# better62/MM-VQA-Healthcare

Hardware: AMD Instinct MI355X
Metric: image-question pairs/sec, M3AE-base fine-tune step (fwd+bwd+AdamW) @384px (higher is better)
Workload: dtype bf16

## Files before the change

include/m3ae_hip.h:

```cpp
#ifndef M3AE_HIP_H
#define M3AE_HIP_H

#include <stdint.h>

#ifdef __cplusplus
extern "C" {
#endif

#define M3AE_ABI_VERSION 4

enum { M3AE_F32 = 0, M3AE_BF16 = 1 };
enum { M3AE_ACT_NONE = 0, M3AE_ACT_GELU = 1, M3AE_ACT_QUICKGELU = 2, M3AE_ACT_TANH = 3, M3AE_ACT_RELU = 4,
       M3AE_ACT_MULAUX = 5  };
enum { M3AE_ERR_ARG = -1, M3AE_ERR_UNSUPPORTED = -2, M3AE_ERR_ALIGN = -3, M3AE_ERR_WORKSPACE = -4 };

int m3ae_abi_version(void);
void m3ae_desc_sizes(int64_t out3[3]);
const char* m3ae_last_gemm_path(void);

typedef struct {
    int64_t M, N, K;
    int64_t batch1, batch2;
    const void* A; int64_t a_sm, a_sk, a_sb1, a_sb2;
    const void* B; int64_t b_sk, b_sn, b_sb1, b_sb2;
    void* C;       int64_t c_sm, c_sn, c_sb1, c_sb2;
    int32_t dtype_a, dtype_b, dtype_c;
    float alpha;
    int32_t accumulate;
    const float* bias;
    int32_t act;
    void* preact;
    const void* residual;
    const void* dact_aux;
    int32_t dact;
    int32_t force_generic;
    float* a_rowsum;
    float dropout_p;
    uint64_t dropout_seed;
    int32_t preact_grad;
    int32_t launch_flags;
    const void* dropout_salt;
} m3ae_gemm_desc;
enum { M3AE_GEMM_NO_PERSISTENT = 1,
       M3AE_GEMM_F32_X3 = 2,
       M3AE_GEMM_DETERMINISTIC = 4  };
#define M3AE_GEMM_NT_VARIANT(v) ((((v) + 1) & 0xf) << 8)
#define M3AE_GEMM_TN_VARIANT(v) ((((v) + 1) & 0xf) << 12)
#define M3AE_GEMM_COL_GROUP(g) (((g) & 0xf) << 16)
int m3ae_gemm(const m3ae_gemm_desc* d, void* stream);
int m3ae_gemm_rows(const m3ae_gemm_desc* d, int64_t row_base, int64_t row_step, void* stream);
int64_t m3ae_gemm_det_workspace_bytes(const m3ae_gemm_desc* d);
int m3ae_gemm_det(const m3ae_gemm_desc* d, void* workspace, int64_t workspace_bytes, void* stream);

typedef struct {
    int64_t B, H, Lq, Lk, Dh;
    const void* q; int64_t q_sb, q_sl;
    const void* k; int64_t k_sb, k_sl;
    const void* v; int64_t v_sb, v_sl;
    void* o;       int64_t o_sb, o_sl;
    const float* key_mask;
    const float* pos_bias;
    float scale;
    int32_t causal;
    float* lse; int64_t lse_stride;
    int32_t dtype;
    void* workspace; int64_t workspace_bytes;
    const void* d_o;
    void* dq; void* dk; void* dv;
    float* delta;
    float* d_pos_bias;
    float dropout_p;
    uint64_t dropout_seed;
    const void* dropout_salt;
    int32_t launch_flags;
} m3ae_attn_desc;
enum { M3AE_ATTN_LEGACY_KERNELS = 1,
       M3AE_ATTN_F32_X3 = 2    };
int64_t m3ae_attn_workspace_bytes(const m3ae_attn_desc* d, int backward);
int m3ae_attn_fwd(const m3ae_attn_desc* d, void* stream);
int m3ae_attn_bwd(const m3ae_attn_desc* d, void* stream);
int m3ae_attn_fwd_rows(const m3ae_attn_desc* d, int64_t row_base, int64_t row_step, void* stream);
int m3ae_attn_bwd_rows(const m3ae_attn_desc* d, int64_t row_base, int64_t row_step, void* stream);
int m3ae_attn_probs(const m3ae_attn_desc* d, float* probs, int64_t p_sb, int64_t p_sh, int64_t p_sq, void* stream);

typedef struct {
    int32_t dir;
    int64_t B, Lq, Lk, D, H;
    const void* x;
    const void* y;
    const float* key_mask;
    const void *wq, *wq_t, *wkv, *wkv_t, *wo, *wo_t;
    const float *bq, *bkv, *bo, *ln_g, *ln_b;
    float ln_eps;
    float dropout_p;
    uint64_t seed_attn, seed_hidden;
    void* proj;
    void* prime;
    float* colbias;
    void* probs;
    void* probs_drop;
    float* rowsum;
    void* zctx;
    void* ctx;
    void* s;
    void* out;
    float *mean, *rstd;
    const void* d_out;
    void* dx;
    void* dy;
    float *g_wq, *g_wkv, *g_wo, *g_bq, *g_bkv, *g_bo, *g_ln_g, *g_ln_b;
    void* ws_ds;
    void* ws_dsd;
    void* ws_dscores;
    void* ws_dprime;
    void* ws_dproj;
    void* ws_dz;
    void* ws_dctx;
    float* ws_vec;
    float* ws_ln;
    int32_t launch_flags;
    const void* dropout_salt;
} m3ae_xattn_desc;
enum { M3AE_XATTN_NO_PERSISTENT = 1,
       M3AE_XATTN_LEGACY_CHAIN = 2     };
int m3ae_xattn_supported(const m3ae_xattn_desc* d);
int m3ae_xattn_bwd_supported(const m3ae_xattn_desc* d);
int64_t m3ae_xattn_probs_ld(const m3ae_xattn_desc* d);
int m3ae_xattn_fwd(const m3ae_xattn_desc* d, void* stream);
int m3ae_xattn_bwd(const m3ae_xattn_desc* d, void* stream);
int m3ae_xattn_probs_export(const m3ae_xattn_desc* d, int dropped, float* out, int64_t o_sb, int64_t o_sh, int64_t o_sq,
                            void* stream);

int m3ae_layernorm_fwd(const void* x, const float* gamma, const float* beta, void* y, float* mean, float* rstd,
                       int64_t M, int64_t D, float eps, int dtype, int act, int rms, void* stream);
int64_t m3ae_layernorm_bwd_blocks(int64_t M);
int m3ae_layernorm_bwd(const void* dy, const void* x, const float* gamma, const float* beta, const float* mean,
                       const float* rstd, void* dx, const void* dx_add, float* dgamma, float* dbeta, float* workspace,
                       int64_t M, int64_t D, int dtype, int act, int rms, void* stream);
int m3ae_layernorm_bwd_drop(const void* dy, const void* x, const float* gamma, const float* beta, const float* mean,
                            const float* rstd, void* dx, void* dx_drop, float dropout_p, uint64_t dropout_seed,
                            const void* dropout_salt, float* dgamma, float* dbeta, float* workspace, int64_t M, int64_t D,
                            int dtype, void* stream);
int m3ae_layernorm_bwd_drop_rows(const void* dy, const void* x, const float* gamma, const float* beta, const float* mean,
                                 const float* rstd, void* dx, void* dx_drop, float dropout_p, uint64_t dropout_seed,
                                 const void* dropout_salt, float* dgamma, float* dbeta, float* workspace, int64_t M, int64_t D,
                                 int dtype, int64_t row_base, int64_t row_step, void* stream);
int m3ae_layernorm_fwd_mixed(const float* x, const float* gamma, const float* beta, void* y, float* mean, float* rstd,
                             int64_t M, int64_t D, float eps, void* stream);
int m3ae_layernorm_bwd_mixed(const void* dy, const float* x, const float* gamma, const float* mean, const float* rstd,
                             float* dx, const float* dx_add, void* dx_lo, float* dgamma, float* dbeta, float* workspace,
                             int64_t M, int64_t D, void* stream);
int m3ae_layernorm_bwd_mixed_det(const void* dy, const float* x, const float* gamma, const float* mean, const float* rstd,
                                 float* dx, const float* dx_add, void* dx_lo, float* dgamma, float* dbeta, float* workspace,
                                 int64_t M, int64_t D, void* stream);
int m3ae_dropout(const void* x, void* out, uint8_t* keep_mask, int64_t rows, int64_t cols, float p, uint64_t seed,
                 const void* salt, int dtype, void* stream);
int m3ae_dropout_rows(const void* x, void* out, uint8_t* keep_mask, int64_t rows, int64_t cols, float p, uint64_t seed,
                      const void* salt, int dtype, int64_t row_base, int64_t row_step, void* stream);

int m3ae_colsum(const void* x, float* out, int64_t M, int64_t N, int64_t ldx, int dtype, int accumulate,
                void* stream);

int m3ae_roberta_embed_fwd(const int64_t* ids, const float* word, const float* pos, const float* type, void* out,
                           int64_t B, int64_t S, int64_t D, int64_t pad_id, int dtype, void* stream);
int m3ae_roberta_embed_bwd(const int64_t* ids, const void* d_out, float* d_word, float* d_pos, float* d_type,
                           int64_t B, int64_t S, int64_t D, int64_t pad_id, int dtype, void* stream);

int m3ae_patchify(const float* img, void* out, int64_t B, int64_t R, int64_t P, int dtype, void* stream);
int m3ae_image_normalize_u8(const uint8_t* in, float* out, int64_t B, int64_t H, int64_t W, const float* mean3,
                            const float* std3, void* stream);
int64_t m3ae_image_resample_workspace_bytes(int64_t total_rows, int64_t size);
int m3ae_image_resample_u8(const uint8_t* src, int64_t src_bytes, const int64_t* plan, const int32_t* tab, int64_t tab_ints, int64_t B,
                           int64_t size, uint8_t* workspace, int64_t workspace_bytes, float* out, uint8_t* out_u8,
                           const float* mean3, const float* std3, void* stream);
int m3ae_vit_tokens_fwd(const void* patch, const float* cls, const float* pos, void* out, int64_t B, int64_t G,
                        int64_t D, int dtype, void* stream);
int m3ae_vit_tokens_bwd(const void* d_out, void* d_patch, float* d_cls, float* d_pos, int64_t B, int64_t G,
                        int64_t D, int dtype, void* stream);

int m3ae_bce_logits(const void* logits, const float* targets, float* loss, void* d_logits, int64_t B, int64_t C,
                    float grad_scale, int dtype, void* stream);
int m3ae_xent(const void* logits, const int64_t* labels, float* loss, void* d_logits, float* workspace,
              int64_t rows, int64_t C, int64_t ld, float grad_scale, int dtype, void* stream);

int m3ae_adamw(float* p, const float* g, float* m, float* v, void* shadow_bf16, int64_t n, float lr, float beta1,
               float beta2, float eps, float wd, int64_t step, float grad_scale, const float* hyper_dev, void* stream);

int m3ae_cast_transpose(const float* in, void* out, void* out_t, int64_t R, int64_t C, void* stream);
int m3ae_cast_transpose_batched(const void* jobs_dev, int njobs, int64_t total_tiles, void* stream);
int m3ae_transpose_bf16_batched(const void* jobs_dev, int njobs, int64_t total_tiles, void* stream);
int m3ae_cast(const void* in, void* out, int64_t n, int dtype_in, int dtype_out, void* stream);
int m3ae_zero(void* p, int64_t bytes, void* stream);
int m3ae_add(const void* a, const void* b, void* out, int64_t n, int dtype, void* stream);
int m3ae_act_fwd(const void* x, void* y, int64_t n, int act, int dtype, void* stream);
int m3ae_act_bwd(const void* dy, const void* x_pre, void* dx, int64_t n, int act, int dtype, void* stream);
int m3ae_gather_rows(const void* in, const int64_t* idx, void* out, int64_t n_out, int64_t D, int dtype,
                     void* stream);
int m3ae_scatter_add_rows(const void* d_out, const int64_t* idx, void* d_in, int64_t n_out, int64_t D, int dtype,
                          void* stream);

int m3ae_mask_ranks(const float* noise, int64_t* ids_restore, int64_t* keep_rows, float* mask, int64_t B, int64_t L,
                    int64_t len_keep, void* stream);
int m3ae_mim_targets(const float* img, float* out, int64_t B, int64_t C, int64_t H, int64_t W, int64_t P, int norm_pix,
                     void* stream);
int m3ae_mim_loss_fwd(const void* x, const float* target, const float* mask, float* acc, float* loss, int64_t B, int64_t L,
                      int64_t D, int dtype, void* stream);
int m3ae_mim_loss_bwd(const void* x, const float* target, const float* mask, const float* acc, const float* gout, void* dx,
                      int64_t B, int64_t L, int64_t D, int dtype, void* stream);

enum { M3AE_DET_COLSUM = 0, M3AE_DET_EMBED_BWD = 1, M3AE_DET_BCE = 2, M3AE_DET_XENT = 3, M3AE_DET_MIM = 4 };
int64_t m3ae_det_workspace_bytes(int op, int64_t rows, int64_t cols);
int m3ae_colsum_det(const void* x, float* out, int64_t M, int64_t N, int64_t ldx, int dtype, int accumulate, void* workspace,
                    int64_t workspace_bytes, void* stream);
int m3ae_layernorm_bwd_det(const void* dy, const void* x, const float* gamma, const float* beta, const float* mean,
                           const float* rstd, void* dx, const void* dx_add, float* dgamma, float* dbeta, float* workspace,
                           int64_t M, int64_t D, int dtype, int act, int rms, void* stream);
int m3ae_layernorm_bwd_drop_det(const void* dy, const void* x, const float* gamma, const float* beta, const float* mean,
                                const float* rstd, void* dx, void* dx_drop, float dropout_p, uint64_t dropout_seed,
                                const void* dropout_salt, float* dgamma, float* dbeta, float* workspace, int64_t M, int64_t D,
                                int dtype, void* stream);
int m3ae_roberta_embed_bwd_det(const int64_t* ids, const void* d_out, float* d_word, float* d_pos, float* d_type, int64_t B,
                               int64_t S, int64_t D, int64_t pad_id, int dtype, void* workspace, int64_t workspace_bytes,
                               void* stream);
int m3ae_bce_logits_det(const void* logits, const float* targets, float* loss, void* d_logits, int64_t B, int64_t C,
                        float grad_scale, int dtype, void* workspace, int64_t workspace_bytes, void* stream);
int m3ae_xent_det(const void* logits, const int64_t* labels, float* loss, void* d_logits, int64_t rows, int64_t C, int64_t ld,
                  float grad_scale, int dtype, void* workspace, int64_t workspace_bytes, void* stream);
int m3ae_mim_loss_fwd_det(const void* x, const float* target, const float* mask, float* acc, float* loss, int64_t B, int64_t L,
                          int64_t D, int dtype, void* workspace, int64_t workspace_bytes, void* stream);

int64_t m3ae_beam_topk_workspace_bytes(int64_t B, int64_t nb, int64_t V, int64_t chunk);
int m3ae_beam_topk(const float* logits, int64_t ld, const float* beam_scores, int64_t B, int64_t nb, int64_t V, int64_t chunk,
                   void* workspace, int64_t workspace_bytes, float* top_s, int32_t* top_i, void* stream);
int m3ae_beam_step(const float* top_s, const int32_t* top_i, const int64_t* ids_in, int64_t* ids_out, int64_t* last_tok,
                   float* beam_scores, int64_t* order, int32_t* done, int32_t* n_hyp, double* hyp_score, int32_t* hyp_len,
                   int64_t* hyp_tok, int32_t* open_count, int64_t* err, int64_t B, int64_t nb, int64_t V, int64_t max_length,
                   int64_t cur_len, int64_t eos, int64_t pad, double div, void* stream);
int m3ae_beam_finalize(const int64_t* ids, const float* beam_scores, const int32_t* done, int32_t* n_hyp, double* hyp_score,
                       int32_t* hyp_len, int64_t* hyp_tok, int64_t* seq, int64_t* len, int64_t B, int64_t nb, int64_t max_length,
                       int64_t cur_len, int64_t eos, int64_t pad, double div, void* stream);

int m3ae_expand_samples(const void* in, const int64_t* src, void* out, int64_t n_out, int64_t n_in, int64_t R, int dtype,
                        void* stream);
int m3ae_segment_sum_rows(const void* d_out, const int64_t* offsets, const int64_t* members, void* d_in, int64_t n_in,
                          int64_t n_out, int64_t R, int dtype, void* stream);

int m3ae_selftest(int32_t* out, void* stream);

#ifdef __cplusplus
}
#endif
#endif
```

mm-vqa-healthcare_amd/csrc/common.h:

```cpp
#pragma once
#include <hip/hip_runtime.h>
#include <stdint.h>
#include "m3ae_hip.h"

typedef uint16_t bf16_t;
typedef __attribute__((ext_vector_type(2))) float f32x2;
typedef __attribute__((ext_vector_type(4))) float f32x4;
typedef __attribute__((ext_vector_type(16))) float f32x16;
typedef __attribute__((ext_vector_type(4))) short s16x4;
typedef __attribute__((ext_vector_type(8))) short s16x8;
typedef __attribute__((ext_vector_type(8))) __bf16 bf16x8_t;
typedef __attribute__((ext_vector_type(4))) unsigned int u32x4;
typedef __attribute__((ext_vector_type(2))) unsigned int u32x2;

#define DEVINL __device__ __forceinline__

DEVINL float bf2f(bf16_t h) { return __uint_as_float(((uint32_t)h) << 16); }
DEVINL bf16_t f2bf(float f) {
    __bf16 b = (__bf16)f;
    return __builtin_bit_cast(bf16_t, b);
}
typedef __attribute__((ext_vector_type(2))) __bf16 bf16x2_t;
DEVINL uint32_t pack2bf(float lo, float hi) {
    const bf16x2_t v = __builtin_convertvector((f32x2){lo, hi}, bf16x2_t);
    return __builtin_bit_cast(uint32_t, v);
}

template <typename T> struct Elem;
template <> struct Elem<float> {
    static DEVINL float ld(const float* p) { return *p; }
    static DEVINL void st(float* p, float v) { *p = v; }
};
template <> struct Elem<bf16_t> {
    static DEVINL float ld(const bf16_t* p) { return bf2f(*p); }
    static DEVINL void st(bf16_t* p, float v) { *p = f2bf(v); }
};

DEVINL float act_fwd(float x, int act) {
    switch (act) {
        case M3AE_ACT_GELU: return 0.5f * x * (1.0f + erff(x * 0.70710678118654752440f));
        case M3AE_ACT_QUICKGELU: return x / (1.0f + expf(-1.702f * x));
        case M3AE_ACT_TANH: return tanhf(x);
        case M3AE_ACT_RELU: return x > 0.f ? x : 0.f;
        default: return x;
    }
}
DEVINL float act_bwd(float x, int act) {
    switch (act) {
        case M3AE_ACT_GELU: {
            float cdf = 0.5f * (1.0f + erff(x * 0.70710678118654752440f));
            float pdf = 0.39894228040143267794f * expf(-0.5f * x * x);
            return cdf + x * pdf;
        }
        case M3AE_ACT_QUICKGELU: {
            float s = 1.0f / (1.0f + expf(-1.702f * x));
            return s * (1.0f + 1.702f * x * (1.0f - s));
        }
        case M3AE_ACT_TANH: {
            float t = tanhf(x);
            return 1.0f - t * t;
        }
        case M3AE_ACT_MULAUX: return x;
        case M3AE_ACT_RELU: return x > 0.f ? 1.f : 0.f;
        default: return 1.0f;
    }
}

DEVINL void gelu_terms_fast(float x, float& cdf, float& pdf) {
    const float z = fabsf(x) * 0.70710678118654752440f;
    const float t = __builtin_amdgcn_rcpf(fmaf(0.3275911f, z, 1.0f));
    const float e = __builtin_amdgcn_exp2f(x * x * -0.72134752044448170368f);
    float poly = fmaf(1.061405429f, t, -1.453152027f);
    poly = fmaf(poly, t, 1.421413741f);
    poly = fmaf(poly, t, -0.284496736f);
    poly = fmaf(poly, t, 0.254829592f);
    const float half_erfc = 0.5f * poly * t * e;
    cdf = x < 0.f ? half_erfc : 1.0f - half_erfc;
    pdf = 0.39894228040143267794f * e;
}
DEVINL float act_fwd_fast(float x, int act) {
    if (act == M3AE_ACT_GELU) {
        float cdf, pdf;
        gelu_terms_fast(x, cdf, pdf);
        return x * cdf;
    }
    if (act == M3AE_ACT_QUICKGELU) return x * __builtin_amdgcn_rcpf(1.0f + __builtin_amdgcn_exp2f(-2.45546695959f * x));
// ... 153 lines not shown
```

mm-vqa-healthcare_amd/csrc/gemm_generic.hip:

```cpp
#include "common.h"

namespace {

constexpr int TM = 64, TN = 64, TK = 16, PAD = 4;

template <typename TA, typename TB, typename TC>
__global__ __launch_bounds__(256) void gemm_generic_kernel(m3ae_gemm_desc d, int64_t row_base, int64_t row_step) {
    __shared__ float As[TK][TM + PAD];
    __shared__ float Bs[TK][TN + PAD];
    const int tid = threadIdx.x;
    const int tx = tid & 15, ty = tid >> 4;
    const int64_t m0 = (int64_t)blockIdx.y * TM, n0 = (int64_t)blockIdx.x * TN;
    const int64_t b1 = blockIdx.z / d.batch2, b2 = blockIdx.z % d.batch2;
    const TA* A = (const TA*)d.A + b1 * d.a_sb1 + b2 * d.a_sb2;
    const TB* B = (const TB*)d.B + b1 * d.b_sb1 + b2 * d.b_sb2;
    const int64_t coff = b1 * d.c_sb1 + b2 * d.c_sb2;
    const bool a_kfast = (d.a_sk == 1), b_nfast = (d.b_sn == 1);

    float acc[4][4];
#pragma unroll
    for (int i = 0; i < 4; ++i)
#pragma unroll
        for (int j = 0; j < 4; ++j) acc[i][j] = 0.f;
    const bool do_rowsum = d.a_rowsum != nullptr && blockIdx.x == 0 && tx == 0;
    float rs[4] = {0.f, 0.f, 0.f, 0.f};

    for (int64_t k0 = 0; k0 < d.K; k0 += TK) {
#pragma unroll
        for (int i = 0; i < 4; ++i) {
            int e = tid + i * 256;
            int mm, kk;
            if (a_kfast) { kk = e & 15; mm = e >> 4; } else { mm = e & 63; kk = e >> 6; }
            int64_t gm = m0 + mm, gk = k0 + kk;
            float v = 0.f;
            if (gm < d.M && gk < d.K) v = Elem<TA>::ld(A + gm * d.a_sm + gk * d.a_sk);
            As[kk][mm] = v;
        }
#pragma unroll
        for (int i = 0; i < 4; ++i) {
            int e = tid + i * 256;
            int nn, kk;
            if (b_nfast) { nn = e & 63; kk = e >> 6; } else { kk = e & 15; nn = e >> 4; }
            int64_t gn = n0 + nn, gk = k0 + kk;
            float v = 0.f;
            if (gn < d.N && gk < d.K) v = Elem<TB>::ld(B + gk * d.b_sk + gn * d.b_sn);
            Bs[kk][nn] = v;
        }
        __syncthreads();
#pragma unroll
        for (int kk = 0; kk < TK; ++kk) {
            float a[4], b[4];
#pragma unroll
            for (int i = 0; i < 4; ++i) a[i] = As[kk][ty * 4 + i];
#pragma unroll
            for (int j = 0; j < 4; ++j) b[j] = Bs[kk][tx * 4 + j];
#pragma unroll
            for (int i = 0; i < 4; ++i)
#pragma unroll
                for (int j = 0; j < 4; ++j) acc[i][j] = fmaf(a[i], b[j], acc[i][j]);
            if (do_rowsum) {
#pragma unroll
                for (int i = 0; i < 4; ++i) rs[i] += a[i];
            }
        }
        __syncthreads();
    }
    if (do_rowsum) {
#pragma unroll
        for (int i = 0; i < 4; ++i) {
            const int64_t gm = m0 + ty * 4 + i;
            if (gm < d.M) d.a_rowsum[gm] += rs[i];
        }
    }

    DropState drop = make_drop_dev(d.dropout_p, d.dropout_seed, d.dropout_salt, row_base, row_step);
    drop_resolve(drop);
    TC* C = (TC*)d.C + coff;
    TC* P = d.preact ? (TC*)d.preact + coff : nullptr;
    const TC* R = d.residual ? (const TC*)d.residual + coff : nullptr;
    const TC* X = d.dact_aux ? (const TC*)d.dact_aux + coff : nullptr;
#pragma unroll
    for (int i = 0; i < 4; ++i) {
        int64_t gm = m0 + ty * 4 + i;
        if (gm >= d.M) continue;
#pragma unroll
        for (int j = 0; j < 4; ++j) {
            int64_t gn = n0 + tx * 4 + j;
            if (gn >= d.N) continue;
            int64_t off = gm * d.c_sm + gn * d.c_sn;
            float x = acc[i][j] * d.alpha;
            if (d.bias) x += d.bias[gn];
            if (P) Elem<TC>::st(P + off, d.preact_grad ? act_bwd(x, d.act) : x);
            x = act_fwd(x, d.act);
            if (d.dropout_p > 0.f) x = drop_apply(drop, (uint64_t)(drop_row(drop, gm) * drop_ld(d.N) + gn), x);
            if (R) x += Elem<TC>::ld(R + off);
            if (X) x *= act_bwd(Elem<TC>::ld(X + off), d.dact);
            if (d.accumulate) x += Elem<TC>::ld(C + off);
            Elem<TC>::st(C + off, x);
        }
    }
}

template <typename TA, typename TB, typename TC>
int launch(const m3ae_gemm_desc& d, hipStream_t s, DropRows rows) {
    dim3 grid((unsigned)cdiv(d.N, TN), (unsigned)cdiv(d.M, TM), (unsigned)(d.batch1 * d.batch2));
    if (grid.y > 65535u || grid.z > 65535u) return M3AE_ERR_UNSUPPORTED;
    hipLaunchKernelGGL((gemm_generic_kernel<TA, TB, TC>), grid, dim3(256), 0, s, d, rows.base, rows.step);
    return hip_launch_status();
}

}

int m3ae_gemm_generic(const m3ae_gemm_desc& d, hipStream_t s, DropRows rows) {
    if (d.dtype_a != d.dtype_b) return M3AE_ERR_UNSUPPORTED;
    if (d.dtype_a == M3AE_F32 && d.dtype_c == M3AE_F32) return launch<float, float, float>(d, s, rows);
    if (d.dtype_a == M3AE_BF16 && d.dtype_c == M3AE_BF16) return launch<bf16_t, bf16_t, bf16_t>(d, s, rows);
    if (d.dtype_a == M3AE_BF16 && d.dtype_c == M3AE_F32) return launch<bf16_t, bf16_t, float>(d, s, rows);
    return M3AE_ERR_UNSUPPORTED;
}
```

mm-vqa-healthcare_amd/csrc/gemm_mfma.hip:

```cpp
#include "gemm_nt_common.h"
#include "launch.h"
#include <stdlib.h>

namespace {

constexpr int BM = 128, BN = 128, BK = 64;
constexpr int STAGE_BYTES = (BM + BN) * BK * 2;
constexpr int LDS_BYTES = 2 * STAGE_BYTES;

using namespace m3g;

template <int BM_, int BN_, int BKT, int NST, int WM, int EPI>
__global__ __launch_bounds__((BM_ / WM) * (BN_ / 64) * 64, 2) void gemm_nt_bf16_kernel(MfmaArgs a) {
    if (a.has_drop) drop_resolve(a.drop);
    constexpr int WAVES_N = BN_ / 64, NWAVES = (BM_ / WM) * WAVES_N, MI = WM / 16;
    constexpr int A_BYTES = BM_ * BKT * 2, ST_BYTES = (BM_ + BN_) * BKT * 2;
    constexpr int A_SEGS = A_BYTES / 1024 / NWAVES, B_SEGS = BN_ * BKT * 2 / 1024 / NWAVES;
    constexpr int G = A_SEGS + B_SEGS;
    extern __shared__ __attribute__((aligned(16))) char smem[];
    const int tid = threadIdx.x;
    const int lane = tid & 63;
    const int wave = __builtin_amdgcn_readfirstlane(tid >> 6);
    const int wr = wave / WAVES_N, wc = wave % WAVES_N;

    const unsigned tiles_n = (unsigned)((a.N + BN_ - 1) / BN_);
    unsigned tm, tn;
    nt_tile_coords(xcd_remap(blockIdx.x, gridDim.x), gridDim.x / tiles_n, tiles_n, tm, tn);
    const int64_t m0 = (int64_t)tm * BM_;
    const int64_t n0 = (int64_t)tn * BN_;

    f32x4 acc[MI][4];
#pragma unroll
    for (int i = 0; i < MI; ++i)
#pragma unroll
        for (int j = 0; j < 4; ++j) acc[i][j] = (f32x4){0.f, 0.f, 0.f, 0.f};

    const int nt = (int)(a.K / BKT);
#pragma unroll
    for (int s = 0; s < NST - 1; ++s) {
        if (s < nt) {
            nt_stage<BKT, A_SEGS, NWAVES>(a.A, a.lda, m0, a.M, (int64_t)s * BKT, smem + s * ST_BYTES, wave, lane);
            nt_stage<BKT, B_SEGS, NWAVES>(a.B, a.ldb, n0, a.N, (int64_t)s * BKT, smem + s * ST_BYTES + A_BYTES, wave, lane);
        }
    }

    const int frow = lane & 15, fchunk = lane >> 4;
    int cur_s = 0, nxt_s = NST - 1;
    for (int t = 0; t < nt; ++t) {
        if (t + NST - 2 < nt) asm volatile("s_waitcnt vmcnt(%0)" ::"n"((NST - 2) * G) : "memory");
        else asm volatile("s_waitcnt vmcnt(0)" ::: "memory");
        __builtin_amdgcn_s_barrier();
        asm volatile("" ::: "memory");
        if (t + NST - 1 < nt) {
            char* nxt = smem + nxt_s * ST_BYTES;
            nt_stage<BKT, A_SEGS, NWAVES>(a.A, a.lda, m0, a.M, (int64_t)(t + NST - 1) * BKT, nxt, wave, lane);
            nt_stage<BKT, B_SEGS, NWAVES>(a.B, a.ldb, n0, a.N, (int64_t)(t + NST - 1) * BKT, nxt + A_BYTES, wave, lane);
        }
        const char* At = smem + cur_s * ST_BYTES;
        const char* Bt = At + A_BYTES;
#pragma unroll
        for (int kk = 0; kk < BKT / 32; ++kk) {
            s16x8 af[MI], bfr[4];
#pragma unroll
            for (int j = 0; j < 4; ++j) bfr[j] = nt_frag<BKT>(Bt, wc * 64 + j * 16 + frow, kk * 4 + fchunk);
#pragma unroll
            for (int i = 0; i < MI; ++i) af[i] = nt_frag<BKT>(At, wr * WM + i * 16 + frow, kk * 4 + fchunk);
#pragma unroll
            for (int i = 0; i < MI; ++i)
#pragma unroll
                for (int j = 0; j < 4; ++j)
                    acc[i][j] = __builtin_amdgcn_mfma_f32_16x16x32_bf16(
                        __builtin_bit_cast(bf16x8_t, bfr[j]), __builtin_bit_cast(bf16x8_t, af[i]), acc[i][j], 0, 0, 0);
        }
        asm volatile("" ::: "memory");
        cur_s = cur_s + 1 == NST ? 0 : cur_s + 1;
        nxt_s = nxt_s + 1 == NST ? 0 : nxt_s + 1;
    }

    if (a.rows_epi) {
        __builtin_amdgcn_s_barrier();
        asm volatile("" ::: "memory");
        if (a.c_f32) epilogue_rows<float, EPI, MI>(a, smem, wave, lane, m0 + wr * WM, n0 + wc * 64, acc);
        else epilogue_rows<bf16_t, EPI, MI>(a, smem, wave, lane, m0 + wr * WM, n0 + wc * 64, acc);
        return;
    }
#pragma unroll
    for (int i = 0; i < MI; ++i) {
        const int64_t m = m0 + wr * WM + i * 16 + (lane & 15);
        if (m >= a.M) continue;
#pragma unroll
        for (int j = 0; j < 4; ++j) {
            const int64_t n = n0 + wc * 64 + j * 16 + 4 * (lane >> 4);
            if (n >= a.N) continue;
            if (a.c_f32) epilogue4<float, EPI>(a, m, n, acc[i][j]);
            else epilogue4<bf16_t, EPI>(a, m, n, acc[i][j]);
        }
    }
}

template <int BM_, int BN_, int WM, int BKR, int NST, bool DET = false>
__global__ __launch_bounds__((BM_ / WM) * (BN_ / 64) * 64, 2) void gemm_tn_bf16_kernel(MfmaArgs a) {
    constexpr int WAVES_N = BN_ / 64, NWAVES = (BM_ / WM) * WAVES_N, MI = WM / 16;
    constexpr int A_BYTES = BM_ * BKR * 2, ST_BYTES = (BM_ + BN_) * BKR * 2;
    constexpr int A_SEGS = A_BYTES / 1024 / NWAVES, B_SEGS = BN_ * BKR * 2 / 1024 / NWAVES;
    constexpr int G = A_SEGS + B_SEGS;
    extern __shared__ __attribute__((aligned(16))) char smem[];
    const int tid = threadIdx.x;
    const int lane = tid & 63;
    const int wave = __builtin_amdgcn_readfirstlane(tid >> 6);
    const int wr = wave / WAVES_N, wc = wave % WAVES_N;

    const unsigned tiles_n = (unsigned)(a.N / BN_);
    const unsigned tiles = (unsigned)(a.M / BM_) * tiles_n;
    const unsigned wg = xcd_remap(blockIdx.x, gridDim.x);
    const unsigned tile_id = wg % tiles, split = wg / tiles;
    const int64_t m0 = (int64_t)(tile_id / tiles_n) * BM_;
    const int64_t n0 = (int64_t)(tile_id % tiles_n) * BN_;
    const int64_t r_begin = (int64_t)split * a.k_chunk;
    int64_t r_end = r_begin + a.k_chunk;
    if (r_end > a.K) r_end = a.K;
    if (r_begin >= r_end) return;
    const int nt = (int)((r_end - r_begin + BKR - 1) / BKR);

    f32x4 acc[MI][4];
#pragma unroll
    for (int i = 0; i < MI; ++i)
#pragma unroll
        for (int j = 0; j < 4; ++j) acc[i][j] = (f32x4){0.f, 0.f, 0.f, 0.f};

    const bool do_rowsum = a.a_rowsum != nullptr && n0 == 0 && wc == 0;
    f32x4 rsum[MI];
#pragma unroll
    for (int i = 0; i < MI; ++i) rsum[i] = (f32x4){0.f, 0.f, 0.f, 0.f};
    const s16x8 ones = {0x3F80, 0x3F80, 0x3F80, 0x3F80, 0x3F80, 0x3F80, 0x3F80, 0x3F80};

#pragma unroll
    for (int s = 0; s < NST - 1; ++s) {
        if (s < nt) {
            const int64_t r0 = r_begin + (int64_t)s * BKR;
// ... 45 lines not shown
#pragma unroll
            for (int i = 0; i < MI; ++i) *(f32x4*)(rs + i * 16) = rsum[i];
        }
        float* P = (float*)a.C + ((int64_t)split * tiles + tile_id) * (BM_ * BN_) + ((int64_t)wave * MI * 4 * 64 + lane) * 4;
#pragma unroll
        for (int i = 0; i < MI; ++i)
#pragma unroll
            for (int j = 0; j < 4; ++j) *(f32x4*)(P + (i * 4 + j) * 256) = acc[i][j];
        return;
    }
    if (do_rowsum && (lane & 15) == 0) {
#pragma unroll
        for (int i = 0; i < MI; ++i)
#pragma unroll
            for (int r = 0; r < 4; ++r) atomicAdd(a.a_rowsum + m0 + wr * WM + i * 16 + 4 * (lane >> 4) + r, rsum[i][r]);
    }

    float* C = (float*)a.C;
    const bool atomic = a.splits > 1;
#pragma unroll
    for (int i = 0; i < MI; ++i)
#pragma unroll
        for (int j = 0; j < 4; ++j)
#pragma unroll
            for (int r = 0; r < 4; ++r) {
                const int64_t n1 = m0 + wr * WM + i * 16 + 4 * (lane >> 4) + r;
                const int64_t n2 = n0 + wc * 64 + j * 16 + (lane & 15);
                float* p = C + n1 * a.ldc + n2;
                const float x = acc[i][j][r] * a.alpha;
                if (atomic) atomicAdd(p, x);
                else if (a.accumulate) *p += x;
                else *p = x;
            }
}

}

static thread_local const char* g_last_path = "none";
const char* m3ae_last_gemm_path(void) { return g_last_path; }

int m3ae_gemm_generic(const m3ae_gemm_desc& d, hipStream_t s, DropRows rows = DropRows{0, 1});
int m3ae_gemm_f32x3(const m3ae_gemm_desc& d, hipStream_t s, DropRows rows = DropRows{0, 1});

static bool aligned16(const void* p) { return (((uintptr_t)p) & 15) == 0; }


template <int BM_, int BN_, int BKT, int NST, int WM, int EPI>
static int launch_nt_t(const MfmaArgs& a, hipStream_t s) {
    constexpr int nwaves = (BM_ / WM) * (BN_ / 64);
    constexpr int ring = NST * (BM_ + BN_) * BKT * 2, slabs = nwaves * 32 * 68 * 4;
    constexpr int lds = ring > slabs ? ring : slabs;
    constexpr int threads = nwaves * 64;
    const int64_t tiles = cdiv(a.M, BM_) * cdiv(a.N, BN_);
    return launch_dyn<gemm_nt_bf16_kernel<BM_, BN_, BKT, NST, WM, EPI>>(dim3((unsigned)tiles), dim3(threads), lds, s, a);
}


#if defined(M3AE_EXP_NT_NODMA)
#define PP_STAGE(G, ld, r0, nr, k0, tile) do { } while (0)
#elif defined(M3AE_EXP_NT_CONTIG)
template <int BKT, int SEGS_PER_WAVE, int NWAVES>
DEVINL void nt_stage_contig(const bf16_t* G, int64_t ld, int64_t row0, int64_t nrows, int64_t k0, char* tile, int wave, int lane) {
    constexpr int CPR = BKT / 8, RPS = 64 / CPR;
#pragma unroll
    for (int q = 0; q < SEGS_PER_WAVE; ++q) {
        const int seg = q * NWAVES + wave;
        const int row = seg * RPS + lane / CPR;
        int64_t grow = row0 + row;
        grow = grow < nrows ? grow : nrows - 1;
        glds16(G + (k0 / BKT) * nrows * BKT + grow * BKT + (lane % CPR) * 8, tile + seg * 1024);
    }
}
#ifdef M3AE_EXP_NT_L2HOT
#define PP_STAGE(G, ld, r0, nr, k0, tile) nt_stage_contig<CK, 2, NW>(G, ld, 0, nr, k0, tile, wave, lane)
#else
#define PP_STAGE(G, ld, r0, nr, k0, tile) nt_stage_contig<CK, 2, NW>(G, ld, r0, nr, k0, tile, wave, lane)
#endif
#elif defined(M3AE_EXP_NT_L2HOT)
#define PP_STAGE(G, ld, r0, nr, k0, tile) nt_stage<CK, 2, NW>(G, ld, 0, nr, k0, tile, wave, lane)
#else
#define PP_STAGE(G, ld, r0, nr, k0, tile) nt_stage<CK, 2, NW>(G, ld, r0, nr, k0, tile, wave, lane)
#endif

template <int EPI>
__global__ __launch_bounds__(512, 2) void gemm_nt_pp_kernel(MfmaArgs a) {
    if (a.has_drop) drop_resolve(a.drop);
    constexpr int CK = 32, NW = 8, A_BYTES = 256 * CK * 2, SLOT = 2 * A_BYTES;
    extern __shared__ __attribute__((aligned(16))) char smem[];
    const int tid = threadIdx.x;
    const int lane = tid & 63;
    const int wave = __builtin_amdgcn_readfirstlane(tid >> 6);
    const int wr = wave >> 2, wc = wave & 3;

    const unsigned tiles_n = (unsigned)((a.N + 255) / 256);
    unsigned tm, tn;
    nt_tile_coords(xcd_remap(blockIdx.x, gridDim.x), gridDim.x / tiles_n, tiles_n, tm, tn, (unsigned)a.col_group);
    const int64_t m0 = (int64_t)tm * 256;
    const int64_t n0 = (int64_t)tn * 256;

    f32x4 acc[8][4];
#pragma unroll
    for (int i = 0; i < 8; ++i)
#pragma unroll
        for (int j = 0; j < 4; ++j) acc[i][j] = (f32x4){0.f, 0.f, 0.f, 0.f};

    const int nc = (int)(a.K / CK);
#pragma unroll
    for (int c = 0; c < 3; ++c) {
        if (c < nc) {
            PP_STAGE(a.B, a.ldb, n0, a.N, (int64_t)c * CK, smem + c * SLOT + A_BYTES);
            PP_STAGE(a.A, a.lda, m0, a.M, (int64_t)c * CK, smem + c * SLOT);
        }
    }
    if (nc >= 3) asm volatile("s_waitcnt vmcnt(8)" ::: "memory");
    else if (nc == 2) asm volatile("s_waitcnt vmcnt(4)" ::: "memory");
    else asm volatile("s_waitcnt vmcnt(0)" ::: "memory");
    PP_FENCE();
    __builtin_amdgcn_s_barrier();
    PP_FENCE();
    if (wr == 1) { __builtin_amdgcn_s_barrier(); PP_FENCE(); }

    const int frow = lane & 15, fchunk = lane >> 4;
    for (int c = 0; c < nc; ++c) {
        const char* At = smem + (c & 3) * SLOT;
        const char* Bt = At + A_BYTES;
        char* nxt = smem + ((c + 3) & 3) * SLOT;
        const bool more = c + 3 < nc;
        s16x8 bfr[4], af[4];
#pragma unroll
        for (int j = 0; j < 4; ++j) bfr[j] = nt_frag<CK>(Bt, wc * 64 + j * 16 + frow, fchunk);
#pragma unroll
        for (int i = 0; i < 4; ++i) af[i] = nt_frag<CK>(At, wr * 128 + i * 16 + frow, fchunk);
        if (more) PP_STAGE(a.B, a.ldb, n0, a.N, (int64_t)(c + 3) * CK, nxt + A_BYTES);
        PP_FENCE();
        __builtin_amdgcn_s_barrier();
        PP_FENCE();
        asm volatile("s_waitcnt lgkmcnt(0)" ::: "memory");
        __builtin_amdgcn_sched_barrier(0);
        __builtin_amdgcn_s_setprio(1);
#pragma unroll
        for (int i = 0; i < 4; ++i)
#pragma unroll
            for (int j = 0; j < 4; ++j)
                acc[i][j] = __builtin_amdgcn_mfma_f32_16x16x32_bf16(
                    __builtin_bit_cast(bf16x8_t, bfr[j]), __builtin_bit_cast(bf16x8_t, af[i]), acc[i][j], 0, 0, 0);
        __builtin_amdgcn_s_setprio(0);
        PP_FENCE();
        __builtin_amdgcn_s_barrier();
        PP_FENCE();
#pragma unroll
        for (int i = 0; i < 4; ++i) af[i] = nt_frag<CK>(At, wr * 128 + 64 + i * 16 + frow, fchunk);
        if (more) PP_STAGE(a.A, a.lda, m0, a.M, (int64_t)(c + 3) * CK, nxt);
        {
            const int rem = nc - 1 - c;
            if (rem >= 3) asm volatile("s_waitcnt vmcnt(8)" ::: "memory");
            else if (rem == 2) asm volatile("s_waitcnt vmcnt(4)" ::: "memory");
            else asm volatile("s_waitcnt vmcnt(0)" ::: "memory");
        }
        PP_FENCE();
        __builtin_amdgcn_s_barrier();
        PP_FENCE();
        asm volatile("s_waitcnt lgkmcnt(0)" ::: "memory");
        __builtin_amdgcn_sched_barrier(0);
        __builtin_amdgcn_s_setprio(1);
#pragma unroll
        for (int i = 0; i < 4; ++i)
#pragma unroll
            for (int j = 0; j < 4; ++j)
                acc[4 + i][j] = __builtin_amdgcn_mfma_f32_16x16x32_bf16(
                    __builtin_bit_cast(bf16x8_t, bfr[j]), __builtin_bit_cast(bf16x8_t, af[i]), acc[4 + i][j], 0, 0, 0);
        __builtin_amdgcn_s_setprio(0);
        PP_FENCE();
        __builtin_amdgcn_s_barrier();
        PP_FENCE();
    }
    if (wr == 0) { __builtin_amdgcn_s_barrier(); PP_FENCE(); }

    if (a.rows_epi) {
        if (a.c_f32) epilogue_rows<float, EPI, 8>(a, smem, wave, lane, m0 + wr * 128, n0 + wc * 64, acc);
        else epilogue_rows<bf16_t, EPI, 8>(a, smem, wave, lane, m0 + wr * 128, n0 + wc * 64, acc);
        return;
    }
#pragma unroll
    for (int i = 0; i < 8; ++i) {
        const int64_t m = m0 + wr * 128 + i * 16 + (lane & 15);
        if (m >= a.M) continue;
#pragma unroll
        for (int j = 0; j < 4; ++j) {
            const int64_t n = n0 + wc * 64 + j * 16 + 4 * (lane >> 4);
            if (n >= a.N) continue;
            if (a.c_f32) epilogue4<float, EPI>(a, m, n, acc[i][j]);
            else epilogue4<bf16_t, EPI>(a, m, n, acc[i][j]);
        }
    }
}

template <int EPI>
static int launch_nt_pp(const MfmaArgs& a, hipStream_t s) {
    constexpr int lds = 4 * (256 + 256) * 32 * 2;
    const int64_t tiles = cdiv(a.M, 256) * cdiv(a.N, 256);
    g_last_path = "mfma_nt_pp";
    return launch_dyn<gemm_nt_pp_kernel<EPI>>(dim3((unsigned)tiles), dim3(512), lds, s, a);
}


#ifdef M3AE_NT_TRACE
__device__ uint64_t g_nt_trace[1024 * 2 * 8];
#define NT_CLK() ({ __builtin_amdgcn_sched_barrier(0); uint64_t t_ = __builtin_readcyclecounter(); __builtin_amdgcn_sched_barrier(0); t_; })
#define NT_ACC(i) do { const uint64_t n_ = NT_CLK(); nt_acc[i] += n_ - nt_t; nt_t = n_; } while (0)
#else
#define NT_ACC(i) do { } while (0)
#endif

template <int EPI>
__global__ __launch_bounds__(512, 2) void gemm_nt_pp_persistent_kernel(MfmaArgs a) {
    if (a.has_drop) drop_resolve(a.drop);
    constexpr int CK = 32, NW = 8, A_BYTES = 256 * CK * 2, SLOT = 2 * A_BYTES;
    extern __shared__ __attribute__((aligned(16))) char smem[];
    const int tid = threadIdx.x;
    const int lane = tid & 63;
    const int wave = __builtin_amdgcn_readfirstlane(tid >> 6);
    const int wr = wave >> 2, wc = wave & 3;
    const unsigned tiles_n = (unsigned)((a.N + 255) / 256);
    const unsigned tiles_m = (unsigned)((a.M + 255) / 256);
    const unsigned total = tiles_m * tiles_n;
    const int nc = (int)(a.K / CK);
    const int frow = lane & 15, fchunk = lane >> 4;

    unsigned v = blockIdx.x;
    unsigned tm, tn;
    nt_tile_coords(xcd_remap(v, total), tiles_m, tiles_n, tm, tn, (unsigned)a.col_group);
    int64_t m0 = (int64_t)tm * 256, n0 = (int64_t)tn * 256;
#pragma unroll
    for (int c = 0; c < 3; ++c) {
        char* sl = smem + ((c + 2) & 3) * SLOT;
        PP_STAGE(a.B, a.ldb, n0, a.N, (int64_t)c * CK, sl + A_BYTES);
        PP_STAGE(a.A, a.lda, m0, a.M, (int64_t)c * CK, sl);
    }
    int top_wait = 0;
#ifdef M3AE_NT_TRACE
    uint64_t nt_acc[8] = {0, 0, 0, 0, 0, 0, 0, 0}, nt_t = 0;
#endif
    const int interior_wait = a.c_f32 ? 1 : (a.preact ? 3 : 2);
    for (;;) {
        f32x4 acc[8][4];
#pragma unroll
        for (int i = 0; i < 8; ++i)
#pragma unroll
            for (int j = 0; j < 4; ++j) acc[i][j] = (f32x4){0.f, 0.f, 0.f, 0.f};
        if (top_wait == 0) asm volatile("s_waitcnt vmcnt(8)" ::: "memory");
        else if (top_wait == 2) asm volatile("s_waitcnt vmcnt(20)" ::: "memory");
        else if (top_wait == 3) asm volatile("s_waitcnt vmcnt(36)" ::: "memory");
        else asm volatile("s_waitcnt vmcnt(4)" ::: "memory");
        PP_FENCE();
        __builtin_amdgcn_s_barrier();
        PP_FENCE();
        if (wr == 1) { __builtin_amdgcn_s_barrier(); PP_FENCE(); }
#ifdef M3AE_NT_TRACE
        nt_t = NT_CLK();
#endif
        for (int c = 0; c < nc; ++c) {
            const char* At = smem + ((c + 2) & 3) * SLOT;
            const char* Bt = At + A_BYTES;
            char* nxt = smem + ((c + 5) & 3) * SLOT;
            const bool more = c + 3 < nc;
            s16x8 bfr[4], af[4];
#pragma unroll
            for (int j = 0; j < 4; ++j) bfr[j] = nt_frag<CK>(Bt, wc * 64 + j * 16 + frow, fchunk);
#pragma unroll
            for (int i = 0; i < 4; ++i) af[i] = nt_frag<CK>(At, wr * 128 + i * 16 + frow, fchunk);
            NT_ACC(0);
            if (more) PP_STAGE(a.B, a.ldb, n0, a.N, (int64_t)(c + 3) * CK, nxt + A_BYTES);
            NT_ACC(1);
            PP_FENCE();
            __builtin_amdgcn_s_barrier();
            PP_FENCE();
            NT_ACC(2);
            asm volatile("s_waitcnt lgkmcnt(0)" ::: "memory");
            __builtin_amdgcn_sched_barrier(0);
            NT_ACC(3);
            __builtin_amdgcn_s_setprio(1);
#pragma unroll
            for (int i = 0; i < 4; ++i)
#pragma unroll
                for (int j = 0; j < 4; ++j)
                    acc[i][j] = __builtin_amdgcn_mfma_f32_16x16x32_bf16(
                        __builtin_bit_cast(bf16x8_t, bfr[j]), __builtin_bit_cast(bf16x8_t, af[i]), acc[i][j], 0, 0, 0);
            __builtin_amdgcn_s_setprio(0);
            NT_ACC(4);
            PP_FENCE();
            __builtin_amdgcn_s_barrier();
            PP_FENCE();
            NT_ACC(5);
#pragma unroll
            for (int i = 0; i < 4; ++i) af[i] = nt_frag<CK>(At, wr * 128 + 64 + i * 16 + frow, fchunk);
            NT_ACC(0);
            if (more) PP_STAGE(a.A, a.lda, m0, a.M, (int64_t)(c + 3) * CK, nxt);
            NT_ACC(1);
            {
                const int rem = nc - 1 - c;
                if (rem >= 3) asm volatile("s_waitcnt vmcnt(8)" ::: "memory");
                else if (rem == 2) asm volatile("s_waitcnt vmcnt(4)" ::: "memory");
                else asm volatile("s_waitcnt vmcnt(0)" ::: "memory");
            }
            NT_ACC(6);
            PP_FENCE();
            __builtin_amdgcn_s_barrier();
            PP_FENCE();
            NT_ACC(2);
            asm volatile("s_waitcnt lgkmcnt(0)" ::: "memory");
            __builtin_amdgcn_sched_barrier(0);
            NT_ACC(3);
            __builtin_amdgcn_s_setprio(1);
#pragma unroll
            for (int i = 0; i < 4; ++i)
#pragma unroll
                for (int j = 0; j < 4; ++j)
                    acc[4 + i][j] = __builtin_amdgcn_mfma_f32_16x16x32_bf16(
                        __builtin_bit_cast(bf16x8_t, bfr[j]), __builtin_bit_cast(bf16x8_t, af[i]), acc[4 + i][j], 0, 0, 0);
            __builtin_amdgcn_s_setprio(0);
            NT_ACC(4);
            PP_FENCE();
            __builtin_amdgcn_s_barrier();
            PP_FENCE();
            NT_ACC(5);
        }
#ifdef M3AE_NT_TRACE
        nt_acc[7] += (uint64_t)nc;
#endif
        if (wr == 0) { __builtin_amdgcn_s_barrier(); PP_FENCE(); }
        const unsigned vn = v + gridDim.x;
        const bool again = vn < total;
        const int64_t m_cur = m0, n_cur = n0;
        if (again) {
            nt_tile_coords(xcd_remap(vn, total), tiles_m, tiles_n, tm, tn, (unsigned)a.col_group);
            m0 = (int64_t)tm * 256; n0 = (int64_t)tn * 256;
#pragma unroll
            for (int c = 0; c < 2; ++c) {
                char* sl = smem + ((c + 2) & 3) * SLOT;
                PP_STAGE(a.B, a.ldb, n0, a.N, (int64_t)c * CK, sl + A_BYTES);
                PP_STAGE(a.A, a.lda, m0, a.M, (int64_t)c * CK, sl);
            }
        }
        if (a.c_f32) epilogue_rows<float, EPI, 8, 1>(a, smem, wave, lane, m_cur + wr * 128, n_cur + wc * 64, acc);
        else epilogue_rows<bf16_t, EPI, 8, 1>(a, smem, wave, lane, m_cur + wr * 128, n_cur + wc * 64, acc);
#ifdef M3AE_NT_TRACE
        if (!again && lane == 0 && (wave & 3) == 0 && blockIdx.x < 1024)
            for (int q_ = 0; q_ < 8; ++q_) g_nt_trace[((size_t)blockIdx.x * 2 + wr) * 8 + q_] = nt_acc[q_];
#endif
        if (!again) break;
        top_wait = (m_cur + 256 <= a.M && n_cur + 256 <= a.N) ? interior_wait : 1;
        PP_FENCE();
        __builtin_amdgcn_s_barrier();
        PP_FENCE();
        {
            char* sl = smem + ((2 + 2) & 3) * SLOT;
            PP_STAGE(a.B, a.ldb, n0, a.N, (int64_t)2 * CK, sl + A_BYTES);
            PP_STAGE(a.A, a.lda, m0, a.M, (int64_t)2 * CK, sl);
        }
        v = vn;
    }
}

template <int EPI>
static int launch_nt_pp_persistent(const MfmaArgs& a, hipStream_t s) {
    constexpr int lds = 4 * (256 + 256) * 32 * 2;
    g_last_path = "mfma_nt_pp";
    const int dev = current_device();
    return launch_dyn_on<gemm_nt_pp_persistent_kernel<EPI>>(dev, dim3((unsigned)device_cus8(dev)), dim3(512), lds, s, a);
}

template <int EPI>
static int launch_nt_v(const MfmaArgs& a, hipStream_t s) {
    const int g_nt_variant = a.nt_variant;
    if (g_nt_variant < 0) {
        const int64_t t256 = cdiv(a.M, 256) * cdiv(a.N, 256), t128 = cdiv(a.M, 128) * cdiv(a.N, 128);
        const double eff256 = (double)t256 / (double)(cdiv(t256, 256) * 256);
        const double eff128 = (double)t128 / (double)(cdiv(t128, 512) * 512);
        const bool big = a.M > 128 && a.N > 128 && eff256 >= 0.93 * eff128;
        const bool persist_ok = t256 >= 512;
        if (big && a.rows_epi && a.K >= 256) {
            g_last_path = "mfma_nt_pp2";
            return launch_nt_pp2(a, EPI, persist_ok && !a.no_persist, s);
        }
        if (big && persist_ok && !a.no_persist && a.rows_epi && a.K >= 96) return launch_nt_pp_persistent<EPI>(a, s);
        if (big) return launch_nt_pp<EPI>(a, s);
        return launch_nt_t<128, 128, 64, 2, 64, EPI>(a, s);
    }
    if ((g_nt_variant == 9 || g_nt_variant == 10) && a.M > 128 && a.N > 128 && a.rows_epi && a.K >= 256) {
        g_last_path = "mfma_nt_pp2";
        return launch_nt_pp2(a, EPI, g_nt_variant == 10, s);
    }
    if (g_nt_variant == 7 && a.M > 128 && a.N > 128) return launch_nt_pp<EPI>(a, s);
    if (g_nt_variant == 8 && a.rows_epi && a.K >= 96 && cdiv(a.M, 256) * cdiv(a.N, 256) >= 512)
        return launch_nt_pp_persistent<EPI>(a, s);
    if (g_nt_variant == 8 && a.M > 128 && a.N > 128) return launch_nt_pp<EPI>(a, s);
    if (g_nt_variant == 4 && a.M > 128 && a.N > 128) return launch_nt_t<256, 256, 64, 2, 128, EPI>(a, s);
    return launch_nt_t<128, 128, 64, 2, 64, EPI>(a, s);
}

static int launch_nt(const m3ae_gemm_desc& d, hipStream_t s, DropRows rows) {
    MfmaArgs a{};
    a.A = (const bf16_t*)d.A; a.lda = d.a_sm;
    a.B = (const bf16_t*)d.B; a.ldb = d.b_sn;
    a.C = d.C; a.ldc = d.c_sm;
    a.M = d.M; a.N = d.N; a.K = d.K;
    a.c_f32 = d.dtype_c == M3AE_F32;
    a.alpha = d.alpha; a.accumulate = d.accumulate; a.bias = d.bias; a.act = d.act; a.preact = d.preact;
    a.preact_grad = d.preact_grad;
    a.residual = d.residual; a.dact_aux = d.dact_aux; a.dact = d.dact;
    a.rows_epi = (d.N % 8 == 0 && d.c_sm % 8 == 0) ? 1 : 0;
    {
        const int tiles_n = (int)((d.N + 255) / 256);
        const int g_nt_col_group = (d.launch_flags >> 16) & 0xf;
        a.col_group = g_nt_col_group > 0 ? g_nt_col_group : (tiles_n <= 9 ? tiles_n : 6);
    }
    a.has_drop = d.dropout_p > 0.f;
    a.drop = make_drop(d.dropout_p, d.dropout_seed, d.dropout_salt, rows);
    a.no_persist = (d.launch_flags & M3AE_GEMM_NO_PERSISTENT) ? 1 : 0;
    a.nt_variant = ((d.launch_flags >> 8) & 0xf) - 1;
    a.st_policy = (d.launch_flags >> 20) & 0x3;
    if (a.st_policy == 0) a.st_policy = (d.M * d.N >= (int64_t)16 << 20) ? 3 : 1;
    const bool has_act = d.act != M3AE_ACT_NONE, has_dact = d.dact_aux != nullptr;
    if (!has_act && !has_dact && !d.preact) return launch_nt_v<EPI_PLAIN>(a, s);
    if (!has_dact && d.act == M3AE_ACT_RELU) return launch_nt_v<EPI_RELU>(a, s);
    if (!has_act && has_dact && d.dact == M3AE_ACT_MULAUX) return launch_nt_v<EPI_DMUL>(a, s);
    if (a.has_drop) return launch_nt_v<EPI_ANY>(a, s);
    if (!has_dact && d.act == M3AE_ACT_GELU) return launch_nt_v<EPI_GELU>(a, s);
    if (!has_dact && d.act == M3AE_ACT_QUICKGELU) return launch_nt_v<EPI_QGELU>(a, s);
    if (!has_act && d.dact == M3AE_ACT_GELU) return launch_nt_v<EPI_DGELU>(a, s);
    if (!has_act && d.dact == M3AE_ACT_QUICKGELU) return launch_nt_v<EPI_DQGELU>(a, s);
    return launch_nt_v<EPI_ANY>(a, s);
}


#ifdef M3AE_TN_TRACE
__device__ uint64_t g_tn_trace[512 * 2 * 16];
#define TN_STAMP(k) do { if (tn_tr) g_tn_trace[((size_t)blockIdx.x * 2 + wr) * 16 + (k)] = __builtin_readcyclecounter(); } while (0)
extern "C" int m3ae_tn_trace_dump(uint64_t* out) {
    hipDeviceSynchronize();
    hipMemcpyFromSymbol(out, HIP_SYMBOL(g_tn_trace), sizeof(uint64_t) * 512 * 2 * 16);
    static uint64_t zeros[512 * 2 * 16];
    hipMemcpyToSymbol(HIP_SYMBOL(g_tn_trace), zeros, sizeof(zeros));
    return 0;
}
#else
#define TN_STAMP(k) do { } while (0)
#endif
template <bool DET>
__global__ __launch_bounds__(512, 2) void gemm_tn_pp_kernel(MfmaArgs a) {
    constexpr int CK = 32, NW = 8, A_BYTES = 256 * CK * 2, SLOT = 2 * A_BYTES;
    extern __shared__ __attribute__((aligned(16))) char smem[];
    const int tid = threadIdx.x;
    const int lane = tid & 63;
    const int wave = __builtin_amdgcn_readfirstlane(tid >> 6);
    const int wr = wave >> 2, wc = wave & 3;

    const unsigned tiles_n = (unsigned)(a.N / 256);
    const unsigned tiles = (unsigned)(a.M / 256) * tiles_n;
    const unsigned wg = xcd_remap(blockIdx.x, gridDim.x);
    const unsigned tile_id = wg % tiles, split = wg / tiles;
    const int64_t m0 = (int64_t)(tile_id / tiles_n) * 256;
    const int64_t n0 = (int64_t)(tile_id % tiles_n) * 256;
    const int64_t r_begin = (int64_t)split * a.k_chunk;
    int64_t r_end = r_begin + a.k_chunk;
    if (r_end > a.K) r_end = a.K;
    if (r_begin >= r_end) return;
    const int nc = (int)((r_end - r_begin + CK - 1) / CK);

    f32x4 acc[8][4];
#pragma unroll
    for (int i = 0; i < 8; ++i)
#pragma unroll
        for (int j = 0; j < 4; ++j) acc[i][j] = (f32x4){0.f, 0.f, 0.f, 0.f};
    const bool do_rowsum = a.a_rowsum != nullptr && n0 == 0 && wc == 0;
    f32x4 rsum[8];
#pragma unroll
    for (int i = 0; i < 8; ++i) rsum[i] = (f32x4){0.f, 0.f, 0.f, 0.f};
    const s16x8 ones = {0x3F80, 0x3F80, 0x3F80, 0x3F80, 0x3F80, 0x3F80, 0x3F80, 0x3F80};

#pragma unroll
    for (int c = 0; c < 3; ++c) {
        if (c < nc) {
            const int64_t r0 = r_begin + (int64_t)c * CK;
            tn_stage<256, 2, NW>(a.B, a.ldb, r0, r_end, n0, smem + c * SLOT + A_BYTES, wave, lane);
            tn_stage<256, 2, NW>(a.A, a.lda, r0, r_end, m0, smem + c * SLOT, wave, lane);
        }
    }
    if (nc >= 3) asm volatile("s_waitcnt vmcnt(8)" ::: "memory");
    else if (nc == 2) asm volatile("s_waitcnt vmcnt(4)" ::: "memory");
    else asm volatile("s_waitcnt vmcnt(0)" ::: "memory");
    PP_FENCE();
    __builtin_amdgcn_s_barrier();
    PP_FENCE();
    if (wr == 1) { __builtin_amdgcn_s_barrier(); PP_FENCE(); }

    for (int c = 0; c < nc; ++c) {
#ifdef M3AE_TN_TRACE
        const bool tn_tr = (c == 64 || c == 65) && lane == 0 && wc == 0 && blockIdx.x < 512;
        if (tn_tr && c == 65) g_tn_trace[((size_t)blockIdx.x * 2 + wr) * 16 + 8] = __builtin_readcyclecounter();
#undef TN_STAMP
#define TN_STAMP(k) do { if (tn_tr && c == 64) g_tn_trace[((size_t)blockIdx.x * 2 + wr) * 16 + (k)] = __builtin_readcyclecounter(); } while (0)
#endif
// ... 206 lines not shown
    if (splits > ksteps / min_steps) splits = ksteps / min_steps;
    if (splits < 1) splits = 1;
    if (!d.accumulate) splits = 1;
    const int64_t steps_per = cdiv(ksteps, splits);
    *k_chunk = steps_per * 64;
    return cdiv(ksteps, steps_per);
}

template <int BM_, int BN_, int WM, int BKR, int NST>
static int launch_tn_t(MfmaArgs a, const m3ae_gemm_desc& d, hipStream_t s, float* det_ws = nullptr) {
    static_assert(BM_ == 128 && BN_ == 128, "tn_t_splits and tn_det_fold assume the 128 x 128 tile");
    constexpr int lds = tn_t_lds(NST, BKR);
    constexpr int threads = (BM_ / WM) * (BN_ / 64) * 64;
    const int64_t tiles = (d.M / BM_) * (d.N / BN_);
    const int64_t splits = tn_t_splits(d, lds, &a.k_chunk);
    a.splits = (int)splits;
    if (det_ws) return tn_run<gemm_tn_bf16_kernel<BM_, BN_, WM, BKR, NST, true>>(a, d, tiles * splits, threads, lds, BM_, WM, det_ws, s);
    return tn_run<gemm_tn_bf16_kernel<BM_, BN_, WM, BKR, NST>>(a, d, tiles * splits, threads, lds, BM_, WM, nullptr, s);
}

static int tn_kernel_choice(const m3ae_gemm_desc& d) {
    const bool pp_ok = d.M % 256 == 0 && d.N % 256 == 0 && d.K >= 4096;
    const int g_tn_variant = ((d.launch_flags >> 12) & 0xf) - 1;
    if (g_tn_variant == 5 && pp_ok) return 5;
    if (g_tn_variant < 0 || g_tn_variant == 6) {
        const bool r3_rule = pp_ok && (d.K >= 65536 || (d.K >= 32768 && d.M * d.N >= 768 * 3072));
        const bool r4_rule = pp_ok && d.K >= 65536 && d.M * d.N >= 768 * 3072;
        if (g_tn_variant == 6 ? r3_rule : r4_rule) return 5;
        return 2;
    }
    if (g_tn_variant == 2) return 2;
    return 0;
}

static int launch_tn(const m3ae_gemm_desc& d, hipStream_t s, float* det_ws = nullptr) {
    MfmaArgs a{};
    a.A = (const bf16_t*)d.A; a.lda = d.a_sk;
    a.B = (const bf16_t*)d.B; a.ldb = d.b_sk;
    a.C = d.C; a.ldc = d.c_sm;
    a.M = d.M; a.N = d.N; a.K = d.K;
    a.c_f32 = 1; a.alpha = d.alpha; a.accumulate = d.accumulate; a.a_rowsum = d.a_rowsum;
    const int k = tn_kernel_choice(d);
    if (k == 5) return launch_tn_pp(a, d, s, det_ws);
    if (k == 2) return launch_tn_t<128, 128, 64, 32, 2>(a, d, s, det_ws);
    return launch_tn_t<128, 128, 64, 64, 2>(a, d, s, det_ws);
}

#ifdef M3AE_NT_TRACE
extern "C" int m3ae_nt_trace_dump(uint64_t* host_out) {
    return (int)hipMemcpyFromSymbol(host_out, HIP_SYMBOL(g_nt_trace), sizeof(uint64_t) * 1024 * 2 * 8);
}
#endif

enum GemmRoute { ROUTE_BAD_DIMS, ROUTE_F32X3, ROUTE_NT, ROUTE_TN, ROUTE_GENERIC };
static GemmRoute gemm_route(const m3ae_gemm_desc& d) {
    if (d.M <= 0 || d.N <= 0 || d.K <= 0 || d.batch1 <= 0 || d.batch2 <= 0) return ROUTE_BAD_DIMS;
    if ((d.launch_flags & M3AE_GEMM_F32_X3) && !d.force_generic) return ROUTE_F32X3;
    const bool bf = d.dtype_a == M3AE_BF16 && d.dtype_b == M3AE_BF16;
    const bool single = d.batch1 == 1 && d.batch2 == 1;
    if (bf && single && !d.force_generic && d.c_sn == 1) {
        const bool ptr_ok = aligned16(d.A) && aligned16(d.B) && aligned16(d.C) &&
                            (!d.preact || aligned16(d.preact)) && (!d.residual || aligned16(d.residual)) &&
                            (!d.dact_aux || aligned16(d.dact_aux)) && (!d.bias || aligned16(d.bias));
        if (ptr_ok && !d.a_rowsum && d.a_sk == 1 && d.b_sk == 1 && d.K % BK == 0 && d.N % 4 == 0 && d.a_sm % 8 == 0 &&
            d.b_sn % 8 == 0 && d.c_sm % 4 == 0)
            return ROUTE_NT;
        if (ptr_ok && d.a_sm == 1 && d.b_sn == 1 && d.dtype_c == M3AE_F32 && d.M % BM == 0 && d.N % BN == 0 &&
            d.a_sk % 8 == 0 && d.b_sk % 8 == 0 && !d.bias && d.act == M3AE_ACT_NONE && !d.preact && !d.residual &&
            !d.dact_aux)
            return ROUTE_TN;
    }
    return ROUTE_GENERIC;
}

extern "C" int m3ae_gemm(const m3ae_gemm_desc* dp, void* stream) { return m3ae_gemm_rows(dp, 0, 1, stream); }

extern "C" int m3ae_gemm_rows(const m3ae_gemm_desc* dp, int64_t row_base, int64_t row_step, void* stream) {
    if (!dp || !dp->A || !dp->B || !dp->C) return M3AE_ERR_ARG;
    const m3ae_gemm_desc& d = *dp;
    const GemmRoute route = gemm_route(d);
    if (route == ROUTE_BAD_DIMS) return M3AE_ERR_ARG;
    const DropRows rows{row_base, row_step};
    if (!drop_rows_ok(rows, d.M, d.N)) return M3AE_ERR_ARG;
    if (route == ROUTE_TN && d.dropout_p > 0.f && (row_base != 0 || row_step != 1)) return M3AE_ERR_UNSUPPORTED;
    if (d.launch_flags & M3AE_GEMM_DETERMINISTIC) return M3AE_ERR_UNSUPPORTED;
    hipStream_t s = (hipStream_t)stream;
    switch (route) {
    case ROUTE_F32X3:
        if (d.dtype_a != M3AE_F32 || d.dtype_b != M3AE_F32 || d.dtype_c != M3AE_F32) return M3AE_ERR_UNSUPPORTED;
        g_last_path = "f32x3";
        return m3ae_gemm_f32x3(d, s, rows);
    case ROUTE_NT:
        g_last_path = "mfma_nt";
        return launch_nt(d, s, rows);
    case ROUTE_TN:
        g_last_path = "mfma_tn";
        return launch_tn(d, s);
    default:
        g_last_path = "generic";
        return m3ae_gemm_generic(d, s, rows);
    }
}

extern "C" int64_t m3ae_gemm_det_workspace_bytes(const m3ae_gemm_desc* dp) {
    if (!dp) return M3AE_ERR_ARG;
    const m3ae_gemm_desc& d = *dp;
    if (gemm_route(d) != ROUTE_TN) return 0;
    int64_t k_chunk = 0;
    const int k = tn_kernel_choice(d);
    const int64_t splits = k == 5 ? tn_pp_splits(d, &k_chunk) : tn_t_splits(d, tn_t_lds(2, k == 2 ? 32 : 64), &k_chunk);
    return tn_det_bytes(d, splits);
}

extern "C" int m3ae_gemm_det(const m3ae_gemm_desc* dp, void* workspace, int64_t workspace_bytes, void* stream) {
    if (!dp || !dp->A || !dp->B || !dp->C) return M3AE_ERR_ARG;
    const m3ae_gemm_desc& d = *dp;
    if (!(d.launch_flags & M3AE_GEMM_DETERMINISTIC)) return M3AE_ERR_ARG;
    if (gemm_route(d) != ROUTE_TN) return M3AE_ERR_UNSUPPORTED;
    if (!workspace || !aligned16(workspace) || workspace_bytes < m3ae_gemm_det_workspace_bytes(dp)) return M3AE_ERR_WORKSPACE;
    g_last_path = "mfma_tn";
    return launch_tn(d, (hipStream_t)stream, (float*)workspace);
}
```

mm-vqa-healthcare_amd/csrc/gemm_nt_common.h:

```cpp
#pragma once
#include "mfma_tiles.h"

namespace m3g {

enum { EPI_PLAIN = 0, EPI_GELU = 1, EPI_QGELU = 2, EPI_DGELU = 3, EPI_DQGELU = 4, EPI_ANY = 5, EPI_DMUL = 6, EPI_RELU = 7 };

struct MfmaArgs {
    const bf16_t* A; int64_t lda;
    const bf16_t* B; int64_t ldb;
    void* C; int64_t ldc;
    int64_t M, N, K;
    int c_f32;
    float alpha;
    int accumulate;
    const float* bias;
    int act;
    void* preact;
    int preact_grad;
    const void* residual;
    const void* dact_aux;
    int dact;
    float* a_rowsum;
    DropState drop;
    int has_drop;
    int rows_epi;
    int splits;
    int64_t k_chunk;
    int col_group;
    int no_persist;
    int nt_variant;
    int st_policy;
};

DEVINL void nt_tile_coords(unsigned wg, unsigned tiles_m, unsigned tiles_n, unsigned& tm, unsigned& tn, unsigned GC = 4) {
    const unsigned per_group = tiles_m * GC;
    const unsigned g = wg / per_group;
    const unsigned first = g * GC;
    const unsigned gc = tiles_n - first < GC ? tiles_n - first : GC;
    const unsigned local = wg - g * per_group;
    tm = local / gc;
    tn = first + local % gc;
}

template <typename TC> struct Vec4;
template <> struct Vec4<float> {
    static DEVINL void ld(const float* p, float* x) {
        const f32x4 v = *(const f32x4*)p;
        x[0] = v[0]; x[1] = v[1]; x[2] = v[2]; x[3] = v[3];
    }
    static DEVINL void st(float* p, const float* x) { *(f32x4*)p = (f32x4){x[0], x[1], x[2], x[3]}; }
};
template <> struct Vec4<bf16_t> {
    static DEVINL void ld(const bf16_t* p, float* x) {
        const u32x2 v = *(const u32x2*)p;
        x[0] = __uint_as_float(v[0] << 16); x[1] = __uint_as_float(v[0] & 0xffff0000u);
        x[2] = __uint_as_float(v[1] << 16); x[3] = __uint_as_float(v[1] & 0xffff0000u);
    }
    static DEVINL void st(bf16_t* p, const float* x) { *(u32x2*)p = (u32x2){pack2bf(x[0], x[1]), pack2bf(x[2], x[3])}; }
};

template <typename TC, int EPI>
DEVINL void epilogue4(const MfmaArgs& a, int64_t m, int64_t n, f32x4 v) {
    const int64_t off = m * a.ldc + n;
    float x[4] = {v[0] * a.alpha, v[1] * a.alpha, v[2] * a.alpha, v[3] * a.alpha};
    float y[4];
    if (a.bias) {
        Vec4<float>::ld(a.bias + n, y);
#pragma unroll
        for (int t = 0; t < 4; ++t) x[t] += y[t];
    }
    if (EPI == EPI_GELU || EPI == EPI_QGELU || EPI == EPI_RELU || EPI == EPI_ANY) {
        const int act = EPI == EPI_GELU ? M3AE_ACT_GELU : (EPI == EPI_QGELU ? M3AE_ACT_QUICKGELU : (EPI == EPI_RELU ? M3AE_ACT_RELU : a.act));
        if (a.preact && a.preact_grad) {
            float dd[4];
            act_fwd_grad_fast_n<4>(x, dd, act);
            Vec4<TC>::st((TC*)a.preact + off, dd);
        } else {
            if (a.preact) Vec4<TC>::st((TC*)a.preact + off, x);
            act_fwd_fast_n<4>(x, act);
        }
    }
    if ((EPI == EPI_PLAIN || EPI == EPI_ANY || EPI == EPI_RELU || EPI == EPI_DMUL) && a.has_drop) {
        drop_apply4(a.drop, (uint64_t)(drop_row(a.drop, m) * a.N + n), x);
    }
    if (a.residual) {
        Vec4<TC>::ld((const TC*)a.residual + off, y);
#pragma unroll
        for (int t = 0; t < 4; ++t) x[t] += y[t];
    }
    if (EPI == EPI_DMUL) {
        Vec4<TC>::ld((const TC*)a.dact_aux + off, y);
#pragma unroll
        for (int t = 0; t < 4; ++t) x[t] *= y[t];
    }
    if (EPI == EPI_DGELU || EPI == EPI_DQGELU || EPI == EPI_ANY) {
        if (a.dact_aux) {
            const int dact = EPI == EPI_DGELU ? M3AE_ACT_GELU : (EPI == EPI_DQGELU ? M3AE_ACT_QUICKGELU : a.dact);
            Vec4<TC>::ld((const TC*)a.dact_aux + off, y);
            act_bwd_mul_fast_n<4>(x, y, dact);
        }
    }
    if (a.accumulate) {
        Vec4<TC>::ld((const TC*)a.C + off, y);
#pragma unroll
        for (int t = 0; t < 4; ++t) x[t] += y[t];
    }
    Vec4<TC>::st((TC*)a.C + off, x);
}

template <typename TC> struct Vec8;
template <> struct Vec8<float> {
    static DEVINL void unpack(const u32x4&, float*) {}
    static DEVINL void ld(const float* p, float* x) { Vec4<float>::ld(p, x); Vec4<float>::ld(p + 4, x + 4); }
    static DEVINL void st(float* p, const float* x) { Vec4<float>::st(p, x); Vec4<float>::st(p + 4, x + 4); }
// ... 176 lines not shown
```

mm-vqa-healthcare_amd/csrc/gemm_nt_pp2.hip:

```cpp
#include "gemm_nt_common.h"
#include "launch.h"

using namespace m3g;

#ifdef M3AE_EXP_PP2_CLOCK
__device__ uint64_t g_pp2_clock[2 * 256];
extern "C" int m3ae_diag_pp2_clock(uint64_t* out, int n) {
    return hipMemcpyFromSymbol(out, HIP_SYMBOL(g_pp2_clock), (size_t)n * sizeof(uint64_t)) == hipSuccess ? 0 : 1;
}
#endif

namespace {

template <int BASE> DEVINL void wait_vm_s(int s) {
    if (s == 0) asm volatile("s_waitcnt vmcnt(%0)" ::"n"(BASE) : "memory");
    else if (s == 16) asm volatile("s_waitcnt vmcnt(%0)" ::"n"(BASE + 16) : "memory");
    else asm volatile("s_waitcnt vmcnt(%0)" ::"n"(BASE + 32) : "memory");
}

DEVINL void glds16_asm(const void* base, unsigned voff, unsigned dst) {
    unsigned keep;
    asm volatile("s_mov_b32 %0, m0\n\ts_mov_b32 m0, %3\n\ts_nop 0\n\tglobal_load_lds_dwordx4 %1, %2\n\ts_mov_b32 m0, %0"
                 : "=&s"(keep) : "v"(voff), "s"(base), "s"(dst) : "memory");
}
// ... 21 lines not shown
        for (int p = 0; p < 2; ++p) L.pre[i][p] = (u32x4){0u, 0u, 0u, 0u};
    const int64_t m_last = a.M - 1;
    if (EPI == EPI_ANY) {
        if (L.has_bias) {
            L.bias[0] = *(const u32x4*)(a.bias + ncol);
            L.bias[1] = *(const u32x4*)(a.bias + ncol + 4);
        }
        if (L.has_pre) {
#pragma unroll
            for (int i = 0; i < 8; ++i)
#pragma unroll
                for (int p = 0; p < 2; ++p) {
                    const int64_t m = m_base + 16 * i + p * 8 + (lane >> 3);
                    L.pre[i][p] = *(const u32x4*)(src + (m < m_last ? m : m_last) * a.ldc + ncol);
                }
        }
        return;
    }
    if (L.has_bias) {
        gload16_asm(L.bias[0], a.bias + ncol);
        gload16_asm(L.bias[1], a.bias + ncol + 4);
    }
    if (L.has_pre) {
        if (a.st_policy >= 3) {
#pragma unroll
            for (int i = 0; i < 8; ++i)
#pragma unroll
                for (int p = 0; p < 2; ++p) {
                    const int64_t m = m_base + 16 * i + p * 8 + (lane >> 3);
                    gload16_asm_nt(L.pre[i][p], src + (m < m_last ? m : m_last) * a.ldc + ncol);
                }
        } else {
#pragma unroll
            for (int i = 0; i < 8; ++i)
#pragma unroll
                for (int p = 0; p < 2; ++p) {
                    const int64_t m = m_base + 16 * i + p * 8 + (lane >> 3);
                    gload16_asm(L.pre[i][p], src + (m < m_last ? m : m_last) * a.ldc + ncol);
                }
        }
    }
}

template <typename TC, int EPI>
DEVINL void epi_wait_loads(EpiLoads<TC, EPI>& L, bool prefetched) {
    if (EPI == EPI_ANY) return;
    if (prefetched) asm volatile("s_waitcnt vmcnt(16)" ::: "memory");
    else asm volatile("s_waitcnt vmcnt(0)" ::: "memory");
    asm volatile("" : "+v"(L.bias[0]), "+v"(L.bias[1]));
#pragma unroll
    for (int i = 0; i < 8; ++i) asm volatile("" : "+v"(L.pre[i][0]), "+v"(L.pre[i][1]));
}

template <typename TC, int EPI>
DEVINL void epi_finish(const MfmaArgs& a, float* slab, int lane, int64_t m_base, int64_t n_base, f32x4 (&acc)[8][4],
                       EpiLoads<TC, EPI>& L, bool prefetched) {
    const int wrow = lane & 15, wq = lane >> 4;
    const int rq = lane & 7;
    float bias8[8];
#pragma unroll
    for (int i = 0; i < 8; ++i) {
#pragma unroll
        for (int j = 0; j < 4; ++j) *(f32x4*)(slab + wrow * 64 + (((4 * j + wq) ^ wrow) << 2)) = acc[i][j];
        if (i == 0) {
            epi_wait_loads(L, prefetched);
#pragma unroll
            for (int t = 0; t < 8; ++t) {
                const u32x4 v = L.bias[t >> 2];
                bias8[t] = __uint_as_float(v[t & 3]);
            }
        }
#pragma unroll
        for (int p = 0; p < 2; ++p) {
            const int row = p * 8 + (lane >> 3);
            const f32x4 v0 = *(const f32x4*)(slab + row * 64 + (((2 * rq) ^ row) << 2));
            const f32x4 v1 = *(const f32x4*)(slab + row * 64 + (((2 * rq + 1) ^ row) << 2));
            float x[8] = {v0[0], v0[1], v0[2], v0[3], v1[0], v1[1], v1[2], v1[3]};
            const int64_t m = m_base + 16 * i + row, n = n_base + rq * 8;
            if (m < a.M && n < a.N) epilogue8<TC, EPI>(a, m, n, x, bias8, L.has_pre, L.pre[i][p]);
        }
    }
}

template <int EPI>
__global__ __launch_bounds__(512, 2) void gemm_nt_pp2_kernel(MfmaArgs a) {
    if (a.has_drop) drop_resolve(a.drop);
    constexpr int CK = 32, A_BYTES = 256 * CK * 2, SLOT = 2 * A_BYTES, RING = 4 * SLOT;
    extern __shared__ __attribute__((aligned(16))) char smem[];
    const int tid = threadIdx.x;
    const int lane = tid & 63;
    const int wave = __builtin_amdgcn_readfirstlane(tid >> 6);
    const int wr = wave >> 2, wc = wave & 3;
    const unsigned tiles_n = (unsigned)((a.N + 255) / 256);
    const unsigned tiles_m = (unsigned)((a.M + 255) / 256);
    const unsigned total = tiles_m * tiles_n;
    const int nc = (int)(a.K / CK);
    constexpr int npre = 4;
    const int frow = lane & 15, fchunk = lane >> 4;
    const unsigned lds_wave = (unsigned)(uintptr_t)(lds_void*)smem + (unsigned)wave * 1024u;
    unsigned v = blockIdx.x;
    if (v >= total) return;
#ifdef M3AE_EXP_PP2_STAGGER
    {
        const unsigned k = (blockIdx.x >> 3) & 3u;
        const uint64_t t0 = __builtin_readcyclecounter();
        while (__builtin_readcyclecounter() - t0 < (uint64_t)k * M3AE_EXP_PP2_STAGGER) __builtin_amdgcn_s_sleep(32);
    }
#endif
    unsigned tm, tn;
    nt_tile_coords(xcd_remap(v, total), tiles_m, tiles_n, tm, tn, (unsigned)a.col_group);
    int64_t m0 = (int64_t)tm * 256, n0 = (int64_t)tn * 256;

    const bf16_t *abase, *bbase;
    unsigned va0, va1, vb0, vb1;
    auto set_ptrs = [&]() {
        int lane_p = lane;
        asm volatile("" : "+v"(lane_p));
        const int r0 = wave * 16 + (lane_p >> 2), r1 = r0 + 128;
        const unsigned c0 = (unsigned)(((lane_p & 3) ^ nt_swz<CK>(r0)) * 16), c1 = (unsigned)(((lane_p & 3) ^ nt_swz<CK>(r1)) * 16);
        const int ma = (int)(a.M - 1 - m0 < 255 ? a.M - 1 - m0 : 255), mb = (int)(a.N - 1 - n0 < 255 ? a.N - 1 - n0 : 255);
        abase = a.A + m0 * a.lda;
        bbase = a.B + n0 * a.ldb;
        va0 = (unsigned)(r0 < ma ? r0 : ma) * (unsigned)a.lda * 2u + c0;
        va1 = (unsigned)(r1 < ma ? r1 : ma) * (unsigned)a.lda * 2u + c1;
        vb0 = (unsigned)(r0 < mb ? r0 : mb) * (unsigned)a.ldb * 2u + c0;
        vb1 = (unsigned)(r1 < mb ? r1 : mb) * (unsigned)a.ldb * 2u + c1;
    };
    auto issue_b = [&](int c) {
        const unsigned dst = lds_wave + (unsigned)(c & 3) * SLOT + A_BYTES;
        glds16_asm(bbase + (int64_t)c * CK, vb0, dst);
        glds16_asm(bbase + (int64_t)c * CK, vb1, dst + 8192u);
    };
    auto issue_a = [&](int c) {
        const unsigned dst = lds_wave + (unsigned)(c & 3) * SLOT;
        glds16_asm(abase + (int64_t)c * CK, va0, dst);
        glds16_asm(abase + (int64_t)c * CK, va1, dst + 8192u);
    };
    set_ptrs();
    for (int c = 0; c < npre; ++c) { issue_b(c); issue_a(c); }

#ifdef M3AE_EXP_PP2_CLOCK
    const uint64_t clk_c0 = __builtin_amdgcn_s_memtime(), clk_r0 = __builtin_amdgcn_s_memrealtime();
#endif
    int s_prev = 0;
    const int s_interior = a.c_f32 || a.accumulate ? 0 : (a.preact ? 32 : 16);
    for (;;) {
        f32x4 acc[8][4];
#pragma unroll
        for (int i = 0; i < 8; ++i)
#pragma unroll
            for (int j = 0; j < 4; ++j) acc[i][j] = (f32x4){0.f, 0.f, 0.f, 0.f};
        wait_vm_s<12>(s_prev);
        PP_FENCE();
        __builtin_amdgcn_s_barrier();
        PP_FENCE();
        if (wr == 1) { __builtin_amdgcn_s_barrier(); PP_FENCE(); }

        for (int c = 0; c < nc; ++c) {
            unsigned slot_off = (unsigned)(c & 3) * SLOT;
            asm volatile("" : "+s"(slot_off));
            const char* At = smem + slot_off;
            const char* Bt = At + A_BYTES;
            const bool issue = c >= 1 && c + 3 < nc;
            auto wait_next = [&]() {
                if (c >= 3 && c + 3 < nc) asm volatile("s_waitcnt vmcnt(8)" ::: "memory");
                else if (c < 3) wait_vm_s<8>(s_prev);
                else if (c == nc - 3) asm volatile("s_waitcnt vmcnt(4)" ::: "memory");
                else if (c == nc - 2) asm volatile("s_waitcnt vmcnt(0)" ::: "memory");
            };
            s16x8 bfr[4];
            {
                s16x8 af[4];
#pragma unroll
                for (int j = 0; j < 4; ++j) bfr[j] = nt_frag<CK>(Bt, wc * 64 + j * 16 + frow, fchunk);
#pragma unroll
                for (int i = 0; i < 4; ++i) af[i] = nt_frag<CK>(At, wr * 128 + i * 16 + frow, fchunk);
                if (issue) issue_b(c + 3);
                asm volatile("s_waitcnt lgkmcnt(0)" ::: "memory");
                PP_FENCE();
                __builtin_amdgcn_s_barrier();
                PP_FENCE();
                __builtin_amdgcn_s_setprio(1);
#pragma unroll
                for (int i = 0; i < 4; ++i)
#pragma unroll
                    for (int j = 0; j < 4; ++j)
                        acc[i][j] = __builtin_amdgcn_mfma_f32_16x16x32_bf16(
                            __builtin_bit_cast(bf16x8_t, bfr[j]), __builtin_bit_cast(bf16x8_t, af[i]), acc[i][j], 0, 0, 0);
                __builtin_amdgcn_s_setprio(0);
                PP_FENCE();
                __builtin_amdgcn_s_barrier();
                PP_FENCE();
#ifndef M3AE_EXP_PP2_HALFREADS
#pragma unroll
                for (int i = 0; i < 4; ++i) af[i] = nt_frag<CK>(At, wr * 128 + 64 + i * 16 + frow, fchunk);
#endif
                if (issue) issue_a(c + 3);
                wait_next();
                asm volatile("s_waitcnt lgkmcnt(0)" ::: "memory");
                PP_FENCE();
                __builtin_amdgcn_s_barrier();
                PP_FENCE();
                __builtin_amdgcn_s_setprio(1);
#pragma unroll
                for (int i = 0; i < 4; ++i)
#pragma unroll
                    for (int j = 0; j < 4; ++j)
                        acc[4 + i][j] = __builtin_amdgcn_mfma_f32_16x16x32_bf16(
                            __builtin_bit_cast(bf16x8_t, bfr[j]), __builtin_bit_cast(bf16x8_t, af[i]), acc[4 + i][j], 0, 0, 0);
                __builtin_amdgcn_s_setprio(0);
                PP_FENCE();
                __builtin_amdgcn_s_barrier();
                PP_FENCE();
            }
        }
        if (wr == 0) { __builtin_amdgcn_s_barrier(); PP_FENCE(); }
        const unsigned vn = v + gridDim.x;
        const bool again = vn < total;
        const int64_t m_cur = m0 + wr * 128, n_cur = n0 + wc * 64;
        const bool interior = m0 + 256 <= a.M && n0 + 256 <= a.N;
        auto prefetch_next = [&]() {
            if (again) {
                nt_tile_coords(xcd_remap(vn, total), tiles_m, tiles_n, tm, tn, (unsigned)a.col_group);
                m0 = (int64_t)tm * 256; n0 = (int64_t)tn * 256;
                set_ptrs();
                for (int c = 0; c < npre; ++c) { issue_b(c); issue_a(c); }
            }
        };
        int lane_e = lane;
        asm volatile("" : "+v"(lane_e));
        float* slab = (float*)(smem + RING) + wave * 1024;
        if (a.c_f32) {
            EpiLoads<float, EPI> L;
            epi_issue_loads<float, EPI>(a, lane_e, m_cur, n_cur, L);
            prefetch_next();
            epi_finish<float, EPI>(a, slab, lane_e, m_cur, n_cur, acc, L, again);
        } else {
            EpiLoads<bf16_t, EPI> L;
            epi_issue_loads<bf16_t, EPI>(a, lane_e, m_cur, n_cur, L);
            prefetch_next();
            epi_finish<bf16_t, EPI>(a, slab, lane_e, m_cur, n_cur, acc, L, again);
        }
#ifdef M3AE_EXP_PP2_CLOCK
        if (!again && tid == 0 && blockIdx.x < 256) {
            g_pp2_clock[2 * blockIdx.x] = __builtin_amdgcn_s_memtime() - clk_c0;
            g_pp2_clock[2 * blockIdx.x + 1] = __builtin_amdgcn_s_memrealtime() - clk_r0;
        }
#endif
        if (!again) break;
        s_prev = interior ? s_interior : 0;
        v = vn;
    }
}

template <int EPI>
int launch_pp2_t(const MfmaArgs& a, bool persistent, hipStream_t s) {
    constexpr int lds = 4 * (256 + 256) * 32 * 2 + 8 * 4096;
    const int dev = current_device();
    const int64_t tiles = cdiv(a.M, 256) * cdiv(a.N, 256), cus = device_cus8(dev);
    const unsigned grid = (unsigned)(persistent && tiles > cus ? cus : tiles);
    return launch_dyn_on<gemm_nt_pp2_kernel<EPI>>(dev, dim3(grid), dim3(512), lds, s, a);
}

int launch_pp2_e(const MfmaArgs& a, int epi, bool persistent, hipStream_t s) {
    switch (epi) {
        case EPI_PLAIN: return launch_pp2_t<EPI_PLAIN>(a, persistent, s);
        case EPI_GELU: return launch_pp2_t<EPI_GELU>(a, persistent, s);
        case EPI_QGELU: return launch_pp2_t<EPI_QGELU>(a, persistent, s);
        case EPI_DGELU: return launch_pp2_t<EPI_DGELU>(a, persistent, s);
        case EPI_DQGELU: return launch_pp2_t<EPI_DQGELU>(a, persistent, s);
        case EPI_DMUL: return launch_pp2_t<EPI_DMUL>(a, persistent, s);
        case EPI_RELU: return launch_pp2_t<EPI_RELU>(a, persistent, s);
        default: return launch_pp2_t<EPI_ANY>(a, persistent, s);
    }
}

}

int m3g::launch_nt_pp2(const MfmaArgs& a, int epi, bool persistent, hipStream_t s) { return launch_pp2_e(a, epi, persistent, s); }
```

mm-vqa-healthcare_amd/csrc/mfma_tiles.h:

```cpp
#pragma once
#include "common.h"

typedef __attribute__((address_space(3))) void lds_void;
typedef __attribute__((address_space(1))) const void gbl_cvoid;

static __device__ __attribute__((aligned(256))) uint32_t g_m3ae_zero_page[64];

#define PP_FENCE() do { asm volatile("" ::: "memory"); __builtin_amdgcn_sched_barrier(0); } while (0)

DEVINL unsigned xcd_remap(unsigned bid, unsigned nwg) {
    const unsigned q = nwg >> 3, r = nwg & 7, xcd = bid & 7;
    const unsigned base = (xcd < r) ? xcd * (q + 1) : r * (q + 1) + (xcd - r) * q;
    return base + (bid >> 3);
}

DEVINL void glds16(const void* src, char* lds_dst_uniform) {
    __builtin_amdgcn_global_load_lds((gbl_cvoid*)src, (lds_void*)lds_dst_uniform, 16, 0, 0);
}
DEVINL void glds16_raw(const void* src, char* lds_dst_uniform) {
    unsigned keep;
    const unsigned dst = (unsigned)(uintptr_t)(lds_void*)lds_dst_uniform;
    asm volatile("s_mov_b32 %0, m0\n\ts_mov_b32 m0, %2\n\ts_nop 0\n\tglobal_load_lds_dwordx4 %1, off\n\ts_mov_b32 m0, %0"
                 : "=&s"(keep) : "v"(src), "s"(dst) : "memory");
}

template <int BKT> DEVINL int nt_swz(int row) {
    return BKT == 64 ? ((row >> 1) & 7) : ((4 - ((row >> 2) & 3)) & 3);
}

template <int BKT, int SEGS_PER_WAVE, int NWAVES>
DEVINL void nt_stage(const bf16_t* G, int64_t ld, int64_t row0, int64_t nrows, int64_t k0, char* tile, int wave,
                     int lane) {
    constexpr int CPR = BKT / 8;
    constexpr int RPS = 64 / CPR;
#pragma unroll
    for (int q = 0; q < SEGS_PER_WAVE; ++q) {
        const int seg = q * NWAVES + wave;
        const int row = seg * RPS + lane / CPR;
        const int chunk = (lane % CPR) ^ nt_swz<BKT>(row);
        int64_t grow = row0 + row;
        grow = grow < nrows ? grow : nrows - 1;
        glds16(G + grow * ld + k0 + chunk * 8, tile + seg * 1024);
    }
}

template <int BKT> DEVINL s16x8 nt_frag(const char* tile, int row, int chunk) {
    return *(const s16x8*)(tile + row * (BKT * 2) + ((chunk ^ nt_swz<BKT>(row)) << 4));
}

DEVINL int tn_swz(int row) { return (((row & 3) << 1) | ((row >> 3) & 1)) << 1; }

template <int COLS, int SEGS_PER_WAVE, int NWAVES>
DEVINL void tn_stage(const bf16_t* G, int64_t ld, int64_t r0, int64_t r_end, int64_t n0, char* tile, int wave,
                     int lane) {
    constexpr int CPR = COLS / 8;
    constexpr int RPS = 64 / CPR;
#pragma unroll
    for (int q = 0; q < SEGS_PER_WAVE; ++q) {
        const int seg = q * NWAVES + wave;
        const int row = seg * RPS + lane / CPR;
        const int chunk = (lane % CPR) ^ tn_swz(row);
        const int64_t grow = r0 + row;
        const void* src = (grow < r_end) ? (const void*)(G + grow * ld + n0 + chunk * 8)
                                         : (const void*)((const char*)g_m3ae_zero_page + (lane & 15) * 16);
        glds16_raw(src, tile + seg * 1024);
    }
}

template <int COLS>
DEVINL s16x8 tn_frag(const char* tile, int kbase, int ncol0, int lane) {
    const int g = lane >> 4, i16 = lane & 15, q = i16 >> 2, p = i16 & 3;
    const int col = ncol0 + 4 * p;
    const int chunk = col >> 3, within = (col & 7) * 2;
    const int r1 = kbase + 8 * g + q, r2 = r1 + 4;
    const char* a1 = tile + r1 * (COLS * 2) + ((chunk ^ tn_swz(r1)) << 4) + within;
    const char* a2 = tile + r2 * (COLS * 2) + ((chunk ^ tn_swz(r2)) << 4) + within;
    typedef __attribute__((address_space(3))) s16x4 lds_s16x4;
    const s16x4 lo = __builtin_amdgcn_ds_read_tr16_b64_v4i16((lds_s16x4*)a1);
    const s16x4 hi = __builtin_amdgcn_ds_read_tr16_b64_v4i16((lds_s16x4*)a2);
    return (s16x8){lo[0], lo[1], lo[2], lo[3], hi[0], hi[1], hi[2], hi[3]};
}


template <int BKT> DEVINL int nt_frag_off(int row, int chunk) { return row * (BKT * 2) + ((chunk ^ nt_swz<BKT>(row)) << 4); }
DEVINL s16x8 nt_frag_at(const char* tile, int off) { return *(const s16x8*)(tile + off); }
template <int COLS> DEVINL void tn_frag_offs(int ncol0, int lane, int& o1, int& o2) {
    const int g = lane >> 4, i16 = lane & 15, q = i16 >> 2, p = i16 & 3;
    const int col = ncol0 + 4 * p;
    const int chunk = col >> 3, within = (col & 7) * 2;
    const int r1 = 8 * g + q, r2 = r1 + 4;
    o1 = r1 * (COLS * 2) + ((chunk ^ tn_swz(r1)) << 4) + within;
    o2 = r2 * (COLS * 2) + ((chunk ^ tn_swz(r2)) << 4) + within;
}
DEVINL s16x8 tn_frag_at(const char* tile, int o1, int o2) {
    typedef __attribute__((address_space(3))) s16x4 lds_s16x4;
    const s16x4 lo = __builtin_amdgcn_ds_read_tr16_b64_v4i16((lds_s16x4*)(tile + o1));
    const s16x4 hi = __builtin_amdgcn_ds_read_tr16_b64_v4i16((lds_s16x4*)(tile + o2));
    return (s16x8){lo[0], lo[1], lo[2], lo[3], hi[0], hi[1], hi[2], hi[3]};
}
```

mm-vqa-healthcare_amd/csrc/misc.hip:

```cpp
#include "common.h"
#include "det_fold.h"

namespace {

template <typename T> DEVINL float ldf(const void* p, int64_t i) { return Elem<T>::ld((const T*)p + i); }
template <typename T> DEVINL void stf(void* p, int64_t i, float v) { Elem<T>::st((T*)p + i, v); }

#define DT_SWITCH(dtype, CALL)                        \
    do {                                              \
        if ((dtype) == M3AE_F32) { using T = float; CALL; }        \
        else if ((dtype) == M3AE_BF16) { using T = bf16_t; CALL; } \
        else return M3AE_ERR_UNSUPPORTED;             \
    } while (0)

constexpr int EW_BLOCK = 256;
inline unsigned ew_grid(int64_t n) {
    int64_t g = cdiv(n, EW_BLOCK);
    return (unsigned)(g < 1 ? 1 : (g > 8192 ? 8192 : g));
}

template <typename T> DEVINL void ld8(const T* p, float* x);
template <> DEVINL void ld8<float>(const float* p, float* x) {
    const f32x4 a = *(const f32x4*)p, b = *(const f32x4*)(p + 4);
    x[0] = a[0]; x[1] = a[1]; x[2] = a[2]; x[3] = a[3]; x[4] = b[0]; x[5] = b[1]; x[6] = b[2]; x[7] = b[3];
// ... 384 lines not shown
        }
        tile[j][tx] = v;
    }
    __syncthreads();
    if (out_t) {
        for (int j = ty; j < 32; j += 8) {
            const int64_t c = c0 + j, r = r0 + tx;
            if (r < R && c < C) out_t[c * R + r] = f2bf(tile[tx][j]);
        }
    }
}
struct TransposeJob { const float* in; bf16_t* out_t; int64_t R, C; int64_t first_tile; };
__global__ void cast_transpose_batched_kernel(const TransposeJob* jobs, int njobs) {
    __shared__ float tile[32][33];
    const int64_t tid = blockIdx.x;
    int lo = 0, hi = njobs - 1;
    while (lo < hi) {
        const int mid = (lo + hi + 1) >> 1;
        if (jobs[mid].first_tile <= tid) lo = mid; else hi = mid - 1;
    }
    const TransposeJob j = jobs[lo];
    const int64_t local = tid - j.first_tile;
    const int64_t tiles_c = (j.C + 31) / 32;
    const int64_t c0 = (local % tiles_c) * 32, r0 = (local / tiles_c) * 32;
    const int tx = threadIdx.x & 31, ty = threadIdx.x >> 5;
    for (int k = ty; k < 32; k += 8) {
        const int64_t r = r0 + k, c = c0 + tx;
        tile[k][tx] = (r < j.R && c < j.C) ? j.in[r * j.C + c] : 0.f;
    }
    __syncthreads();
    for (int k = ty; k < 32; k += 8) {
        const int64_t c = c0 + k, r = r0 + tx;
        if (r < j.R && c < j.C) j.out_t[c * j.R + r] = f2bf(tile[tx][k]);
    }
}

struct TransposeJob16 { const bf16_t* in; bf16_t* out_t; int64_t R, C; int64_t first_tile; };
__global__ __launch_bounds__(256) void transpose_bf16_batched_kernel(const TransposeJob16* jobs, int njobs) {
    __shared__ __attribute__((aligned(16))) bf16_t tile[64][66];
    const int64_t tid = blockIdx.x;
    int lo = 0, hi = njobs - 1;
    while (lo < hi) {
        const int mid = (lo + hi + 1) >> 1;
        if (jobs[mid].first_tile <= tid) lo = mid; else hi = mid - 1;
    }
    const TransposeJob16 j = jobs[lo];
    const int64_t local = tid - j.first_tile;
    const int64_t tiles_c = (j.C + 63) / 64;
    const int64_t c0 = (local % tiles_c) * 64, r0 = (local / tiles_c) * 64;
    const int t = threadIdx.x, q = t >> 3, ch = t & 7;
    const bool fast = ((j.R | j.C) & 7) == 0 && r0 + 64 <= j.R && c0 + 64 <= j.C &&
                      ((((uintptr_t)j.in) | ((uintptr_t)j.out_t)) & 15) == 0;
    if (fast) {
#pragma unroll
        for (int p = 0; p < 2; ++p) {
            const int r = q + 32 * p;
            const u32x4 v = *(const u32x4*)(j.in + (r0 + r) * j.C + c0 + ch * 8);
            uint32_t* d = (uint32_t*)&tile[r][ch * 8];
            d[0] = v[0]; d[1] = v[1]; d[2] = v[2]; d[3] = v[3];
        }
        __syncthreads();
#pragma unroll
        for (int p = 0; p < 2; ++p) {
            const int c = q + 32 * p;
            u32x4 v;
#pragma unroll
            for (int i = 0; i < 4; ++i)
                v[i] = (uint32_t)tile[ch * 8 + 2 * i][c] | ((uint32_t)tile[ch * 8 + 2 * i + 1][c] << 16);
            *(u32x4*)(j.out_t + (c0 + c) * j.R + r0 + ch * 8) = v;
        }
        return;
    }
    for (int e = t; e < 64 * 64; e += 256) {
        const int r = e >> 6, c = e & 63;
        tile[r][c] = (r0 + r < j.R && c0 + c < j.C) ? j.in[(r0 + r) * j.C + c0 + c] : (bf16_t)0;
    }
    __syncthreads();
    for (int e = t; e < 64 * 64; e += 256) {
        const int c = e >> 6, r = e & 63;
        if (r0 + r < j.R && c0 + c < j.C) j.out_t[(c0 + c) * j.R + r0 + r] = tile[r][c];
    }
}

template <typename TI, typename TO>
__global__ void cast_kernel(const TI* in, TO* out, int64_t n) {
    for (int64_t i = (int64_t)blockIdx.x * blockDim.x + threadIdx.x; i < n; i += (int64_t)gridDim.x * blockDim.x)
        Elem<TO>::st(out + i, Elem<TI>::ld(in + i));
}
template <typename T>
__global__ void add_kernel(const T* a, const T* b, T* out, int64_t n) {
    for (int64_t i = (int64_t)blockIdx.x * blockDim.x + threadIdx.x; i < n; i += (int64_t)gridDim.x * blockDim.x)
        Elem<T>::st(out + i, Elem<T>::ld(a + i) + Elem<T>::ld(b + i));
}
__global__ void add_bf16x8_kernel(const u32x4* a, const u32x4* b, u32x4* out, int64_t n8) {
    for (int64_t i = (int64_t)blockIdx.x * blockDim.x + threadIdx.x; i < n8; i += (int64_t)gridDim.x * blockDim.x) {
        const u32x4 x = a[i], y = b[i];
        u32x4 r;
#pragma unroll
        for (int t = 0; t < 4; ++t)
            r[t] = pack2bf(__uint_as_float(x[t] << 16) + __uint_as_float(y[t] << 16),
                           __uint_as_float(x[t] & 0xffff0000u) + __uint_as_float(y[t] & 0xffff0000u));
        out[i] = r;
    }
}
template <typename T>
__global__ void act_fwd_kernel(const T* x, T* y, int64_t n, int act) {
    for (int64_t i = (int64_t)blockIdx.x * blockDim.x + threadIdx.x; i < n; i += (int64_t)gridDim.x * blockDim.x)
        Elem<T>::st(y + i, act_fwd(Elem<T>::ld(x + i), act));
}
template <typename T>
__global__ void act_bwd_kernel(const T* dy, const T* x, T* dx, int64_t n, int act) {
    for (int64_t i = (int64_t)blockIdx.x * blockDim.x + threadIdx.x; i < n; i += (int64_t)gridDim.x * blockDim.x)
        Elem<T>::st(dx + i, Elem<T>::ld(dy + i) * act_bwd(Elem<T>::ld(x + i), act));
}
template <typename T>
__global__ void dropout_kernel(const T* x, T* out, uint8_t* keep, int64_t n, int64_t cols, int64_t ld, DropState ds) {
    drop_resolve(ds);
    for (int64_t i = (int64_t)blockIdx.x * blockDim.x + threadIdx.x; i < n; i += (int64_t)gridDim.x * blockDim.x) {
        const int64_t r = i / cols;
        const bool k = drop_keep(ds, (uint64_t)(drop_row(ds, r) * ld + (i - r * cols)));
        if (out) Elem<T>::st(out + i, k ? Elem<T>::ld(x + i) * ds.inv_keep : 0.f);
        if (keep) keep[i] = k ? 1 : 0;
    }
}

template <typename T>
__global__ void gather_rows_kernel(const T* in, const int64_t* idx, T* out, int64_t n_out, int64_t D) {
    const int64_t total = n_out * D;
    for (int64_t i = (int64_t)blockIdx.x * blockDim.x + threadIdx.x; i < total; i += (int64_t)gridDim.x * blockDim.x) {
        const int64_t r = i / D, d = i - r * D;
        out[i] = in[idx[r] * D + d];
    }
}
template <typename T>
__global__ void scatter_add_rows_kernel(const T* d_out, const int64_t* idx, T* d_in, int64_t n_out, int64_t D) {
    const int64_t total = n_out * D;
    for (int64_t i = (int64_t)blockIdx.x * blockDim.x + threadIdx.x; i < total; i += (int64_t)gridDim.x * blockDim.x) {
        const int64_t r = i / D, d = i - r * D;
        const int64_t o = idx[r] * D + d;
        Elem<T>::st(d_in + o, Elem<T>::ld(d_in + o) + Elem<T>::ld(d_out + i));
    }
}

}

extern "C" int m3ae_abi_version(void) { return M3AE_ABI_VERSION; }
extern "C" void m3ae_desc_sizes(int64_t out3[3]) {
    out3[0] = (int64_t)sizeof(m3ae_gemm_desc); out3[1] = (int64_t)sizeof(m3ae_attn_desc); out3[2] = (int64_t)sizeof(m3ae_xattn_desc);
}

static int64_t colsum_chunks(int64_t M, int64_t N, int64_t* rows_per) {
    int64_t chunks = cdiv(1024, cdiv(N, 256));
    if (chunks > cdiv(M, 64)) chunks = cdiv(M, 64);
    if (chunks < 1) chunks = 1;
    *rows_per = cdiv(M, chunks);
    return cdiv(M, *rows_per);
}
static int colsum_impl(const void* x, float* out, int64_t M, int64_t N, int64_t ldx, int dtype, int accumulate, float* part,
                       hipStream_t s) {
    if (!part) {
        if (!accumulate) {
            hipError_t e = hipMemsetAsync(out, 0, N * sizeof(float), s);
            if (e != hipSuccess) return (int)e;
        }
        if (N % 8 == 0 && ldx == N && N / 8 <= 512 && M >= 4096 && ((((uintptr_t)x) & 15) == 0) &&
            (dtype == M3AE_BF16 || dtype == M3AE_F32)) {
// ... 92 lines not shown
                                        (const T*)d_out, (T*)d_patch, d_cls, d_pos, B, G, D));
    return hip_launch_status();
}

constexpr unsigned BCE_MAX_GRID = 64;
static int bce_impl(const void* logits, const float* targets, float* loss, void* d_logits, int64_t B, int64_t C, float grad_scale,
                    int dtype, float* part, hipStream_t s) {
    const int64_t n = B * C;
    const unsigned grid = ew_grid(n) > BCE_MAX_GRID ? BCE_MAX_GRID : ew_grid(n);
    if (part) {
        DT_SWITCH(dtype, hipLaunchKernelGGL((bce_kernel<T, true>), dim3(grid), dim3(EW_BLOCK), 0, s, (const T*)logits, targets, part,
                                            (T*)d_logits, n, 1.0f / (float)n, (float)C, grad_scale));
        det_fold(part, loss, nullptr, grid, 1, 1, 1, 1.0f, 0, s);
        return hip_launch_status();
    }
    hipError_t e = hipMemsetAsync(loss, 0, sizeof(float), s);
    if (e != hipSuccess) return (int)e;
    DT_SWITCH(dtype, hipLaunchKernelGGL(bce_kernel<T>, dim3(grid), dim3(EW_BLOCK), 0, s, (const T*)logits, targets, loss,
                                        (T*)d_logits, n, 1.0f / (float)n, (float)C, grad_scale));
    return hip_launch_status();
}
extern "C" int m3ae_bce_logits(const void* logits, const float* targets, float* loss, void* d_logits, int64_t B,
                               int64_t C, float grad_scale, int dtype, void* stream) {
    if (!logits || !targets || !loss || B <= 0 || C <= 0) return M3AE_ERR_ARG;
    return bce_impl(logits, targets, loss, d_logits, B, C, grad_scale, dtype, nullptr, (hipStream_t)stream);
}

static int xent_impl(const void* logits, const int64_t* labels, float* loss, void* d_logits, float* count, int64_t rows, int64_t C,
                     int64_t ld, float grad_scale, int dtype, float* part, hipStream_t s) {
    if (!part) {
        hipError_t e = hipMemsetAsync(loss, 0, sizeof(float), s);
        if (e != hipSuccess) return (int)e;
    }
    hipLaunchKernelGGL(xent_count_kernel, dim3(1), dim3(256), 0, s, labels, count, rows);
    if (part) {
        DT_SWITCH(dtype, hipLaunchKernelGGL((xent_kernel<T, true>), dim3((unsigned)rows), dim3(256), 0, s, (const T*)logits, labels,
                                            part, (T*)d_logits, count, C, ld, grad_scale));
        det_fold(part, loss, nullptr, rows, 1, 1, 1, 1.0f, 0, s);
    } else {
        DT_SWITCH(dtype, hipLaunchKernelGGL(xent_kernel<T>, dim3((unsigned)rows), dim3(256), 0, s, (const T*)logits, labels,
                                            loss, (T*)d_logits, count, C, ld, grad_scale));
    }
    return hip_launch_status();
}
extern "C" int m3ae_xent(const void* logits, const int64_t* labels, float* loss, void* d_logits, float* workspace,
                         int64_t rows, int64_t C, int64_t ld, float grad_scale, int dtype, void* stream) {
    if (!logits || !labels || !loss || !workspace || rows <= 0 || C <= 0) return M3AE_ERR_ARG;
    return xent_impl(logits, labels, loss, d_logits, workspace, rows, C, ld, grad_scale, dtype, nullptr, (hipStream_t)stream);
}

extern "C" int m3ae_adamw(float* p, const float* g, float* m, float* v, void* shadow_bf16, int64_t n, float lr,
                          float beta1, float beta2, float eps, float wd, int64_t step, float grad_scale,
                          const float* hyper_dev, void* stream) {
    if (!p || !g || !m || !v || n <= 0 || step <= 0) return M3AE_ERR_ARG;
    if (n % 4 != 0 || (((uintptr_t)p | (uintptr_t)g | (uintptr_t)m | (uintptr_t)v) & 15)) return M3AE_ERR_ALIGN;
    hipStream_t s = (hipStream_t)stream;
    const double bc1 = 1.0 - pow((double)beta1, (double)step), bc2 = 1.0 - pow((double)beta2, (double)step);
    const float step_size = (float)((double)lr * sqrt(bc2) / bc1);
    hipLaunchKernelGGL(adamw_kernel, dim3(ew_grid(n / 4)), dim3(EW_BLOCK), 0, s, p, g, m, v, (bf16_t*)shadow_bf16, n / 4,
                       lr, beta1, beta2, eps, wd, step_size, grad_scale, hyper_dev);
    return hip_launch_status();
}

extern "C" int m3ae_cast_transpose(const float* in, void* out, void* out_t, int64_t R, int64_t C, void* stream) {
    if (!in || R <= 0 || C <= 0) return M3AE_ERR_ARG;
    hipStream_t s = (hipStream_t)stream;
    dim3 grid((unsigned)cdiv(C, 32), (unsigned)cdiv(R, 32));
    if (grid.y > 65535u) return M3AE_ERR_UNSUPPORTED;
    hipLaunchKernelGGL(cast_transpose_kernel, grid, dim3(256), 0, s, in, (bf16_t*)out, (bf16_t*)out_t, R, C);
    return hip_launch_status();
}

extern "C" int m3ae_cast_transpose_batched(const void* jobs_dev, int njobs, int64_t total_tiles, void* stream) {
    if (!jobs_dev || njobs <= 0 || total_tiles <= 0) return M3AE_ERR_ARG;
    hipLaunchKernelGGL(cast_transpose_batched_kernel, dim3((unsigned)total_tiles), dim3(256), 0, (hipStream_t)stream,
                       (const TransposeJob*)jobs_dev, njobs);
    return hip_launch_status();
}

extern "C" int m3ae_transpose_bf16_batched(const void* jobs_dev, int njobs, int64_t total_tiles, void* stream) {
    if (!jobs_dev || njobs <= 0 || total_tiles <= 0) return M3AE_ERR_ARG;
    hipLaunchKernelGGL(transpose_bf16_batched_kernel, dim3((unsigned)total_tiles), dim3(256), 0, (hipStream_t)stream,
                       (const TransposeJob16*)jobs_dev, njobs);
    return hip_launch_status();
}

extern "C" int m3ae_cast(const void* in, void* out, int64_t n, int dtype_in, int dtype_out, void* stream) {
    if (!in || !out || n <= 0) return M3AE_ERR_ARG;
    hipStream_t s = (hipStream_t)stream;
    const dim3 g(ew_grid(n)), b(EW_BLOCK);
    if (dtype_in == M3AE_F32 && dtype_out == M3AE_BF16)
        hipLaunchKernelGGL((cast_kernel<float, bf16_t>), g, b, 0, s, (const float*)in, (bf16_t*)out, n);
    else if (dtype_in == M3AE_BF16 && dtype_out == M3AE_F32)
        hipLaunchKernelGGL((cast_kernel<bf16_t, float>), g, b, 0, s, (const bf16_t*)in, (float*)out, n);
    else if (dtype_in == M3AE_F32 && dtype_out == M3AE_F32)
        hipLaunchKernelGGL((cast_kernel<float, float>), g, b, 0, s, (const float*)in, (float*)out, n);
    else if (dtype_in == M3AE_BF16 && dtype_out == M3AE_BF16)
        hipLaunchKernelGGL((cast_kernel<bf16_t, bf16_t>), g, b, 0, s, (const bf16_t*)in, (bf16_t*)out, n);
    else return M3AE_ERR_UNSUPPORTED;
    return hip_launch_status();
}
extern "C" int m3ae_zero(void* p, int64_t bytes, void* stream) {
    if (!p || bytes <= 0) return M3AE_ERR_ARG;
    const hipError_t e = hipMemsetAsync(p, 0, (size_t)bytes, (hipStream_t)stream);
    return e == hipSuccess ? 0 : (int)e;
}
extern "C" int m3ae_add(const void* a, const void* b, void* out, int64_t n, int dtype, void* stream) {
    if (!a || !b || !out || n <= 0) return M3AE_ERR_ARG;
    hipStream_t s = (hipStream_t)stream;
    if (dtype == M3AE_BF16 && n % 8 == 0 && ((((uintptr_t)a) | ((uintptr_t)b) | ((uintptr_t)out)) & 15) == 0) {
        hipLaunchKernelGGL(add_bf16x8_kernel, dim3(ew_grid(n / 8)), dim3(EW_BLOCK), 0, s, (const u32x4*)a, (const u32x4*)b, (u32x4*)out, n / 8);
        return hip_launch_status();
    }
    DT_SWITCH(dtype, hipLaunchKernelGGL(add_kernel<T>, dim3(ew_grid(n)), dim3(EW_BLOCK), 0, s, (const T*)a, (const T*)b, (T*)out, n));
    return hip_launch_status();
}
extern "C" int m3ae_act_fwd(const void* x, void* y, int64_t n, int act, int dtype, void* stream) {
    if (!x || !y || n <= 0) return M3AE_ERR_ARG;
    hipStream_t s = (hipStream_t)stream;
    DT_SWITCH(dtype, hipLaunchKernelGGL(act_fwd_kernel<T>, dim3(ew_grid(n)), dim3(EW_BLOCK), 0, s, (const T*)x, (T*)y, n, act));
    return hip_launch_status();
}
extern "C" int m3ae_act_bwd(const void* dy, const void* x_pre, void* dx, int64_t n, int act, int dtype, void* stream) {
    if (!dy || !x_pre || !dx || n <= 0) return M3AE_ERR_ARG;
    hipStream_t s = (hipStream_t)stream;
    DT_SWITCH(dtype, hipLaunchKernelGGL(act_bwd_kernel<T>, dim3(ew_grid(n)), dim3(EW_BLOCK), 0, s, (const T*)dy, (const T*)x_pre, (T*)dx, n, act));
    return hip_launch_status();
}
extern "C" int m3ae_dropout(const void* x, void* out, uint8_t* keep_mask, int64_t rows, int64_t cols, float p,
                            uint64_t seed, const void* salt, int dtype, void* stream) {
    return m3ae_dropout_rows(x, out, keep_mask, rows, cols, p, seed, salt, dtype, 0, 1, stream);
}
extern "C" int m3ae_dropout_rows(const void* x, void* out, uint8_t* keep_mask, int64_t rows, int64_t cols, float p,
                                 uint64_t seed, const void* salt, int dtype, int64_t row_base, int64_t row_step, void* stream) {
    if (rows <= 0 || cols <= 0 || p < 0.f || p >= 1.f || (!out && !keep_mask) || (out && !x)) return M3AE_ERR_ARG;
    if (!drop_rows_ok(DropRows{row_base, row_step}, rows, cols)) return M3AE_ERR_ARG;
    const int64_t n = rows * cols;
    hipStream_t s = (hipStream_t)stream;
    const DropState ds = make_drop(p, seed, salt, DropRows{row_base, row_step});
    DT_SWITCH(dtype, hipLaunchKernelGGL(dropout_kernel<T>, dim3(ew_grid(n)), dim3(EW_BLOCK), 0, s, (const T*)x, (T*)out,
                                        keep_mask, n, cols, drop_ld(cols), ds));
    return hip_launch_status();
}

extern "C" int m3ae_gather_rows(const void* in, const int64_t* idx, void* out, int64_t n_out, int64_t D, int dtype,
                                void* stream) {
    if (!in || !idx || !out || n_out <= 0 || D <= 0) return M3AE_ERR_ARG;
    hipStream_t s = (hipStream_t)stream;
    DT_SWITCH(dtype, hipLaunchKernelGGL(gather_rows_kernel<T>, dim3(ew_grid(n_out * D)), dim3(EW_BLOCK), 0, s, (const T*)in, idx, (T*)out, n_out, D));
    return hip_launch_status();
}
extern "C" int m3ae_scatter_add_rows(const void* d_out, const int64_t* idx, void* d_in, int64_t n_out, int64_t D,
                                     int dtype, void* stream) {
    if (!d_out || !idx || !d_in || n_out <= 0 || D <= 0) return M3AE_ERR_ARG;
    hipStream_t s = (hipStream_t)stream;
    DT_SWITCH(dtype, hipLaunchKernelGGL(scatter_add_rows_kernel<T>, dim3(ew_grid(n_out * D)), dim3(EW_BLOCK), 0, s, (const T*)d_out, idx, (T*)d_in, n_out, D));
    return hip_launch_status();
}

namespace {
__global__ void mask_ranks_kernel(const float* __restrict__ noise, int64_t* __restrict__ ids_restore,
                                  int64_t* __restrict__ keep_rows, float* __restrict__ mask, int L, int len_keep) {
    extern __shared__ float row[];
    const int64_t b = blockIdx.x;
    for (int i = threadIdx.x; i < L; i += blockDim.x) row[i] = noise[b * L + i];
    __syncthreads();
// ... 204 lines not shown
```

mm-vqa-healthcare_amd/m3ae_amd/_lib.py:

```python
import ctypes as C
import os

_PKG = os.path.dirname(os.path.abspath(__file__))
DIAGNOSTIC = os.environ.get("M3AE_DIAGNOSTIC_LIB", "") == "1"
LIB_PATH = os.path.join(_PKG, "lib_diag" if DIAGNOSTIC else "lib", "libm3ae_hip.so")

F32, BF16 = 0, 1
ACT_NONE, ACT_GELU, ACT_QUICKGELU, ACT_TANH, ACT_RELU, ACT_MULAUX = 0, 1, 2, 3, 4, 5

vp, i64, i32, f32 = C.c_void_p, C.c_int64, C.c_int32, C.c_float


class GemmDesc(C.Structure):
    _fields_ = [
        ("M", i64), ("N", i64), ("K", i64), ("batch1", i64), ("batch2", i64),
        ("A", vp), ("a_sm", i64), ("a_sk", i64), ("a_sb1", i64), ("a_sb2", i64),
        ("B", vp), ("b_sk", i64), ("b_sn", i64), ("b_sb1", i64), ("b_sb2", i64),
        ("C", vp), ("c_sm", i64), ("c_sn", i64), ("c_sb1", i64), ("c_sb2", i64),
        ("dtype_a", i32), ("dtype_b", i32), ("dtype_c", i32),
        ("alpha", f32), ("accumulate", i32), ("bias", vp), ("act", i32), ("preact", vp), ("residual", vp),
        ("dact_aux", vp), ("dact", i32), ("force_generic", i32), ("a_rowsum", vp),
        ("dropout_p", f32), ("dropout_seed", C.c_uint64), ("preact_grad", i32), ("launch_flags", i32), ("dropout_salt", vp),
    ]


class AttnDesc(C.Structure):
    _fields_ = [
        ("B", i64), ("H", i64), ("Lq", i64), ("Lk", i64), ("Dh", i64),
        ("q", vp), ("q_sb", i64), ("q_sl", i64),
        ("k", vp), ("k_sb", i64), ("k_sl", i64),
        ("v", vp), ("v_sb", i64), ("v_sl", i64),
        ("o", vp), ("o_sb", i64), ("o_sl", i64),
        ("key_mask", vp), ("pos_bias", vp), ("scale", f32), ("causal", i32),
        ("lse", vp), ("lse_stride", i64), ("dtype", i32), ("workspace", vp), ("workspace_bytes", i64),
        ("d_o", vp), ("dq", vp), ("dk", vp), ("dv", vp), ("delta", vp), ("d_pos_bias", vp),
        ("dropout_p", f32), ("dropout_seed", C.c_uint64), ("dropout_salt", vp), ("launch_flags", i32),
    ]


class XattnDesc(C.Structure):
    _fields_ = [
        ("dir", i32), ("B", i64), ("Lq", i64), ("Lk", i64), ("D", i64), ("H", i64),
        ("x", vp), ("y", vp), ("key_mask", vp),
        ("wq", vp), ("wq_t", vp), ("wkv", vp), ("wkv_t", vp), ("wo", vp), ("wo_t", vp),
        ("bq", vp), ("bkv", vp), ("bo", vp), ("ln_g", vp), ("ln_b", vp),
        ("ln_eps", f32), ("dropout_p", f32), ("seed_attn", C.c_uint64), ("seed_hidden", C.c_uint64),
        ("proj", vp), ("prime", vp), ("colbias", vp), ("probs", vp), ("probs_drop", vp), ("rowsum", vp),
        ("zctx", vp), ("ctx", vp), ("s", vp), ("out", vp), ("mean", vp), ("rstd", vp),
        ("d_out", vp), ("dx", vp), ("dy", vp),
        ("g_wq", vp), ("g_wkv", vp), ("g_wo", vp), ("g_bq", vp), ("g_bkv", vp), ("g_bo", vp), ("g_ln_g", vp), ("g_ln_b", vp),
        ("ws_ds", vp), ("ws_dsd", vp), ("ws_dscores", vp), ("ws_dprime", vp), ("ws_dproj", vp), ("ws_dz", vp), ("ws_dctx", vp),
        ("ws_vec", vp), ("ws_ln", vp), ("launch_flags", i32), ("dropout_salt", vp),
    ]


GEMM_NO_PERSISTENT, GEMM_F32_X3, GEMM_DETERMINISTIC = 1, 2, 4
DET_COLSUM, DET_EMBED_BWD, DET_BCE, DET_XENT, DET_MIM = 0, 1, 2, 3, 4
ATTN_LEGACY_KERNELS, ATTN_F32_X3 = 1, 2
XATTN_NO_PERSISTENT, XATTN_LEGACY_CHAIN = 1, 2
ABI_VERSION = 4


_SIGS = {
    "m3ae_abi_version": (C.c_int, []),
    "m3ae_desc_sizes": (None, [C.POINTER(i64)]),
    "m3ae_last_gemm_path": (C.c_char_p, []),
    "m3ae_gemm": (C.c_int, [C.POINTER(GemmDesc), vp]),
    "m3ae_attn_workspace_bytes": (i64, [C.POINTER(AttnDesc), C.c_int]),
    "m3ae_attn_fwd": (C.c_int, [C.POINTER(AttnDesc), vp]),
    "m3ae_attn_bwd": (C.c_int, [C.POINTER(AttnDesc), vp]),
    "m3ae_attn_probs": (C.c_int, [C.POINTER(AttnDesc), vp, i64, i64, i64, vp]),
    "m3ae_xattn_supported": (C.c_int, [C.POINTER(XattnDesc)]),
    "m3ae_xattn_bwd_supported": (C.c_int, [C.POINTER(XattnDesc)]),
    "m3ae_xattn_probs_ld": (i64, [C.POINTER(XattnDesc)]),
    "m3ae_xattn_fwd": (C.c_int, [C.POINTER(XattnDesc), vp]),
    "m3ae_xattn_bwd": (C.c_int, [C.POINTER(XattnDesc), vp]),
    "m3ae_xattn_probs_export": (C.c_int, [C.POINTER(XattnDesc), C.c_int, vp, i64, i64, i64, vp]),
    "m3ae_layernorm_fwd": (C.c_int, [vp, vp, vp, vp, vp, vp, i64, i64, f32, C.c_int, C.c_int, C.c_int, vp]),
    "m3ae_layernorm_bwd_blocks": (i64, [i64]),
    "m3ae_layernorm_bwd": (C.c_int, [vp, vp, vp, vp, vp, vp, vp, vp, vp, vp, vp, i64, i64, C.c_int, C.c_int, C.c_int, vp]),
    "m3ae_layernorm_bwd_drop": (C.c_int, [vp, vp, vp, vp, vp, vp, vp, vp, f32, C.c_uint64, vp, vp, vp, vp, i64, i64, C.c_int, vp]),
    "m3ae_dropout": (C.c_int, [vp, vp, vp, i64, i64, f32, C.c_uint64, vp, C.c_int, vp]),
    "m3ae_colsum": (C.c_int, [vp, vp, i64, i64, i64, C.c_int, C.c_int, vp]),
    "m3ae_roberta_embed_fwd": (C.c_int, [vp, vp, vp, vp, vp, i64, i64, i64, i64, C.c_int, vp]),
    "m3ae_roberta_embed_bwd": (C.c_int, [vp, vp, vp, vp, vp, i64, i64, i64, i64, C.c_int, vp]),
    "m3ae_patchify": (C.c_int, [vp, vp, i64, i64, i64, C.c_int, vp]),
    "m3ae_image_normalize_u8": (C.c_int, [vp, vp, i64, i64, i64, C.POINTER(C.c_float), C.POINTER(C.c_float), vp]),
    "m3ae_vit_tokens_fwd": (C.c_int, [vp, vp, vp, vp, i64, i64, i64, C.c_int, vp]),
    "m3ae_vit_tokens_bwd": (C.c_int, [vp, vp, vp, vp, i64, i64, i64, C.c_int, vp]),
    "m3ae_bce_logits": (C.c_int, [vp, vp, vp, vp, i64, i64, f32, C.c_int, vp]),
    "m3ae_xent": (C.c_int, [vp, vp, vp, vp, vp, i64, i64, i64, f32, C.c_int, vp]),
    "m3ae_adamw": (C.c_int, [vp, vp, vp, vp, vp, i64, f32, f32, f32, f32, f32, i64, f32, vp, vp]),
    "m3ae_cast_transpose": (C.c_int, [vp, vp, vp, i64, i64, vp]),
    "m3ae_cast_transpose_batched": (C.c_int, [vp, C.c_int, i64, vp]),
    "m3ae_transpose_bf16_batched": (C.c_int, [vp, C.c_int, i64, vp]),
    "m3ae_cast": (C.c_int, [vp, vp, i64, C.c_int, C.c_int, vp]),
    "m3ae_zero": (C.c_int, [vp, i64, vp]),
    "m3ae_add": (C.c_int, [vp, vp, vp, i64, C.c_int, vp]),
    "m3ae_act_fwd": (C.c_int, [vp, vp, i64, C.c_int, C.c_int, vp]),
    "m3ae_act_bwd": (C.c_int, [vp, vp, vp, i64, C.c_int, C.c_int, vp]),
    "m3ae_gather_rows": (C.c_int, [vp, vp, vp, i64, i64, C.c_int, vp]),
    "m3ae_scatter_add_rows": (C.c_int, [vp, vp, vp, i64, i64, C.c_int, vp]),
    "m3ae_mask_ranks": (C.c_int, [vp, vp, vp, vp, i64, i64, i64, vp]),
    "m3ae_mim_targets": (C.c_int, [vp, vp, i64, i64, i64, i64, i64, C.c_int, vp]),
    "m3ae_mim_loss_fwd": (C.c_int, [vp, vp, vp, vp, vp, i64, i64, i64, C.c_int, vp]),
    "m3ae_mim_loss_bwd": (C.c_int, [vp, vp, vp, vp, vp, vp, i64, i64, i64, C.c_int, vp]),
    "m3ae_selftest": (C.c_int, [vp, vp]),
    "m3ae_gemm_det_workspace_bytes": (i64, [C.POINTER(GemmDesc)]),
    "m3ae_gemm_det": (C.c_int, [C.POINTER(GemmDesc), vp, i64, vp]),
    "m3ae_det_workspace_bytes": (i64, [C.c_int, i64, i64]),
    "m3ae_colsum_det": (C.c_int, [vp, vp, i64, i64, i64, C.c_int, C.c_int, vp, i64, vp]),
    "m3ae_layernorm_bwd_det": (C.c_int, [vp, vp, vp, vp, vp, vp, vp, vp, vp, vp, vp, i64, i64, C.c_int, C.c_int, C.c_int, vp]),
    "m3ae_layernorm_bwd_drop_det": (C.c_int, [vp, vp, vp, vp, vp, vp, vp, vp, f32, C.c_uint64, vp, vp, vp, vp, i64, i64, C.c_int, vp]),
    "m3ae_roberta_embed_bwd_det": (C.c_int, [vp, vp, vp, vp, vp, i64, i64, i64, i64, C.c_int, vp, i64, vp]),
    "m3ae_bce_logits_det": (C.c_int, [vp, vp, vp, vp, i64, i64, f32, C.c_int, vp, i64, vp]),
    "m3ae_xent_det": (C.c_int, [vp, vp, vp, vp, i64, i64, i64, f32, C.c_int, vp, i64, vp]),
    "m3ae_mim_loss_fwd_det": (C.c_int, [vp, vp, vp, vp, vp, i64, i64, i64, C.c_int, vp, i64, vp]),
    "m3ae_image_resample_workspace_bytes": (i64, [i64, i64]),
    "m3ae_image_resample_u8": (C.c_int, [vp, i64, vp, vp, i64, i64, i64, vp, i64, vp, vp, C.POINTER(C.c_float), C.POINTER(C.c_float), vp]),
    "m3ae_gemm_rows": (C.c_int, [C.POINTER(GemmDesc), i64, i64, vp]),
    "m3ae_attn_fwd_rows": (C.c_int, [C.POINTER(AttnDesc), i64, i64, vp]),
    "m3ae_attn_bwd_rows": (C.c_int, [C.POINTER(AttnDesc), i64, i64, vp]),
    "m3ae_layernorm_bwd_drop_rows": (C.c_int, [vp, vp, vp, vp, vp, vp, vp, vp, f32, C.c_uint64, vp, vp, vp, vp, i64, i64, C.c_int, i64, i64, vp]),
    "m3ae_dropout_rows": (C.c_int, [vp, vp, vp, i64, i64, f32, C.c_uint64, vp, C.c_int, i64, i64, vp]),
    "m3ae_beam_topk_workspace_bytes": (i64, [i64, i64, i64, i64]),
    "m3ae_beam_topk": (C.c_int, [vp, i64, vp, i64, i64, i64, i64, vp, i64, vp, vp, vp]),
    "m3ae_beam_step": (C.c_int, [vp, vp, vp, vp, vp, vp, vp, vp, vp, vp, vp, vp, vp, vp, i64, i64, i64, i64, i64, i64, i64, C.c_double, vp]),
    "m3ae_beam_finalize": (C.c_int, [vp, vp, vp, vp, vp, vp, vp, vp, vp, i64, i64, i64, i64, i64, i64, C.c_double, vp]),
    "m3ae_expand_samples": (C.c_int, [vp, vp, vp, i64, i64, i64, C.c_int, vp]),
    "m3ae_segment_sum_rows": (C.c_int, [vp, vp, vp, vp, i64, i64, i64, C.c_int, vp]),
    "m3ae_layernorm_fwd_mixed": (C.c_int, [vp, vp, vp, vp, vp, vp, i64, i64, f32, vp]),
    "m3ae_layernorm_bwd_mixed": (C.c_int, [vp, vp, vp, vp, vp, vp, vp, vp, vp, vp, vp, i64, i64, vp]),
    "m3ae_layernorm_bwd_mixed_det": (C.c_int, [vp, vp, vp, vp, vp, vp, vp, vp, vp, vp, vp, i64, i64, vp]),
}

EXPORTS = tuple(_SIGS)
_lib = None


class M3AEHipError(RuntimeError):
    pass


def lib():
    global _lib
    if _lib is None:
        if not os.path.exists(LIB_PATH):
            raise M3AEHipError(f"{LIB_PATH} is missing: build it with `python -m m3ae_amd.build` "
                               f"(or __graft_entry__.build()); this package has no CPU fallback")
        import torch
        if DIAGNOSTIC:
            import warnings
            warnings.warn(f"m3ae_amd: loading the DIAGNOSTIC library {LIB_PATH} (timing-only builds may compute wrong results)")
        l = C.CDLL(LIB_PATH)
        for name, (res, args) in _SIGS.items():
            fn = getattr(l, name)
            fn.restype, fn.argtypes = res, args
        if l.m3ae_abi_version() != ABI_VERSION:
            raise M3AEHipError(f"ABI version mismatch: library {l.m3ae_abi_version()}, binding {ABI_VERSION}")
        sizes = (i64 * 3)()
        l.m3ae_desc_sizes(sizes)
        mine = (C.sizeof(GemmDesc), C.sizeof(AttnDesc), C.sizeof(XattnDesc))
        if tuple(sizes) != mine:
            raise M3AEHipError(f"descriptor layout mismatch: library {tuple(sizes)}, binding {mine}")
        _lib = l
    return _lib


def check(rc, what):
    if rc != 0:
        kind = {-1: "invalid argument", -2: "unsupported shape/dtype", -3: "misaligned", -4: "workspace too small"}.get(
            rc, f"hipError_t {rc}" if rc > 0 else f"error {rc}")
        raise M3AEHipError(f"{what} failed: {kind}")
```

mm-vqa-healthcare_amd/m3ae_amd/ops.py:

```python
import contextlib
import ctypes as C
import functools
import math
import os
import threading

import torch

from . import _lib
from ._lib import (ACT_GELU, ACT_MULAUX, ACT_NONE, ACT_QUICKGELU, ACT_RELU, ACT_TANH, BF16, F32, AttnDesc, GemmDesc, XattnDesc,
                   check)

grad_ready_hook = None
SAVE_DACT = os.environ.get("M3AE_SAVE_DACT", "1") != "0"
NT_NO_PERSISTENT = os.environ.get("M3AE_NT_NO_PERSISTENT", "0") == "1"
GEMM_NT_VARIANT, GEMM_TN_VARIANT, GEMM_COL_GROUP = int(os.environ.get("M3AE_GEMM_NT_VARIANT", -1)), int(os.environ.get("M3AE_GEMM_TN_VARIANT", -1)), int(os.environ.get("M3AE_GEMM_COL_GROUP", 0))


ATTN_LEGACY = os.environ.get("M3AE_ATTN_LEGACY", "0") == "1"
GEMM_ST_POLICY = int(os.environ.get("M3AE_GEMM_ST_POLICY", 0))


def _gemm_flags():
    return ((1 if NT_NO_PERSISTENT else 0) | (((GEMM_NT_VARIANT + 1) & 0xF) << 8) | (((GEMM_TN_VARIANT + 1) & 0xF) << 12)
            | ((GEMM_COL_GROUP & 0xF) << 16) | ((GEMM_ST_POLICY & 0x3) << 20))
PROFILE = None


class _Mode(threading.local):
    x3 = False


_MODE = _Mode()


@contextlib.contextmanager
def f32x3_mode(on):
    prev, _MODE.x3 = _MODE.x3, bool(on)
    try:
        yield
    finally:
        _MODE.x3 = prev


def f32x3_active():
    return _MODE.x3


def model_mode(fn):
    @functools.wraps(fn)
    def run(self, *args, **kwargs):
        with f32x3_mode(getattr(self, "f32x3", False)):
            return fn(self, *args, **kwargs)
    return run


class DeterministicError(_lib.M3AEHipError):
    pass


_DETERMINISTIC = False


def set_deterministic(on):
    global _DETERMINISTIC
    _DETERMINISTIC = bool(on)


def deterministic():
    return _DETERMINISTIC


@contextlib.contextmanager
def deterministic_mode(on=True):
    prev = deterministic()
    set_deterministic(on)
    try:
        yield
    finally:
        set_deterministic(prev)


def _no_ordered_form(op):
    if _DETERMINISTIC:
        raise DeterministicError(f"{op} has no deterministic form (it adds with fp32 atomics) and ops.deterministic() is on: "
                                 f"switch the mode off for this op with ops.set_deterministic(False)")


def _det_ws(nbytes, device):
    return torch.empty(max(int(nbytes), 16), dtype=torch.uint8, device=device)


def _small_ws(op, rows, cols, device):
    n = _lib.lib().m3ae_det_workspace_bytes(op, rows, cols)
    if n < 0:
        check(int(n), "m3ae_det_workspace_bytes")
    return _det_ws(n, device), n


class Function(torch.autograd.Function):

    def __init_subclass__(cls, **kwargs):
        super().__init_subclass__(**kwargs)
# ... 23 lines not shown
    e0 = torch.cuda.Event(enable_timing=True)
    e0.record()
    return e0


def _prof_end(e0, kind, dims):
    if e0 is None:
        return
    e1 = torch.cuda.Event(enable_timing=True)
    e1.record()
    PROFILE.append((kind, dims, e0, e1))


_drop_base, _drop_ctr = 0x5EED, 0


def set_dropout_seed(seed):
    global _drop_base, _drop_ctr
    _drop_base, _drop_ctr = int(seed) & 0xFFFFFFFF, 0


DROPOUT_SALT = None


def _salt():
    return None if DROPOUT_SALT is None else C.c_void_p(DROPOUT_SALT.data_ptr())


def next_dropout_seed():
    global _drop_ctr
    _drop_ctr += 1
    return ((_drop_base << 32) | (_drop_ctr & 0xFFFFFFFF)) & 0xFFFFFFFFFFFFFFFF


def dropout_pair(p):
    return (p, next_dropout_seed()) if p > 0 else None


def _set_dropout(d, dropout):
    if dropout is not None and dropout[0] > 0:
        d.dropout_p, d.dropout_seed = dropout
        d.dropout_salt = _salt()


def _dt(t):
    if t.dtype == torch.float32:
        return F32
    if t.dtype == torch.bfloat16:
        return BF16
    raise TypeError(f"unsupported dtype {t.dtype}")


_raw_stream = getattr(torch._C, "_cuda_getCurrentRawStream", None)
_dev_index = None


def _stream():
    global _dev_index
    if _raw_stream is None:
        return C.c_void_p(torch.cuda.current_stream().cuda_stream)
    if _dev_index is None:
        _dev_index = torch.cuda.current_device()
    return C.c_void_p(_raw_stream(_dev_index))


def _p(t):
    return None if t is None else C.c_void_p(t.data_ptr())


def _need_cuda(t):
    if not t.is_cuda:
        raise _lib.M3AEHipError("m3ae_amd ops run on the GPU only (no CPU fallback); got a CPU tensor")
    if _dev_index is not None and t.device.index != _dev_index:
        raise _lib.M3AEHipError(f"m3ae_amd ops were first used on cuda:{_dev_index}; got a tensor on {t.device} "
                                f"(one process drives one GPU: call torch.cuda.set_device before the first op)")


def compute_weight(w):
    return getattr(w, "m3ae_c", w)


def gemm(a, a_sm, a_sk, b, b_sk, b_sn, c, c_sm, M, N, K, *, alpha=1.0, accumulate=False, bias=None, act=ACT_NONE,
         preact=None, residual=None, dact_aux=None, dact=ACT_NONE, force_generic=False, batch=(1, 1),
         a_sb=(0, 0), b_sb=(0, 0), c_sb=(0, 0), a_rowsum=None, dropout=None, preact_grad=False, rows=None):
    _need_cuda(c)
    d = GemmDesc()
    d.M, d.N, d.K = M, N, K
    d.batch1, d.batch2 = batch
    d.A, d.a_sm, d.a_sk, d.a_sb1, d.a_sb2 = a.data_ptr(), a_sm, a_sk, a_sb[0], a_sb[1]
    d.B, d.b_sk, d.b_sn, d.b_sb1, d.b_sb2 = b.data_ptr(), b_sk, b_sn, b_sb[0], b_sb[1]
    d.C, d.c_sm, d.c_sn, d.c_sb1, d.c_sb2 = c.data_ptr(), c_sm, 1, c_sb[0], c_sb[1]
    d.dtype_a, d.dtype_b, d.dtype_c = _dt(a), _dt(b), _dt(c)
    d.alpha = alpha
    d.accumulate = int(accumulate)
    if bias is not None:
        assert bias.dtype == torch.float32
        d.bias = bias.data_ptr()
    d.act = act
    for name, t in (("preact", preact), ("residual", residual), ("dact_aux", dact_aux)):
        if t is not None:
            assert t.dtype == c.dtype and t.stride(-1) == 1 and t.stride(-2) == c_sm, name
            setattr(d, name, t.data_ptr())
    d.dact = dact
    d.preact_grad = int(preact_grad)
    d.launch_flags = _gemm_flags()
    if _MODE.x3 and d.dtype_a == F32 and d.dtype_b == F32 and d.dtype_c == F32:
        d.launch_flags |= _lib.GEMM_F32_X3
    d.force_generic = int(force_generic)
    if a_rowsum is not None:
        assert a_rowsum.dtype == torch.float32 and a_rowsum.numel() >= M and batch == (1, 1)
        d.a_rowsum = a_rowsum.data_ptr()
    _set_dropout(d, dropout)
    e0 = _prof_begin()
    nws = _lib.lib().m3ae_gemm_det_workspace_bytes(C.byref(d)) if _DETERMINISTIC else 0
    if nws > 0:
        d.launch_flags |= _lib.GEMM_DETERMINISTIC
        ws = _det_ws(nws, c.device)
        check(_lib.lib().m3ae_gemm_det(C.byref(d), _p(ws), nws, _stream()), "m3ae_gemm_det")
        del ws
    elif rows is not None:
        check(_lib.lib().m3ae_gemm_rows(C.byref(d), rows[0], rows[1], _stream()), "m3ae_gemm_rows")
    else:
        check(_lib.lib().m3ae_gemm(C.byref(d), _stream()), "m3ae_gemm")
    if e0 is not None:
        _prof_end(e0, "gemm:" + last_gemm_path(), (M, N, K, batch[0] * batch[1]))


def last_gemm_path():
    return _lib.lib().m3ae_last_gemm_path().decode()


def _rows(x):
    K = x.shape[-1]
    if x.dim() == 2:
        assert x.stride(1) == 1
        return x, x.shape[0], K, x.stride(0)
    if not x.is_contiguous():
        x = x.contiguous()
    x2 = x.view(-1, K)
    return x2, x2.shape[0], K, K


_LAUNCH_STREAM = None


def launch_stream():
    global _LAUNCH_STREAM
    if _LAUNCH_STREAM is None:
        _LAUNCH_STREAM = torch.cuda.Stream(priority=-1)
    return _LAUNCH_STREAM


def use_launch_stream():
    prev = torch.cuda.current_stream()
    if os.environ.get("M3AE_LAUNCH_PRIORITY", "high") != "high":
        return prev
    torch.cuda.synchronize()
    torch.cuda.set_stream(launch_stream())
    return prev


def mm_nt(x2, ldx, M, w, bias=None, act=ACT_NONE, residual=None, want_preact=False, out_dtype=None, dact_aux=None,
          dact=ACT_NONE, force_generic=False, alpha=1.0, dropout=None, preact_grad=False, rows=None):
    N, K = w.shape
    y = torch.empty((M, N), dtype=out_dtype or x2.dtype, device=x2.device)
    pre = torch.empty_like(y) if want_preact else None
    gemm(x2, ldx, 1, w, 1, w.stride(0), y, N, M, N, K, bias=bias, act=act, preact=pre, residual=residual,
         dact_aux=dact_aux, dact=dact, force_generic=force_generic, alpha=alpha, dropout=dropout,
         preact_grad=preact_grad and want_preact, rows=rows)
    return y, pre


def mm_dgrad(dy, w_param, dact_aux=None, dact=ACT_NONE, residual=None, alpha=1.0, dropout=None, out=None, ld_out=None, rows=None):
    M, N = dy.shape
    wt = getattr(w_param, "m3ae_t", None)
    if wt is not None:
        b, b_sk, b_sn, K = wt, 1, wt.stride(0), wt.shape[0]
    else:
        b = compute_weight(w_param)
        b_sk, b_sn, K = b.stride(0), 1, b.shape[1]
    if out is None:
        out, ld_out = torch.empty((M, K), dtype=dy.dtype, device=dy.device), K
    gemm(dy, dy.stride(0), 1, b, b_sk, b_sn, out, ld_out, M, K, N, dact_aux=dact_aux, dact=dact, residual=residual,
         alpha=alpha, dropout=dropout, rows=rows)
    return out


def mm_wgrad(dy, x2, ldx, w_param, b_param=None, alpha=1.0):
    want_b = b_param is not None and b_param.requires_grad
    if not w_param.requires_grad:
        if want_b:
            bias_grad(dy, b_param)
        return
    g = _grad_buf(w_param)
    M, N = dy.shape
    K = g.shape[1]
    gemm(dy, 1, dy.stride(0), x2, ldx, 1, g, g.stride(0), N, K, M, accumulate=True, alpha=alpha,
         a_rowsum=_grad_buf(b_param) if want_b else None)
    _done(w_param)
    if want_b:
        _done(b_param)


def colsum(x, out, accumulate):
    M, N = x.shape
    if _DETERMINISTIC:
        ws, n = _small_ws(_lib.DET_COLSUM, M, N, x.device)
        check(_lib.lib().m3ae_colsum_det(_p(x), _p(out), M, N, x.stride(0), _dt(x), int(accumulate), _p(ws), n, _stream()),
              "m3ae_colsum_det")
        return
    check(_lib.lib().m3ae_colsum(_p(x), _p(out), M, N, x.stride(0), _dt(x), int(accumulate), _stream()), "m3ae_colsum")


def bias_grad(dy, b_param):
    if b_param is None or not b_param.requires_grad:
        return
    colsum(dy, _grad_buf(b_param), True)
    _done(b_param)


def act_bwd(dy, pre, act):
    dx = torch.empty_like(dy)
    check(_lib.lib().m3ae_act_bwd(_p(dy), _p(pre), _p(dx), dy.numel(), act, _dt(dy), _stream()), "m3ae_act_bwd")
    return dx


def _members(p):
    return getattr(p, "members", None) or ([p] if p is not None else [])


def _done(p):
    if grad_ready_hook is not None and p is not None:
        for m in _members(p):
            grad_ready_hook(m)


def _grad_buf(p):
    if getattr(p, "members", None) is not None:
        g = p.grad
        if g is None:
            raise _lib.M3AEHipError("packed parameters need ParamStore-managed gradients")
        return g
    if p.grad is None:
        p.grad = torch.zeros_like(p, dtype=torch.float32)
    return p.grad


def add(a, b, out=None):
    _need_cuda(a)
    a, b = a.contiguous(), b.contiguous()
    out = torch.empty_like(a) if out is None else out
    check(_lib.lib().m3ae_add(_p(a), _p(b), _p(out), a.numel(), _dt(a), _stream()), "m3ae_add")
    return out


def cast(x, dtype):
    if x.dtype == dtype:
        return x
    _need_cuda(x)
    x = x.contiguous()
    out = torch.empty_like(x, dtype=dtype)
    check(_lib.lib().m3ae_cast(_p(x), _p(out), x.numel(), _dt(x), _dt(out), _stream()), "m3ae_cast")
    return out


class Fork2Fn(Function):

# ... 1468 lines not shown
```

mm-vqa-healthcare_amd/m3ae_amd/param_store.py:

```python
import ctypes as C
import math

import torch

from . import _lib

ALIGN = 64

NO_DECAY = ["bias", "LayerNorm.bias", "LayerNorm.weight", "norm.bias", "norm.weight", "norm1.bias", "norm1.weight",
            "norm2.bias", "norm2.weight"]
HEAD_NAMES = ["mlm_head", "mim_head", "itm_head", "vqa_head", "cls_head", "irtr_head"]
NEVER_USED = ("vision_encoder.positional_embedding", "vision_encoder.token_embedding.weight",
              "vision_encoder.ln_final.weight", "vision_encoder.ln_final.bias",
              "language_encoder.pooler.dense.weight", "language_encoder.pooler.dense.bias")


def param_group_of(name):
    nd = any(k in name for k in NO_DECAY)
    hd = any(k in name for k in HEAD_NAMES)
    mm = "multi_modal" in name
    if not hd and not mm:
        return 1 if nd else 0
    if hd and not mm:
        return 3 if nd else 2
    if mm and not hd:
        return 5 if nd else 4
    return -1


def group_hparams(cfg):
    lr, wd = cfg["learning_rate"], cfg["weight_decay"]
    lh, lm = cfg["lr_multiplier_head"], cfg["lr_multiplier_multi_modal"]
    return [(lr, wd), (lr, 0.0), (lr * lh, wd), (lr * lh, 0.0), (lr * lm, wd), (lr * lm, 0.0)]


class PackedParam:

    def __init__(self, members):
        self.members = list(members)
        m0 = self.members[0]
        rows = sum(m.shape[0] for m in self.members)
        self.shape = (rows,) + tuple(m0.shape[1:])
        self.m3ae_t = None
        self._check_adjacent()

    def _check_adjacent(self):
        off = 0
        m0 = self.members[0]
        for m in self.members:
            if m.data_ptr() != m0.data_ptr() + off * m0.element_size():
                raise _lib.M3AEHipError("PackedParam members are not adjacent: apply ParamStore before forward")
            off += m.numel()

    def _view(self, t0):
        stride = (self.shape[1], 1) if len(self.shape) == 2 else (1,)
        return t0.as_strided(self.shape, stride)

    @property
    def data(self):
        return self._view(self.members[0].data)

    @property
    def m3ae_c(self):
        m0 = self.members[0]
        return self._view(getattr(m0, "m3ae_c", m0.data))

    @property
    def requires_grad(self):
        return all(m.requires_grad for m in self.members)

    @property
    def grad(self):
        g0 = self.members[0].grad
        return None if g0 is None else self._view(g0)


def param_group_of_decoder(name):
    nd = ["bias", "LayerNorm.bias", "LayerNorm.weight", "norm.bias", "norm.weight"]
    return 1 if any(k in name for k in nd) else 0


def group_hparams_decoder(cfg):
    lr, wd = cfg["learning_rate"], cfg["weight_decay"]
    return [(lr, wd), (lr, 0.0)] + [(lr, 0.0)] * 4


class ParamStore:
    def __init__(self, module, cfg, device, compute_dtype=torch.bfloat16, weight_units=None, frozen=(),
                 group_fn=param_group_of, hparams_fn=group_hparams):
        self.module, self.cfg, self.device, self.compute_dtype = module, cfg, device, compute_dtype
        self.streams = set()
        self.hparams_fn = hparams_fn
        named = [(n, p) for n, p in module.named_parameters()]
        self.names = {id(p): n for n, p in named}
        groups = [[] for _ in range(12)]
        for n, p in named:
            gi = group_fn(n)
            unused = any(n == u or n.endswith("." + u) for u in NEVER_USED) or any(n.startswith(f) for f in frozen)
            if unused or gi < 0 or not p.requires_grad:
                groups[6 + max(gi, 0)].append((n, p))
            else:
                groups[gi].append((n, p))
        self.groups = groups
        self.offset, self.segments = {}, []
        off = 0
        for gi, g in enumerate(groups):
            start = off
            for n, p in g:
                self.offset[id(p)] = off
                off += (p.numel() + ALIGN - 1) // ALIGN * ALIGN
            self.segments.append((start, off))
        self.total = off
        self.trainable_end = self.segments[5][1]
        self.flat = torch.zeros(self.total, dtype=torch.float32, device=device)
        self.grad = torch.zeros(self.trainable_end, dtype=torch.float32, device=device)
        self.exp_avg = None
        self.exp_avg_sq = None
        self.shadow = torch.zeros(self.total, dtype=torch.bfloat16, device=device) \
            if compute_dtype == torch.bfloat16 else None
        for gi, g in enumerate(groups):
            for n, p in g:
                o = self.offset[id(p)]
                view = self.flat[o:o + p.numel()].view(p.shape)
                view.copy_(p.data.to(device=device, dtype=torch.float32))
                p.data = view
                if gi < 6:
                    p.grad = self.grad[o:o + p.numel()].view(p.shape)
                else:
                    p.requires_grad_(False)
                    p.grad = None
                if self.shadow is not None:
                    p.m3ae_c = self.shadow[o:o + p.numel()].view(p.shape)
        self.step_count = 0
        self.units = list(weight_units() if callable(weight_units) else (weight_units or []))
        self._t_bufs = []
        if self.shadow is not None:
            for u in self.units:
                shp = u.shape
                rows, cols = shp[0], int(math.prod(shp[1:]))
                t = torch.empty((cols, rows), dtype=torch.bfloat16, device=device)
                u.m3ae_t = t
                self._t_bufs.append((u, rows, cols, t))
            import numpy as np
            tab = np.zeros((len(self._t_bufs), 5), dtype=np.int64)
            first = 0
            for i, (u, rows, cols, t) in enumerate(self._t_bufs):
                off = (u.data.data_ptr() - self.flat.data_ptr()) // 4
                assert 0 <= off < self.total
                tab[i] = (self.shadow.data_ptr() + 2 * off, t.data_ptr(), rows, cols, first)
                first += ((rows + 63) // 64) * ((cols + 63) // 64)
            self._t_tiles = first
            self._t_jobs = torch.from_numpy(tab).to(device)
        self.sync_shadows()

    @torch.no_grad()
    def sync_shadows(self, cast=True):
        if self.shadow is None:
            return
        L = _lib.lib()
        s = C.c_void_p(torch.cuda.current_stream().cuda_stream)
        if cast:
            _lib.check(L.m3ae_cast(C.c_void_p(self.flat.data_ptr()), C.c_void_p(self.shadow.data_ptr()), self.total,
                                   _lib.F32, _lib.BF16, s), "m3ae_cast")
        if self._t_bufs:
            _lib.check(L.m3ae_transpose_bf16_batched(C.c_void_p(self._t_jobs.data_ptr()), len(self._t_bufs),
                                                     self._t_tiles, s), "m3ae_transpose_bf16_batched")

    def zero_grad(self):
        from . import ops as _ops
        _lib.check(_lib.lib().m3ae_zero(C.c_void_p(self.grad.data_ptr()), self.grad.numel() * 4, _ops._stream()), "m3ae_zero")

    def lr_factor(self, step, max_steps):
        cfg = self.cfg
        warm = cfg["warmup_steps"]
        if isinstance(warm, float):
            warm = int(max_steps * warm)
        lr_init, lr_end, power = cfg["learning_rate"], cfg["end_lr"], cfg["decay_power"]
        if step < warm:
            return float(step) / float(max(1, warm))
        if power == "cosine":
            progress = float(step - warm) / float(max(1, max_steps - warm))
            return max(0.0, 0.5 * (1.0 + math.cos(math.pi * progress)))
        if step > max_steps:
            return lr_end / lr_init
        pct = 1 - (step - warm) / (max_steps - warm)
        return ((lr_init - lr_end) * pct ** power + lr_end) / lr_init

    def begin_update(self, max_steps=None, grad_scale=1.0, lr_factor=None, group_lrs=None, betas=(0.9, 0.98), eps=1e-8,
                     group_wds=None):
        if self.exp_avg is None:
            self.exp_avg = torch.zeros_like(self.grad)
            self.exp_avg_sq = torch.zeros_like(self.grad)
        hp = self.hparams_fn(self.cfg)
        if group_lrs is None:
            if lr_factor is None:
                max_steps = max_steps or self.cfg["max_steps"]
                lr_factor = self.lr_factor(self.step_count, max_steps)
            group_lrs = [lr * lr_factor for lr, _ in hp]
        if group_wds is None:
            group_wds = [wd for _, wd in hp]
        self.step_count += 1
        return dict(lrs=[float(x) for x in group_lrs], wds=[float(x) for x in group_wds], b1=float(betas[0]), b2=float(betas[1]),
                    eps=float(eps), step=self.step_count, grad_scale=grad_scale)

    hyper_dev = None

    def _hyper_dev_ptr(self, gi):
        return None if self.hyper_dev is None else C.c_void_p(self.hyper_dev.data_ptr() + 8 * gi)

    @staticmethod
    def hyper_values(hyper):
        t = hyper["step"]
        bc1, bc2 = 1.0 - hyper["b1"] ** t, 1.0 - hyper["b2"] ** t
        return [[lr, lr * math.sqrt(bc2) / bc1] for lr in hyper["lrs"]]

    @torch.no_grad()
    def adamw_range(self, a, b, gi, hyper):
        if b <= a:
            return
        from . import ops as _ops
        es = 4
        sh = C.c_void_p(self.shadow.data_ptr() + a * 2) if self.shadow is not None else None
        _lib.check(_lib.lib().m3ae_adamw(C.c_void_p(self.flat.data_ptr() + a * es), C.c_void_p(self.grad.data_ptr() + a * es),
                                         C.c_void_p(self.exp_avg.data_ptr() + a * es),
                                         C.c_void_p(self.exp_avg_sq.data_ptr() + a * es), sh, b - a, hyper["lrs"][gi],
                                         hyper["b1"], hyper["b2"], hyper["eps"], hyper["wds"][gi], hyper["step"],
                                         hyper["grad_scale"], self._hyper_dev_ptr(gi), _ops._stream()), "m3ae_adamw")

    @torch.no_grad()
    def adamw_step(self, max_steps=None, grad_scale=1.0, lr_factor=None, group_lrs=None, betas=(0.9, 0.98), eps=1e-8,
                   group_wds=None):
        self.adamw_apply(self.begin_update(max_steps, grad_scale, lr_factor, group_lrs, betas, eps, group_wds))

    @torch.no_grad()
    def adamw_apply(self, hyper):
        for gi in range(6):
            a, b = self.segments[gi]
            self.adamw_range(a, min(b, self.trainable_end), gi, hyper)
        self.sync_shadows(cast=False)

    def make_optimizer(self, max_steps=None):
        max_steps = max_steps or self.cfg["max_steps"]
        opt = FlatAdamW(self)
        sched = torch.optim.lr_scheduler.LambdaLR(opt, lambda step: self.lr_factor(step, max_steps))
        return [opt], [{"scheduler": sched, "interval": "step"}]

    def group_names(self):
        return [[n for n, _ in g] for g in self.groups[:6]]

# ... 70 lines not shown
```

Before: 1430.

## Store bf16 weight shadows in pre-tiled GEMM layout for contiguous B staging

Adds a tiled bf16 weight layout (256-row by 32-k chunks, with the LDS swizzle baked in) that is produced when shadows are synced, covering both the forward weight and its transpose. The NT GEMM kernels (mfma, pp, pp2) and the generic path gain a B_TILED flag, so B tiles load as contiguous 1KB segments with simpler address math. The aim is less address arithmetic and better coalescing of B loads in the weight GEMMs. In exchange it keeps extra weight copies in memory and runs an extra tiling kernel after each optimizer step.

```diff
diff --git a/include/m3ae_hip.h b/include/m3ae_hip.h
--- a/include/m3ae_hip.h
+++ b/include/m3ae_hip.h
@@ -43,7 +43,8 @@
 } m3ae_gemm_desc;
 enum { M3AE_GEMM_NO_PERSISTENT = 1,
        M3AE_GEMM_F32_X3 = 2,
-       M3AE_GEMM_DETERMINISTIC = 4  };
+       M3AE_GEMM_DETERMINISTIC = 4,
+       M3AE_GEMM_B_TILED = 8    };
 #define M3AE_GEMM_NT_VARIANT(v) ((((v) + 1) & 0xf) << 8)
 #define M3AE_GEMM_TN_VARIANT(v) ((((v) + 1) & 0xf) << 12)
 #define M3AE_GEMM_COL_GROUP(g) (((g) & 0xf) << 16)
@@ -189,6 +190,7 @@
 int m3ae_cast_transpose(const float* in, void* out, void* out_t, int64_t R, int64_t C, void* stream);
 int m3ae_cast_transpose_batched(const void* jobs_dev, int njobs, int64_t total_tiles, void* stream);
 int m3ae_transpose_bf16_batched(const void* jobs_dev, int njobs, int64_t total_tiles, void* stream);
+int m3ae_tile_bf16_batched(const void* jobs_dev, int njobs, int64_t total_tiles, void* stream);
 int m3ae_cast(const void* in, void* out, int64_t n, int dtype_in, int dtype_out, void* stream);
 int m3ae_zero(void* p, int64_t bytes, void* stream);
 int m3ae_add(const void* a, const void* b, void* out, int64_t n, int dtype, void* stream);
diff --git a/mm-vqa-healthcare_amd/csrc/common.h b/mm-vqa-healthcare_amd/csrc/common.h
--- a/mm-vqa-healthcare_amd/csrc/common.h
+++ b/mm-vqa-healthcare_amd/csrc/common.h
@@ -2,6 +2,7 @@
 #include <hip/hip_runtime.h>
 #include <stdint.h>
 #include "m3ae_hip.h"
+#include "tiled_b.h"
 
 typedef uint16_t bf16_t;
 typedef __attribute__((ext_vector_type(2))) float f32x2;
diff --git a/mm-vqa-healthcare_amd/csrc/gemm_generic.hip b/mm-vqa-healthcare_amd/csrc/gemm_generic.hip
--- a/mm-vqa-healthcare_amd/csrc/gemm_generic.hip
+++ b/mm-vqa-healthcare_amd/csrc/gemm_generic.hip
@@ -16,6 +16,7 @@
     const TB* B = (const TB*)d.B + b1 * d.b_sb1 + b2 * d.b_sb2;
     const int64_t coff = b1 * d.c_sb1 + b2 * d.c_sb2;
     const bool a_kfast = (d.a_sk == 1), b_nfast = (d.b_sn == 1);
+    const bool b_tiled = (d.launch_flags & M3AE_GEMM_B_TILED) != 0;
 
     float acc[4][4];
 #pragma unroll
@@ -43,7 +44,8 @@
             if (b_nfast) { nn = e & 63; kk = e >> 6; } else { kk = e & 15; nn = e >> 4; }
             int64_t gn = n0 + nn, gk = k0 + kk;
             float v = 0.f;
-            if (gn < d.N && gk < d.K) v = Elem<TB>::ld(B + gk * d.b_sk + gn * d.b_sn);
+            if (gn < d.N && gk < d.K)
+                v = Elem<TB>::ld(b_tiled ? B + m3ae_tiled_b_index(gn, gk, d.K) : B + gk * d.b_sk + gn * d.b_sn);
             Bs[kk][nn] = v;
         }
         __syncthreads();
diff --git a/mm-vqa-healthcare_amd/csrc/gemm_mfma.hip b/mm-vqa-healthcare_amd/csrc/gemm_mfma.hip
--- a/mm-vqa-healthcare_amd/csrc/gemm_mfma.hip
+++ b/mm-vqa-healthcare_amd/csrc/gemm_mfma.hip
@@ -40,7 +40,8 @@
     for (int s = 0; s < NST - 1; ++s) {
         if (s < nt) {
             nt_stage<BKT, A_SEGS, NWAVES>(a.A, a.lda, m0, a.M, (int64_t)s * BKT, smem + s * ST_BYTES, wave, lane);
-            nt_stage<BKT, B_SEGS, NWAVES>(a.B, a.ldb, n0, a.N, (int64_t)s * BKT, smem + s * ST_BYTES + A_BYTES, wave, lane);
+            if (a.b_tiled) nt_stage_tiled<BKT, B_SEGS, NWAVES>(a.B, a.K, n0, (int64_t)s * BKT, smem + s * ST_BYTES + A_BYTES, wave, lane);
+            else nt_stage<BKT, B_SEGS, NWAVES>(a.B, a.ldb, n0, a.N, (int64_t)s * BKT, smem + s * ST_BYTES + A_BYTES, wave, lane);
         }
     }
 
@@ -54,7 +55,8 @@
         if (t + NST - 1 < nt) {
             char* nxt = smem + nxt_s * ST_BYTES;
             nt_stage<BKT, A_SEGS, NWAVES>(a.A, a.lda, m0, a.M, (int64_t)(t + NST - 1) * BKT, nxt, wave, lane);
-            nt_stage<BKT, B_SEGS, NWAVES>(a.B, a.ldb, n0, a.N, (int64_t)(t + NST - 1) * BKT, nxt + A_BYTES, wave, lane);
+            if (a.b_tiled) nt_stage_tiled<BKT, B_SEGS, NWAVES>(a.B, a.K, n0, (int64_t)(t + NST - 1) * BKT, nxt + A_BYTES, wave, lane);
+            else nt_stage<BKT, B_SEGS, NWAVES>(a.B, a.ldb, n0, a.N, (int64_t)(t + NST - 1) * BKT, nxt + A_BYTES, wave, lane);
         }
         const char* At = smem + cur_s * ST_BYTES;
         const char* Bt = At + A_BYTES;
@@ -266,6 +268,20 @@
 #define PP_STAGE(G, ld, r0, nr, k0, tile) nt_stage<CK, 2, NW>(G, ld, r0, nr, k0, tile, wave, lane)
 #endif
 
+#if defined(M3AE_EXP_NT_CONTIG) && defined(M3AE_EXP_NT_CONTIG_B)
+#ifdef M3AE_EXP_NT_L2HOT
+#define PP_STAGE_A(G, ld, r0, nr, k0, tile) nt_stage<CK, 2, NW>(G, ld, 0, nr, k0, tile, wave, lane)
+#else
+#define PP_STAGE_A(G, ld, r0, nr, k0, tile) nt_stage<CK, 2, NW>(G, ld, r0, nr, k0, tile, wave, lane)
+#endif
+#else
+#define PP_STAGE_A(G, ld, r0, nr, k0, tile) PP_STAGE(G, ld, r0, nr, k0, tile)
+#endif
+#define PP_STAGE_B(k0, tile) do { \
+        if (a.b_tiled) nt_stage_tiled32<2, NW>(a.B, a.K, n0, k0, tile, wave, lane); \
+        else PP_STAGE(a.B, a.ldb, n0, a.N, k0, tile); \
+    } while (0)
+
 template <int EPI>
 __global__ __launch_bounds__(512, 2) void gemm_nt_pp_kernel(MfmaArgs a) {
     if (a.has_drop) drop_resolve(a.drop);
@@ -292,8 +308,8 @@
 #pragma unroll
     for (int c = 0; c < 3; ++c) {
         if (c < nc) {
-            PP_STAGE(a.B, a.ldb, n0, a.N, (int64_t)c * CK, smem + c * SLOT + A_BYTES);
-            PP_STAGE(a.A, a.lda, m0, a.M, (int64_t)c * CK, smem + c * SLOT);
+            PP_STAGE_B((int64_t)c * CK, smem + c * SLOT + A_BYTES);
+            PP_STAGE_A(a.A, a.lda, m0, a.M, (int64_t)c * CK, smem + c * SLOT);
         }
     }
     if (nc >= 3) asm volatile("s_waitcnt vmcnt(8)" ::: "memory");
@@ -315,7 +331,7 @@
         for (int j = 0; j < 4; ++j) bfr[j] = nt_frag<CK>(Bt, wc * 64 + j * 16 + frow, fchunk);
 #pragma unroll
         for (int i = 0; i < 4; ++i) af[i] = nt_frag<CK>(At, wr * 128 + i * 16 + frow, fchunk);
-        if (more) PP_STAGE(a.B, a.ldb, n0, a.N, (int64_t)(c + 3) * CK, nxt + A_BYTES);
+        if (more) PP_STAGE_B((int64_t)(c + 3) * CK, nxt + A_BYTES);
         PP_FENCE();
         __builtin_amdgcn_s_barrier();
         PP_FENCE();
@@ -334,7 +350,7 @@
         PP_FENCE();
 #pragma unroll
         for (int i = 0; i < 4; ++i) af[i] = nt_frag<CK>(At, wr * 128 + 64 + i * 16 + frow, fchunk);
-        if (more) PP_STAGE(a.A, a.lda, m0, a.M, (int64_t)(c + 3) * CK, nxt);
+        if (more) PP_STAGE_A(a.A, a.lda, m0, a.M, (int64_t)(c + 3) * CK, nxt);
         {
             const int rem = nc - 1 - c;
             if (rem >= 3) asm volatile("s_waitcnt vmcnt(8)" ::: "memory");
@@ -418,8 +434,8 @@
 #pragma unroll
     for (int c = 0; c < 3; ++c) {
         char* sl = smem + ((c + 2) & 3) * SLOT;
-        PP_STAGE(a.B, a.ldb, n0, a.N, (int64_t)c * CK, sl + A_BYTES);
-        PP_STAGE(a.A, a.lda, m0, a.M, (int64_t)c * CK, sl);
+        PP_STAGE_B((int64_t)c * CK, sl + A_BYTES);
+        PP_STAGE_A(a.A, a.lda, m0, a.M, (int64_t)c * CK, sl);
     }
     int top_wait = 0;
 #ifdef M3AE_NT_TRACE
@@ -454,7 +470,7 @@
 #pragma unroll
             for (int i = 0; i < 4; ++i) af[i] = nt_frag<CK>(At, wr * 128 + i * 16 + frow, fchunk);
             NT_ACC(0);
-            if (more) PP_STAGE(a.B, a.ldb, n0, a.N, (int64_t)(c + 3) * CK, nxt + A_BYTES);
+            if (more) PP_STAGE_B((int64_t)(c + 3) * CK, nxt + A_BYTES);
             NT_ACC(1);
             PP_FENCE();
             __builtin_amdgcn_s_barrier();
@@ -479,7 +495,7 @@
 #pragma unroll
             for (int i = 0; i < 4; ++i) af[i] = nt_frag<CK>(At, wr * 128 + 64 + i * 16 + frow, fchunk);
             NT_ACC(0);
-            if (more) PP_STAGE(a.A, a.lda, m0, a.M, (int64_t)(c + 3) * CK, nxt);
+            if (more) PP_STAGE_A(a.A, a.lda, m0, a.M, (int64_t)(c + 3) * CK, nxt);
             NT_ACC(1);
             {
                 const int rem = nc - 1 - c;
@@ -522,8 +538,8 @@
 #pragma unroll
             for (int c = 0; c < 2; ++c) {
                 char* sl = smem + ((c + 2) & 3) * SLOT;
-                PP_STAGE(a.B, a.ldb, n0, a.N, (int64_t)c * CK, sl + A_BYTES);
-                PP_STAGE(a.A, a.lda, m0, a.M, (int64_t)c * CK, sl);
+                PP_STAGE_B((int64_t)c * CK, sl + A_BYTES);
+                PP_STAGE_A(a.A, a.lda, m0, a.M, (int64_t)c * CK, sl);
             }
         }
         if (a.c_f32) epilogue_rows<float, EPI, 8, 1>(a, smem, wave, lane, m_cur + wr * 128, n_cur + wc * 64, acc);
@@ -539,8 +555,8 @@
         PP_FENCE();
         {
             char* sl = smem + ((2 + 2) & 3) * SLOT;
-            PP_STAGE(a.B, a.ldb, n0, a.N, (int64_t)2 * CK, sl + A_BYTES);
-            PP_STAGE(a.A, a.lda, m0, a.M, (int64_t)2 * CK, sl);
+            PP_STAGE_B((int64_t)2 * CK, sl + A_BYTES);
+            PP_STAGE_A(a.A, a.lda, m0, a.M, (int64_t)2 * CK, sl);
         }
         v = vn;
     }
@@ -603,6 +619,7 @@
     a.drop = make_drop(d.dropout_p, d.dropout_seed, d.dropout_salt, rows);
     a.no_persist = (d.launch_flags & M3AE_GEMM_NO_PERSISTENT) ? 1 : 0;
     a.nt_variant = ((d.launch_flags >> 8) & 0xf) - 1;
+    a.b_tiled = (d.launch_flags & M3AE_GEMM_B_TILED) ? 1 : 0;
     a.st_policy = (d.launch_flags >> 20) & 0x3;
     if (a.st_policy == 0) a.st_policy = (d.M * d.N >= (int64_t)16 << 20) ? 3 : 1;
     const bool has_act = d.act != M3AE_ACT_NONE, has_dact = d.dact_aux != nullptr;
@@ -975,6 +992,10 @@
     if (route == ROUTE_BAD_DIMS) return M3AE_ERR_ARG;
     const DropRows rows{row_base, row_step};
     if (!drop_rows_ok(rows, d.M, d.N)) return M3AE_ERR_ARG;
+    if ((d.launch_flags & M3AE_GEMM_B_TILED) &&
+        (d.dtype_a != M3AE_BF16 || d.dtype_b != M3AE_BF16 || d.b_sk != 1 || d.b_sn != d.K || d.K % 32 != 0 || d.batch1 != 1 ||
+         d.batch2 != 1 || (d.launch_flags & M3AE_GEMM_F32_X3) || !aligned16(d.B)))
+        return M3AE_ERR_UNSUPPORTED;
     if (route == ROUTE_TN && d.dropout_p > 0.f && (row_base != 0 || row_step != 1)) return M3AE_ERR_UNSUPPORTED;
     if (d.launch_flags & M3AE_GEMM_DETERMINISTIC) return M3AE_ERR_UNSUPPORTED;
     hipStream_t s = (hipStream_t)stream;
@@ -1009,6 +1030,7 @@
     if (!dp || !dp->A || !dp->B || !dp->C) return M3AE_ERR_ARG;
     const m3ae_gemm_desc& d = *dp;
     if (!(d.launch_flags & M3AE_GEMM_DETERMINISTIC)) return M3AE_ERR_ARG;
+    if (d.launch_flags & M3AE_GEMM_B_TILED) return M3AE_ERR_UNSUPPORTED;
     if (gemm_route(d) != ROUTE_TN) return M3AE_ERR_UNSUPPORTED;
     if (!workspace || !aligned16(workspace) || workspace_bytes < m3ae_gemm_det_workspace_bytes(dp)) return M3AE_ERR_WORKSPACE;
     g_last_path = "mfma_tn";
diff --git a/mm-vqa-healthcare_amd/csrc/gemm_nt_common.h b/mm-vqa-healthcare_amd/csrc/gemm_nt_common.h
--- a/mm-vqa-healthcare_amd/csrc/gemm_nt_common.h
+++ b/mm-vqa-healthcare_amd/csrc/gemm_nt_common.h
@@ -30,6 +30,7 @@
     int no_persist;
     int nt_variant;
     int st_policy;
+    int b_tiled;
 };
 
 DEVINL void nt_tile_coords(unsigned wg, unsigned tiles_m, unsigned tiles_n, unsigned& tm, unsigned& tn, unsigned GC = 4) {
diff --git a/mm-vqa-healthcare_amd/csrc/gemm_nt_pp2.hip b/mm-vqa-healthcare_amd/csrc/gemm_nt_pp2.hip
--- a/mm-vqa-healthcare_amd/csrc/gemm_nt_pp2.hip
+++ b/mm-vqa-healthcare_amd/csrc/gemm_nt_pp2.hip
@@ -127,7 +127,7 @@
     }
 }
 
-template <int EPI>
+template <int EPI, bool TILED>
 __global__ __launch_bounds__(512, 2) void gemm_nt_pp2_kernel(MfmaArgs a) {
     if (a.has_drop) drop_resolve(a.drop);
     constexpr int CK = 32, A_BYTES = 256 * CK * 2, SLOT = 2 * A_BYTES, RING = 4 * SLOT;
@@ -165,16 +165,23 @@
         const unsigned c0 = (unsigned)(((lane_p & 3) ^ nt_swz<CK>(r0)) * 16), c1 = (unsigned)(((lane_p & 3) ^ nt_swz<CK>(r1)) * 16);
         const int ma = (int)(a.M - 1 - m0 < 255 ? a.M - 1 - m0 : 255), mb = (int)(a.N - 1 - n0 < 255 ? a.N - 1 - n0 : 255);
         abase = a.A + m0 * a.lda;
-        bbase = a.B + n0 * a.ldb;
         va0 = (unsigned)(r0 < ma ? r0 : ma) * (unsigned)a.lda * 2u + c0;
         va1 = (unsigned)(r1 < ma ? r1 : ma) * (unsigned)a.lda * 2u + c1;
-        vb0 = (unsigned)(r0 < mb ? r0 : mb) * (unsigned)a.ldb * 2u + c0;
-        vb1 = (unsigned)(r1 < mb ? r1 : mb) * (unsigned)a.ldb * 2u + c1;
+        if (TILED) {
+            bbase = a.B + (n0 >> 8) * (int64_t)nc * M3AE_TB_CHUNK_ELEMS;
+            vb0 = (unsigned)wave * 1024u + (unsigned)lane_p * 16u;
+            vb1 = vb0 + 8192u;
+        } else {
+            bbase = a.B + n0 * a.ldb;
+            vb0 = (unsigned)(r0 < mb ? r0 : mb) * (unsigned)a.ldb * 2u + c0;
+            vb1 = (unsigned)(r1 < mb ? r1 : mb) * (unsigned)a.ldb * 2u + c1;
+        }
     };
+    constexpr int b_cstep = TILED ? M3AE_TB_CHUNK_ELEMS : CK;
     auto issue_b = [&](int c) {
         const unsigned dst = lds_wave + (unsigned)(c & 3) * SLOT + A_BYTES;
-        glds16_asm(bbase + (int64_t)c * CK, vb0, dst);
-        glds16_asm(bbase + (int64_t)c * CK, vb1, dst + 8192u);
+        glds16_asm(bbase + (int64_t)c * b_cstep, vb0, dst);
+        glds16_asm(bbase + (int64_t)c * b_cstep, vb1, dst + 8192u);
     };
     auto issue_a = [&](int c) {
         const unsigned dst = lds_wave + (unsigned)(c & 3) * SLOT;
@@ -304,7 +311,8 @@
     const int dev = current_device();
     const int64_t tiles = cdiv(a.M, 256) * cdiv(a.N, 256), cus = device_cus8(dev);
     const unsigned grid = (unsigned)(persistent && tiles > cus ? cus : tiles);
-    return launch_dyn_on<gemm_nt_pp2_kernel<EPI>>(dev, dim3(grid), dim3(512), lds, s, a);
+    if (a.b_tiled) return launch_dyn_on<gemm_nt_pp2_kernel<EPI, true>>(dev, dim3(grid), dim3(512), lds, s, a);
+    return launch_dyn_on<gemm_nt_pp2_kernel<EPI, false>>(dev, dim3(grid), dim3(512), lds, s, a);
 }
 
 int launch_pp2_e(const MfmaArgs& a, int epi, bool persistent, hipStream_t s) {
diff --git a/mm-vqa-healthcare_amd/csrc/mfma_tiles.h b/mm-vqa-healthcare_amd/csrc/mfma_tiles.h
--- a/mm-vqa-healthcare_amd/csrc/mfma_tiles.h
+++ b/mm-vqa-healthcare_amd/csrc/mfma_tiles.h
@@ -41,6 +41,27 @@
         int64_t grow = row0 + row;
         grow = grow < nrows ? grow : nrows - 1;
         glds16(G + grow * ld + k0 + chunk * 8, tile + seg * 1024);
+    }
+}
+
+template <int BKT, int SEGS_PER_WAVE, int NWAVES>
+DEVINL void nt_stage_tiled(const bf16_t* Bt, int64_t K, int64_t row0, int64_t k0, char* tile, int wave, int lane) {
+    constexpr int CPR = BKT / 8, RPS = 64 / CPR;
+#pragma unroll
+    for (int q = 0; q < SEGS_PER_WAVE; ++q) {
+        const int seg = q * NWAVES + wave;
+        const int row = seg * RPS + lane / CPR;
+        const int chunk = (lane % CPR) ^ nt_swz<BKT>(row);
+        glds16(Bt + m3ae_tiled_b_index(row0 + row, k0 + chunk * 8, K), tile + seg * 1024);
+    }
+}
+template <int SEGS_PER_WAVE, int NWAVES>
+DEVINL void nt_stage_tiled32(const bf16_t* Bt, int64_t K, int64_t row0, int64_t k0, char* tile, int wave, int lane) {
+    const bf16_t* src = Bt + ((row0 >> 8) * (K >> 5) + (k0 >> 5)) * M3AE_TB_CHUNK_ELEMS + lane * 8;
+#pragma unroll
+    for (int q = 0; q < SEGS_PER_WAVE; ++q) {
+        const int seg = q * NWAVES + wave;
+        glds16(src + seg * M3AE_TB_BLOCK_ELEMS, tile + seg * 1024);
     }
 }
 
diff --git a/mm-vqa-healthcare_amd/csrc/misc.hip b/mm-vqa-healthcare_amd/csrc/misc.hip
--- a/mm-vqa-healthcare_amd/csrc/misc.hip
+++ b/mm-vqa-healthcare_amd/csrc/misc.hip
@@ -490,6 +490,47 @@
     }
 }
 
+struct TileJob16 { const bf16_t* in; bf16_t* out_tiled; bf16_t* out_t; bf16_t* out_t_tiled; int64_t R, C; int64_t first_tile; };
+__global__ __launch_bounds__(256) void tile_bf16_batched_kernel(const TileJob16* jobs, int njobs) {
+    __shared__ __attribute__((aligned(16))) bf16_t tile[64][66];
+    const int64_t tid = blockIdx.x;
+    int lo = 0, hi = njobs - 1;
+    while (lo < hi) {
+        const int mid = (lo + hi + 1) >> 1;
+        if (jobs[mid].first_tile <= tid) lo = mid; else hi = mid - 1;
+    }
+    const TileJob16 j = jobs[lo];
+    const int64_t local = tid - j.first_tile;
+    const int64_t Rp = j.out_tiled ? m3ae_tiled_b_rows(j.R) : j.R, Cp = j.out_t_tiled ? m3ae_tiled_b_rows(j.C) : j.C;
+    const int64_t tiles_c = (Cp + 63) / 64;
+    const int64_t c0 = (local % tiles_c) * 64, r0 = (local / tiles_c) * 64;
+    const int t = threadIdx.x, q = t >> 3, ch = t & 7;
+#pragma unroll
+    for (int p = 0; p < 2; ++p) {
+        const int r = q + 32 * p;
+        const int64_t gr = r0 + r, gc = c0 + ch * 8;
+        u32x4 v = (u32x4){0u, 0u, 0u, 0u};
+        if (gr < j.R && gc < j.C) v = *(const u32x4*)(j.in + gr * j.C + gc);
+        uint32_t* d = (uint32_t*)&tile[r][ch * 8];
+        d[0] = v[0]; d[1] = v[1]; d[2] = v[2]; d[3] = v[3];
+        if (j.out_tiled && gr < Rp && gc < j.C) *(u32x4*)(j.out_tiled + m3ae_tiled_b_index(gr, gc, j.C)) = v;
+    }
+    if (!j.out_t && !j.out_t_tiled) return;
+    __syncthreads();
+#pragma unroll
+    for (int p = 0; p < 2; ++p) {
+        const int c = q + 32 * p;
+        const int64_t gc = c0 + c, gr = r0 + ch * 8;
+        if (gr >= j.R) continue;
+        u32x4 v;
+#pragma unroll
+        for (int i = 0; i < 4; ++i)
+            v[i] = (uint32_t)tile[ch * 8 + 2 * i][c] | ((uint32_t)tile[ch * 8 + 2 * i + 1][c] << 16);
+        if (j.out_t && gc < j.C) *(u32x4*)(j.out_t + gc * j.R + gr) = v;
+        if (j.out_t_tiled && gc < Cp) *(u32x4*)(j.out_t_tiled + m3ae_tiled_b_index(gc, gr, j.R)) = v;
+    }
+}
+
 template <typename TI, typename TO>
 __global__ void cast_kernel(const TI* in, TO* out, int64_t n) {
     for (int64_t i = (int64_t)blockIdx.x * blockDim.x + threadIdx.x; i < n; i += (int64_t)gridDim.x * blockDim.x)
@@ -748,6 +789,13 @@
     if (!jobs_dev || njobs <= 0 || total_tiles <= 0) return M3AE_ERR_ARG;
     hipLaunchKernelGGL(transpose_bf16_batched_kernel, dim3((unsigned)total_tiles), dim3(256), 0, (hipStream_t)stream,
                        (const TransposeJob16*)jobs_dev, njobs);
+    return hip_launch_status();
+}
+
+extern "C" int m3ae_tile_bf16_batched(const void* jobs_dev, int njobs, int64_t total_tiles, void* stream) {
+    if (!jobs_dev || njobs <= 0 || total_tiles <= 0 || total_tiles > 0x7fffffffLL) return M3AE_ERR_ARG;
+    hipLaunchKernelGGL(tile_bf16_batched_kernel, dim3((unsigned)total_tiles), dim3(256), 0, (hipStream_t)stream,
+                       (const TileJob16*)jobs_dev, njobs);
     return hip_launch_status();
 }
 
diff --git a/mm-vqa-healthcare_amd/csrc/tiled_b.h b/mm-vqa-healthcare_amd/csrc/tiled_b.h
--- /dev/null
+++ b/mm-vqa-healthcare_amd/csrc/tiled_b.h
@@ -0,0 +1,19 @@
+#pragma once
+#include <stdint.h>
+
+#if defined(__HIPCC__) || defined(__CUDACC__)
+#define M3AE_TB_FN __host__ __device__ __forceinline__
+#else
+#define M3AE_TB_FN static inline
+#endif
+
+enum { M3AE_TB_ROWS = 256, M3AE_TB_CK = 32, M3AE_TB_BLOCK_ROWS = 16, M3AE_TB_BLOCK_ELEMS = 512, M3AE_TB_CHUNK_ELEMS = 8192 };
+
+M3AE_TB_FN int64_t m3ae_tiled_b_rows(int64_t N) { return (N + M3AE_TB_ROWS - 1) / M3AE_TB_ROWS * M3AE_TB_ROWS; }
+
+M3AE_TB_FN int64_t m3ae_tiled_b_index(int64_t n, int64_t k, int64_t K) {
+    const int64_t T = n >> 8, c = k >> 5;
+    const int p = (int)(n >> 4) & 15, r = (int)n & 15, u = (int)(k >> 3) & 3;
+    const int swz = (4 - ((r >> 2) & 3)) & 3;
+    return (T * (K >> 5) + c) * M3AE_TB_CHUNK_ELEMS + p * M3AE_TB_BLOCK_ELEMS + r * 32 + ((u ^ swz) << 3) + (int)(k & 7);
+}
diff --git a/mm-vqa-healthcare_amd/m3ae_amd/_lib.py b/mm-vqa-healthcare_amd/m3ae_amd/_lib.py
--- a/mm-vqa-healthcare_amd/m3ae_amd/_lib.py
+++ b/mm-vqa-healthcare_amd/m3ae_amd/_lib.py
@@ -54,7 +54,7 @@
     ]
 
 
-GEMM_NO_PERSISTENT, GEMM_F32_X3, GEMM_DETERMINISTIC = 1, 2, 4
+GEMM_NO_PERSISTENT, GEMM_F32_X3, GEMM_DETERMINISTIC, GEMM_B_TILED = 1, 2, 4, 8
 DET_COLSUM, DET_EMBED_BWD, DET_BCE, DET_XENT, DET_MIM = 0, 1, 2, 3, 4
 ATTN_LEGACY_KERNELS, ATTN_F32_X3 = 1, 2
 XATTN_NO_PERSISTENT, XATTN_LEGACY_CHAIN = 1, 2
@@ -94,6 +94,7 @@
     "m3ae_cast_transpose": (C.c_int, [vp, vp, vp, i64, i64, vp]),
     "m3ae_cast_transpose_batched": (C.c_int, [vp, C.c_int, i64, vp]),
     "m3ae_transpose_bf16_batched": (C.c_int, [vp, C.c_int, i64, vp]),
+    "m3ae_tile_bf16_batched": (C.c_int, [vp, C.c_int, i64, vp]),
     "m3ae_cast": (C.c_int, [vp, vp, i64, C.c_int, C.c_int, vp]),
     "m3ae_zero": (C.c_int, [vp, i64, vp]),
     "m3ae_add": (C.c_int, [vp, vp, vp, i64, C.c_int, vp]),
diff --git a/mm-vqa-healthcare_amd/m3ae_amd/ops.py b/mm-vqa-healthcare_amd/m3ae_amd/ops.py
--- a/mm-vqa-healthcare_amd/m3ae_amd/ops.py
+++ b/mm-vqa-healthcare_amd/m3ae_amd/ops.py
@@ -19,6 +19,7 @@
 
 ATTN_LEGACY = os.environ.get("M3AE_ATTN_LEGACY", "0") == "1"
 GEMM_ST_POLICY = int(os.environ.get("M3AE_GEMM_ST_POLICY", 0))
+TILED_B = os.environ.get("M3AE_TILED_B", "1") != "0"
 
 
 def _gemm_flags():
@@ -208,7 +209,7 @@
 
 def gemm(a, a_sm, a_sk, b, b_sk, b_sn, c, c_sm, M, N, K, *, alpha=1.0, accumulate=False, bias=None, act=ACT_NONE,
          preact=None, residual=None, dact_aux=None, dact=ACT_NONE, force_generic=False, batch=(1, 1),
-         a_sb=(0, 0), b_sb=(0, 0), c_sb=(0, 0), a_rowsum=None, dropout=None, preact_grad=False, rows=None):
+         a_sb=(0, 0), b_sb=(0, 0), c_sb=(0, 0), a_rowsum=None, dropout=None, preact_grad=False, rows=None, b_tiled=False):
     _need_cuda(c)
     d = GemmDesc()
     d.M, d.N, d.K = M, N, K
@@ -229,7 +230,7 @@
             setattr(d, name, t.data_ptr())
     d.dact = dact
     d.preact_grad = int(preact_grad)
-    d.launch_flags = _gemm_flags()
+    d.launch_flags = _gemm_flags() | (_lib.GEMM_B_TILED if b_tiled else 0)
     if _MODE.x3 and d.dtype_a == F32 and d.dtype_b == F32 and d.dtype_c == F32:
         d.launch_flags |= _lib.GEMM_F32_X3
     d.force_generic = int(force_generic)
@@ -291,16 +292,20 @@
     N, K = w.shape
     y = torch.empty((M, N), dtype=out_dtype or x2.dtype, device=x2.device)
     pre = torch.empty_like(y) if want_preact else None
-    gemm(x2, ldx, 1, w, 1, w.stride(0), y, N, M, N, K, bias=bias, act=act, preact=pre, residual=residual,
+    tb = getattr(w, "m3ae_tb", None) if TILED_B and x2.dtype == torch.bfloat16 and w.stride(0) == K else None
+    gemm(x2, ldx, 1, w if tb is None else tb, 1, w.stride(0), y, N, M, N, K, bias=bias, act=act, preact=pre, residual=residual,
          dact_aux=dact_aux, dact=dact, force_generic=force_generic, alpha=alpha, dropout=dropout,
-         preact_grad=preact_grad and want_preact, rows=rows)
+         preact_grad=preact_grad and want_preact, rows=rows, b_tiled=tb is not None)
     return y, pre
 
 
 def mm_dgrad(dy, w_param, dact_aux=None, dact=ACT_NONE, residual=None, alpha=1.0, dropout=None, out=None, ld_out=None, rows=None):
     M, N = dy.shape
     wt = getattr(w_param, "m3ae_t", None)
-    if wt is not None:
+    wtt = getattr(w_param, "m3ae_tt", None) if TILED_B and wt is not None and dy.dtype == torch.bfloat16 else None
+    if wtt is not None:
+        b, b_sk, b_sn, K = wtt, 1, N, wt.shape[0]
+    elif wt is not None:
         b, b_sk, b_sn, K = wt, 1, wt.stride(0), wt.shape[0]
     else:
         b = compute_weight(w_param)
@@ -308,7 +313,7 @@
     if out is None:
         out, ld_out = torch.empty((M, K), dtype=dy.dtype, device=dy.device), K
     gemm(dy, dy.stride(0), 1, b, b_sk, b_sn, out, ld_out, M, K, N, dact_aux=dact_aux, dact=dact, residual=residual,
-         alpha=alpha, dropout=dropout, rows=rows)
+         alpha=alpha, dropout=dropout, rows=rows, b_tiled=wtt is not None)
     return out
 
 
diff --git a/mm-vqa-healthcare_amd/m3ae_amd/param_store.py b/mm-vqa-healthcare_amd/m3ae_amd/param_store.py
--- a/mm-vqa-healthcare_amd/m3ae_amd/param_store.py
+++ b/mm-vqa-healthcare_amd/m3ae_amd/param_store.py
@@ -42,6 +42,7 @@
         rows = sum(m.shape[0] for m in self.members)
         self.shape = (rows,) + tuple(m0.shape[1:])
         self.m3ae_t = None
+        self.m3ae_tb = self.m3ae_tt = None
         self._check_adjacent()
 
     def _check_adjacent(self):
@@ -63,7 +64,10 @@
     @property
     def m3ae_c(self):
         m0 = self.members[0]
-        return self._view(getattr(m0, "m3ae_c", m0.data))
+        v = self._view(getattr(m0, "m3ae_c", m0.data))
+        if self.m3ae_tb is not None:
+            v.m3ae_tb = self.m3ae_tb
+        return v
 
     @property
     def requires_grad(self):
@@ -141,16 +145,36 @@
                 t = torch.empty((cols, rows), dtype=torch.bfloat16, device=device)
                 u.m3ae_t = t
                 self._t_bufs.append((u, rows, cols, t))
+            from . import ops as _ops, tiled_b as _tb
+            self._tile_jobs, tiled, plain = None, [], []
+            for (u, rows, cols, t) in self._t_bufs:
+                off = (u.data.data_ptr() - self.flat.data_ptr()) // 4
+                assert 0 <= off < self.total
+                ok = _ops.TILED_B and len(u.shape) == 2 and rows % 8 == 0 and cols % 8 == 0 and (rows % 32 == 0 or cols % 32 == 0)
+                if not ok:
+                    plain.append((u, rows, cols, t))
+                    continue
+                src = self.shadow[off:off + rows * cols].view(rows, cols)
+                fwd = torch.empty(_tb.tiled_rows(rows) * cols, dtype=torch.bfloat16, device=device) if cols % 32 == 0 else None
+                tt = torch.empty(_tb.tiled_rows(cols) * rows, dtype=torch.bfloat16, device=device) if rows % 32 == 0 else None
+                tiled.append((src, fwd, t, tt))
+                u.m3ae_tt = tt
+                if isinstance(u, PackedParam):
+                    u.m3ae_tb = fwd
+                elif fwd is not None:
+                    u.m3ae_c.m3ae_tb = fwd
+            if tiled:
+                self._tile_jobs = _tb.job_table(tiled, device)
             import numpy as np
-            tab = np.zeros((len(self._t_bufs), 5), dtype=np.int64)
+            tab = np.zeros((len(plain), 5), dtype=np.int64)
             first = 0
-            for i, (u, rows, cols, t) in enumerate(self._t_bufs):
+            for i, (u, rows, cols, t) in enumerate(plain):
                 off = (u.data.data_ptr() - self.flat.data_ptr()) // 4
                 assert 0 <= off < self.total
                 tab[i] = (self.shadow.data_ptr() + 2 * off, t.data_ptr(), rows, cols, first)
                 first += ((rows + 63) // 64) * ((cols + 63) // 64)
-            self._t_tiles = first
-            self._t_jobs = torch.from_numpy(tab).to(device)
+            self._t_tiles, self._t_njobs = first, len(plain)
+            self._t_jobs = torch.from_numpy(tab).to(device) if plain else None
         self.sync_shadows()
 
     @torch.no_grad()
@@ -162,9 +186,12 @@
         if cast:
             _lib.check(L.m3ae_cast(C.c_void_p(self.flat.data_ptr()), C.c_void_p(self.shadow.data_ptr()), self.total,
                                    _lib.F32, _lib.BF16, s), "m3ae_cast")
-        if self._t_bufs:
-            _lib.check(L.m3ae_transpose_bf16_batched(C.c_void_p(self._t_jobs.data_ptr()), len(self._t_bufs),
+        if self._t_bufs and self._t_jobs is not None:
+            _lib.check(L.m3ae_transpose_bf16_batched(C.c_void_p(self._t_jobs.data_ptr()), self._t_njobs,
                                                      self._t_tiles, s), "m3ae_transpose_bf16_batched")
+        if self._t_bufs and self._tile_jobs is not None:
+            from . import tiled_b as _tb
+            _tb.run(*self._tile_jobs, stream=s)
 
     def zero_grad(self):
         from . import ops as _ops
diff --git a/mm-vqa-healthcare_amd/m3ae_amd/tiled_b.py b/mm-vqa-healthcare_amd/m3ae_amd/tiled_b.py
--- /dev/null
+++ b/mm-vqa-healthcare_amd/m3ae_amd/tiled_b.py
@@ -0,0 +1,69 @@
+import ctypes as C
+
+import numpy as np
+import torch
+
+from . import _lib
+
+ROWS, CK, BLOCK_ELEMS, CHUNK_ELEMS = 256, 32, 512, 8192
+
+
+def tiled_rows(N):
+    return (N + ROWS - 1) // ROWS * ROWS
+
+
+def tiled_index(n, k, K):
+    T, c = n >> 8, k >> 5
+    p, r, u = (n >> 4) & 15, n & 15, (k >> 3) & 3
+    swz = (4 - ((r >> 2) & 3)) & 3
+    return (T * (K >> 5) + c) * CHUNK_ELEMS + p * BLOCK_ELEMS + r * 32 + ((u ^ swz) << 3) + (k & 7)
+
+
+def tile_reference(w):
+    N, K = w.shape
+    assert K % CK == 0
+    out = torch.zeros(tiled_rows(N) * K, dtype=w.dtype, device=w.device)
+    n = torch.arange(N, device=w.device, dtype=torch.int64)[:, None]
+    k = torch.arange(K, device=w.device, dtype=torch.int64)[None, :]
+    out[tiled_index(n, k, K).reshape(-1)] = w.reshape(-1)
+    return out
+
+
+def job_tiles(R, C_, fwd, t_tiled):
+    Rp = tiled_rows(R) if fwd else R
+    Cp = tiled_rows(C_) if t_tiled else C_
+    return ((Rp + 63) // 64) * ((Cp + 63) // 64)
+
+
+def job_table(entries, device):
+    tab = np.zeros((len(entries), 7), dtype=np.int64)
+    first = 0
+    for i, (src, out_tiled, out_t, out_t_tiled) in enumerate(entries):
+        R, C_ = src.shape
+        assert src.dtype == torch.bfloat16 and src.is_contiguous() and R % 8 == 0 and C_ % 8 == 0
+        for t, need in ((src, R * C_), (out_tiled, tiled_rows(R) * C_), (out_t, R * C_), (out_t_tiled, tiled_rows(C_) * R)):
+            assert t is None or (t.dtype == torch.bfloat16 and t.is_contiguous() and t.numel() >= need and t.data_ptr() % 16 == 0)
+        assert out_tiled is None or C_ % CK == 0
+        assert out_t_tiled is None or R % CK == 0
+        ptr = lambda t: 0 if t is None else t.data_ptr()
+        tab[i] = (src.data_ptr(), ptr(out_tiled), ptr(out_t), ptr(out_t_tiled), R, C_, first)
+        first += job_tiles(R, C_, out_tiled is not None, out_t_tiled is not None)
+    return torch.from_numpy(tab).to(device), len(entries), first
+
+
+def run(jobs, njobs, tiles, stream=None):
+    s = C.c_void_p(torch.cuda.current_stream().cuda_stream) if stream is None else stream
+    _lib.check(_lib.lib().m3ae_tile_bf16_batched(C.c_void_p(jobs.data_ptr()), njobs, tiles, s), "m3ae_tile_bf16_batched")
+
+
+def attach(w_param, device=None):
+    w = w_param.m3ae_c
+    N, K = w.shape
+    fwd = torch.empty(tiled_rows(N) * K, dtype=torch.bfloat16, device=w.device) if K % CK == 0 else None
+    tt = torch.empty(tiled_rows(K) * N, dtype=torch.bfloat16, device=w.device) if N % CK == 0 else None
+    jobs, n, tiles = job_table([(w, fwd, None, tt)], w.device)
+    run(jobs, n, tiles)
+    if fwd is not None:
+        w.m3ae_tb = fwd
+    w_param.m3ae_tt = tt
+    return fwd, tt
```

Measured after the change: 1449 (median of 6 runs). 1.01x the previous value.
